# AronCao49/MoPA

Hardware: AMD Instinct MI355X
Metric: scans/sec (joint 2D+3D train step) at 1/2/4/8 MI355X; sparse-conv HBM GB/s (higher is better)
Workload: dtype f32

## Files before the change

### include/mopa_hip.h

```cpp
#ifndef MOPA_HIP_H
#define MOPA_HIP_H
#include <stddef.h>
#include <stdint.h>
#ifdef __cplusplus
extern "C" {
#endif


size_t mopa_scan_workspace_bytes(int64_t n);
int mopa_scan_exclusive_i32(const int32_t* in, int32_t* out, int32_t n, int32_t* total, void* ws, size_t ws_bytes, void* stream);
size_t mopa_voxel_hash_workspace_bytes(int64_t n_points);
int mopa_voxel_hash_build(const int64_t* coords, int64_t n_points, uint64_t* table_keys, int32_t* table_vals, int64_t table_cap, int32_t* point_row, uint64_t* row_keys, int32_t* num_rows, int32_t* status, void* ws, size_t ws_bytes, void* stream);
size_t mopa_coarsen_workspace_bytes(int64_t n_fine_cap);
int mopa_coarsen_build(const uint64_t* fine_keys, int32_t n_fine_cap, const int32_t* n_fine_dev, uint64_t* table_keys, int32_t* table_vals, int64_t table_cap, int32_t* parent, uint64_t* coarse_keys, int32_t* num_coarse, void* ws, size_t ws_bytes, void* stream);
int mopa_group_split(const int32_t* item_row, const int32_t* n_dev, int32_t n_host, int32_t n_cap, int32_t* out, void* stream);
int mopa_rulebook_subm(const uint64_t* row_keys, int32_t num_rows, const uint64_t* table_keys, const int32_t* table_vals, int64_t table_cap, int32_t spatial_size, int32_t* nbr , void* stream);
int mopa_rulebook_updown(const uint64_t* fine_keys, const int32_t* parent, int32_t num_fine, int32_t num_coarse, int32_t* ch , int32_t* up , void* stream);
size_t mopa_points_csr_workspace_bytes(int64_t num_rows);
int mopa_points_csr(const int32_t* point_row, int32_t n_points, int32_t num_rows, int32_t* row_start , int32_t* row_points , void* ws, size_t ws_bytes, void* stream);
int mopa_rotate_points_f32(const float* points, int32_t n, const float* rot_host , float* out, void* stream);
size_t mopa_voxelize_workspace_bytes(void);
int mopa_voxelize(const float* points, int32_t n, float scale, int32_t full_scale, const double* u_host, int32_t transl, int64_t batch_index, int64_t* coords , uint8_t* keep , void* ws, size_t ws_bytes, void* stream);

int mopa_spconv_fwd(const int32_t* nbr, int32_t K, int32_t num_out, const float* in, int32_t ld_in, int32_t cin, const float* weight, int32_t cout, int32_t w_flip, float* out, int32_t ld_out, void* stream);
int mopa_rulebook_groups_count(const int32_t* nbr, int32_t K, int32_t num_out, int32_t* tile_groups, void* stream);
int mopa_rulebook_groups_fill(const int32_t* nbr, int32_t K, int32_t num_out, const int32_t* grp_start, int32_t* grp_o, int32_t* grp_in, int32_t* grp_out, void* stream);
int mopa_rulebook_groups_count_batched(const int64_t* desc_host, int32_t ntables, int32_t total_tiles, int32_t* tile_groups, void* stream);
int mopa_rulebook_groups_fill_batched(const int64_t* desc_host, int32_t ntables, int32_t total_tiles, const int32_t* grp_start, int32_t* grp_o, int32_t* grp_in, int32_t* grp_out, void* stream);
int mopa_spconv_grouped_wants_packed(int32_t K, int32_t num_out, int32_t cin, int32_t cout);
int mopa_spconv_pack_weight(const float* w, int32_t K, int32_t cin, int32_t cout, int32_t transpose, int32_t ntw, float* wp, void* stream);
int mopa_spconv_pack_weights_batched(const int64_t* desc_host, int32_t n, void* stream);
size_t mopa_spconv_grouped_workspace_bytes(int32_t K, int32_t num_out, int32_t cout);
int mopa_spconv_fwd_grouped(const int32_t* grp_start, const int32_t* grp_o, const int32_t* grp_in, const int32_t* grp_out, int32_t K, int32_t num_out, const float* in, int32_t ld_in, int32_t cin, const float* weight, int32_t cout, int32_t w_flip, float* out, int32_t ld_out, void* ws, size_t ws_bytes, void* stream);
int mopa_spconv_transpose_weight(const float* weight, int32_t K, int32_t cin, int32_t cout, float* wt, void* stream);
size_t mopa_spconv_wgrad_workspace_bytes(int32_t K, int32_t num_out, int32_t cin, int32_t cout);
int mopa_spconv_bwd_weight(const int32_t* nbr, int32_t K, int32_t num_out, const float* in, int32_t ld_in, int32_t cin, const float* dout, int32_t ld_dout, int32_t cout, float* dweight, int32_t accumulate, void* ws, size_t ws_bytes, void* stream);

size_t mopa_rulebook_runs_bytes(int32_t K, int32_t num_out);
int mopa_rulebook_runs_build_batched(const int64_t* desc_host, int32_t n, void* stream);
int mopa_spconv_run_pack_weight(const float* w, int32_t K, int32_t cin, int32_t cout, int32_t transpose, float* wr, void* stream);
int mopa_spconv_run_wanted(int32_t K, int32_t num_out, int32_t cin, int32_t cout, int32_t one_rule_per_row);
int mopa_rulebook_runs_wanted(int32_t K, int32_t num_out, int32_t one_rule_per_row);
int mopa_spconv_run_form(int32_t cin, int32_t cout);
size_t mopa_spconv_run_workspace_bytes(int32_t K, int32_t num_out, int32_t cout);
int mopa_spconv_fwd_run(const int32_t* runs, int32_t K, int32_t num_out, const float* in, int32_t ld_in, int32_t cin, const float* weight_run, int32_t cout, int32_t w_flip, float* out, int32_t ld_out, int32_t one_rule_per_row, void* ws, size_t ws_bytes, void* stream);
int mopa_spconv_wgrad_run_wanted(int32_t K, int32_t num_out, int32_t cin, int32_t cout, int32_t one_rule_per_row);
size_t mopa_spconv_wgrad_run_workspace_bytes(int32_t K, int32_t num_out, int32_t cin, int32_t cout, int32_t one_rule_per_row);
int mopa_spconv_bwd_weight_run(const int32_t* runs, int32_t K, int32_t num_out, int32_t one_rule_per_row, int32_t swap, const float* in, int32_t ld_in, int32_t cin, const float* dout, int32_t ld_dout, int32_t cout, float* dweight, int32_t accumulate, void* ws, size_t ws_bytes, void* stream);

int mopa_exec_fn_id(const char* name_host);
int mopa_exec_fn_count(void);
int mopa_exec_replay(const int64_t* cmds_host, int64_t n_words, int64_t* fail_word_host);

int mopa_spconv_plan(int32_t K, int32_t num_out, int32_t cin, int32_t cout, int32_t ld_in, int32_t has_grouped, int32_t has_runs, int32_t one_rule_per_row);
size_t mopa_spconv_plan_workspace_bytes(int32_t plan, int32_t K, int32_t num_out, int32_t cout, int32_t one_rule_per_row);
int mopa_spconv_wgrad_plan(int32_t ckind, int32_t K, int32_t num_out, int32_t has_runs, int32_t one_rule_per_row, int32_t deconv_num_out, int32_t deconv_has_runs, int32_t deconv_one_rule_per_row, int32_t cin, int32_t cout);
size_t mopa_spconv_wgrad_plan_workspace_bytes(int32_t wplan, int32_t K, int32_t num_out, int32_t cin, int32_t cout, int32_t one_rule_per_row);
size_t mopa_scn_workspace_bytes(const int32_t* prog_host, int32_t n_ops, const int64_t* geom_host, int32_t num_classes, int32_t M);
int mopa_scn_forward(const int32_t* prog_host, int32_t n_ops, const int64_t* params_host, int64_t* forms_host, const int64_t* geom_host, const int64_t* bufs_host, const int64_t* io_host, void* ws, size_t ws_bytes, void* stream);
int mopa_scn_backward(const int32_t* prog_host, int32_t n_ops, const int32_t* plan_host, int32_t n_steps, const int64_t* params_host, int64_t* forms_host, const int64_t* grads_host, const int64_t* geom_host, const int64_t* bufs_host, const int64_t* gbufs_host, const int64_t* io_host, void* ws, size_t ws_bytes, void* stream);

size_t mopa_bnrelu_rows_workspace_bytes(int32_t num_rows, int32_t C);
int mopa_bn_act_fwd_groups(const float* x, int32_t ldx, float* y, int32_t ldy, int32_t num_rows, int32_t C, int32_t n_groups, int32_t split1, int32_t split2, const float* gamma, const float* beta, float* running_mean, float* running_var, float momentum, float eps, float leak, int32_t act, const float* res, int32_t ld_res, int32_t training, float* stats, void* ws, size_t ws_bytes, void* stream);
int mopa_bn_act_fwd_groups_bits(const float* x, int32_t ldx, float* y, int32_t ldy, int32_t num_rows, int32_t C, int32_t n_groups, int32_t split1, int32_t split2, const float* gamma, const float* beta, float* running_mean, float* running_var, float momentum, float eps, float leak, int32_t act, const float* res, int32_t ld_res, int32_t training, float* stats, int32_t want_bits, uint32_t* bits, void* ws, size_t ws_bytes, void* stream);
int mopa_bn_act_fwd(const float* x, int32_t ldx, float* y, int32_t ldy, int32_t num_rows, int32_t C, const float* gamma, const float* beta, float* running_mean, float* running_var, float momentum, float eps, float leak, int32_t act, const float* res, int32_t ld_res, int32_t training, float* stats, void* ws, size_t ws_bytes, void* stream);
int mopa_bnrelu_rows_fwd(const float* x, int32_t ldx, float* y, int32_t ldy, int32_t num_rows, int32_t C, const float* gamma, const float* beta, float* running_mean, float* running_var, float momentum, float eps, float leak, int32_t training, float* stats, void* ws, size_t ws_bytes, void* stream);
size_t mopa_bnrelu_rows_bwd_workspace_bytes(int32_t num_rows, int32_t C);
int mopa_bn_act_bwd_groups(const float* dy, int32_t ld_dy, const float* x, int32_t ldx, float* dx, int32_t ld_dx, int32_t num_rows, int32_t C, int32_t n_groups, int32_t split1, int32_t split2, const float* stats, float leak, int32_t act, const float* ymask, int32_t ld_ym, float* dres, int32_t ld_dres, int32_t accumulate_dres, int32_t training, float* dgamma, float* dbeta, int32_t accumulate_param_grads, int32_t accumulate_dx, void* ws, size_t ws_bytes, void* stream);
size_t mopa_bn_act_bwd_groups_fused_workspace_bytes(int32_t num_rows, int32_t C);
int mopa_bn_act_bwd_groups_fused(const float* dy, int32_t ld_dy, const float* x, int32_t ldx, float* dx, int32_t ld_dx, int32_t num_rows, int32_t C, int32_t n_groups, int32_t split1, int32_t split2, const float* stats, float leak, int32_t act, int32_t use_bits, const uint32_t* bits, float* dres, int32_t ld_dres, int32_t accumulate_dres, int32_t training, float* dgamma, float* dbeta, int32_t accumulate_param_grads, int32_t accumulate_dx, float* colsum_partial, void* ws, size_t ws_bytes, void* stream);
int mopa_bn_bwd_sums_groups(const float* dy, int32_t ld_dy, const float* x, int32_t ldx, int32_t num_rows, int32_t C, int32_t n_groups, int32_t split1, int32_t split2, const float* stats, float leak, int32_t act, const float* ymask, int32_t ld_ym, float* dgamma, float* dbeta, int32_t accumulate_param_grads, float* coef_out, void* ws, size_t ws_bytes, void* stream);
int mopa_bn_bwd_sums_groups_pool(const float* dpool, int32_t ld_dpool, const uint8_t* argmax, int32_t B, int32_t H, int32_t W, float* dy, int32_t ld_dy, int32_t accumulate_dy, const float* x, int32_t ldx, int32_t C, int32_t n_groups, const float* stats, float leak, int32_t act, float* dgamma, float* dbeta, int32_t accumulate_param_grads, float* coef_out, void* ws, size_t ws_bytes, void* stream);
int mopa_bn_act_bwd(const float* dy, int32_t ld_dy, const float* x, int32_t ldx, float* dx, int32_t ld_dx, int32_t num_rows, int32_t C, const float* stats, float leak, int32_t act, const float* ymask, int32_t ld_ym, float* dres, int32_t ld_dres, int32_t accumulate_dres, int32_t training, float* dgamma, float* dbeta, int32_t accumulate_param_grads, int32_t accumulate_dx, void* ws, size_t ws_bytes, void* stream);
int mopa_bnrelu_rows_bwd(const float* dy, int32_t ld_dy, const float* x, int32_t ldx, float* dx, int32_t ld_dx, int32_t num_rows, int32_t C, const float* stats, float leak, int32_t training, float* dgamma, float* dbeta, int32_t accumulate_param_grads, int32_t accumulate_dx, void* ws, size_t ws_bytes, void* stream);
int mopa_bn_sync_moments(const float* x, int32_t ldx, int32_t num_rows, int32_t C, double* moments, void* ws, size_t ws_bytes, void* stream);
int mopa_bn_act_fwd_sync(const float* x, int32_t ldx, float* y, int32_t ldy, int32_t num_rows, int32_t C, const float* gamma, const float* beta, float* running_mean, float* running_var, float momentum, float eps, float leak, int32_t act, const float* res, int32_t ld_res, const double* gathered, int32_t world, float* stats, void* stream);
int mopa_bn_sync_bwd_sums(const float* dy, int32_t ld_dy, const float* x, int32_t ldx, int32_t num_rows, int32_t C, const float* stats, float leak, int32_t act, const float* ymask, int32_t ld_ym, float* dgamma, float* dbeta, int32_t accumulate_param_grads, double* sums, void* ws, size_t ws_bytes, void* stream);
int mopa_bn_act_bwd_sync(const float* dy, int32_t ld_dy, const float* x, int32_t ldx, float* dx, int32_t ld_dx, int32_t num_rows, int32_t C, const float* stats, float leak, int32_t act, const float* ymask, int32_t ld_ym, float* dres, int32_t ld_dres, int32_t accumulate_dres, const double* sums_global, const double* gathered, int32_t world, int32_t accumulate_dx, float* coef_ws, void* stream);
int mopa_rows_add(const float* a, int32_t lda, const float* b, int32_t ldb, float* out, int32_t ldo, int32_t rows, int32_t C, void* stream);
int mopa_input_layer_fwd(const float* feats, int32_t cin, const int32_t* row_start, const int32_t* row_points, int32_t num_rows, float* out, int32_t ld_out, void* stream);
int mopa_input_layer_bwd(const float* dout, int32_t ld_dout, const int32_t* point_row, const int32_t* row_start, int32_t n_points, int32_t cin, float* dfeats, void* stream);
int mopa_heads_supported(int32_t M, int32_t num_classes);
int mopa_output_layer_heads_fwd(const float* y, int32_t ld_y, const int32_t* point_row, int32_t n_points, int32_t M, int32_t num_classes, const float* w1, const float* b1, const float* w2, const float* b2, float* feats, float* logit1, float* logit2, void* stream);
size_t mopa_output_layer_heads_bwd_workspace_bytes(int32_t n_points, int32_t M, int32_t num_classes);
int mopa_output_layer_heads_bwd(const float* dfeats, const float* dl1, const float* dl2, const float* feats, const float* w1, const float* w2, const int32_t* row_start, const int32_t* row_points, int32_t num_rows, int32_t n_points, int32_t M, int32_t num_classes, float* dy, int32_t ld_dy, float* dw1, float* db1, float* dw2, float* db2, int32_t accumulate, void* ws, size_t ws_bytes, void* stream);
int mopa_zero_rows(float* x, int32_t ld, int64_t rows, int32_t C, void* stream);
int mopa_copy_rows(const float* src, int32_t ld_src, float* dst, int32_t ld_dst, int64_t rows, int32_t C, void* stream);
int mopa_add_i64_many(const int64_t* ptrs_host, int32_t n, int64_t value, void* stream);

int mopa_conv2d_igemm(const float* in, const float* weight, const float* bias, float* out, const int32_t* geom_host, int32_t flags, void* stream);
int mopa_conv2d_igemm_classes(const float* in, const float* weight, const float* bias, float* out, const int32_t* geom4_host, int32_t flags, void* stream);
int mopa_conv2d_igemm_batched(const float* in, const float* weight, float* out, const int32_t* geom_host, int32_t nbatch, int64_t in_stride, int64_t w_stride, int64_t out_stride, int32_t flags, void* stream);
size_t mopa_conv2d_wgrad_workspace_bytes(const int32_t* geom_host);
int mopa_conv2d_bwd_weight(const float* in, const float* dy, float* dweight, const int32_t* geom_host, int32_t flags, void* ws, size_t ws_bytes, void* stream);
size_t mopa_convt_wgrad_workspace_bytes(const int32_t* geom_host);
int mopa_convt_bwd_weight(const float* in, const float* dy, float* dweight, const int32_t* geom_host, int32_t flags, void* ws, size_t ws_bytes, void* stream);
int mopa_stem_bwd_weight_bn(const float* in, const float* dy, int32_t ld_dy, const float* xbn, int32_t ld_x, const float* stats, const float* coef, int32_t n_groups, int32_t training, float* dweight, const int32_t* geom_host, int32_t flags, void* ws, size_t ws_bytes, void* stream);
int mopa_stem_bwd_weight2(const float* in, const float* dy, float* dweight, const int32_t* geom_host, int32_t flags, void* ws, size_t ws_bytes, void* stream);
int mopa_stem_bwd_weight_bn2(const float* in, const float* dy, int32_t ld_dy, const float* xbn, int32_t ld_x, const float* stats, const float* coef, int32_t n_groups, int32_t training, float* dweight, const int32_t* geom_host, int32_t flags, void* ws, size_t ws_bytes, void* stream);
size_t mopa_wino_wgrad_workspace_bytes(int32_t T, int32_t Cin, int32_t Cout);
int mopa_wino_bwd_weight(const float* V, const float* dM, int32_t T, int32_t Cin, int32_t Cout, float* dweight, int32_t flags, void* ws, size_t ws_bytes, void* stream);
size_t mopa_wino4_wgrad_workspace_bytes(int32_t T, int32_t Cin, int32_t Cout);
int mopa_wino4_bwd_weight(const float* V, const float* dM, int32_t T, int32_t Cin, int32_t Cout, float* dweight, int32_t flags, void* ws, size_t ws_bytes, void* stream);
int mopa_conv2d_relayout_weight(const float* src, float* dst, int32_t O, int32_t I, int32_t KH, int32_t KW, int32_t mode, int32_t inverse, int32_t accumulate, void* stream);
int mopa_conv2d_stem_relayout(const float* src, float* dst, int32_t O, int32_t inverse, int32_t accumulate, void* stream);
int mopa_img_to_nhwc4(const float* img, int32_t B, int32_t H, int32_t W, int32_t Hp, int32_t Wp, float* out, void* stream);
int mopa_stem_dgrad_image(const float* dout, int32_t ld, int32_t B, int32_t Hp, int32_t Wp, int32_t H, int32_t W, const float* w, float* dimg, void* stream);

int mopa_wino_weight(const float* weight, int32_t O, int32_t I, int32_t dgrad, float* U, void* stream);
int mopa_wino_input(const float* in, int32_t ld_in, int32_t B, int32_t H, int32_t W, int32_t C, float* V, void* stream);
int mopa_wino_output(const float* M, int32_t B, int32_t H, int32_t W, int32_t C, const float* bias, float* out, int32_t ld_out, int32_t accumulate, void* stream);
int mopa_wino_dout(const float* dy, int32_t ld, int32_t B, int32_t H, int32_t W, int32_t C, float* dM, void* stream);
int mopa_wino4_weight(const float* weight, int32_t O, int32_t I, int32_t dgrad, float* U, void* stream);
int mopa_wino4_input(const float* in, int32_t ld_in, int32_t B, int32_t H, int32_t W, int32_t C, float* V, void* stream);
int mopa_wino4_input_bn(const float* in, int32_t ld_in, int32_t B, int32_t H, int32_t W, int32_t C, const float* stats, int32_t n_groups, int32_t bn_c0, float* V, void* stream);
int mopa_wino4_output(const float* M, int32_t B, int32_t H, int32_t W, int32_t C, const float* bias, float* out, int32_t ld_out, int32_t accumulate, void* stream);
int mopa_wino4_dout(const float* dy, int32_t ld, int32_t B, int32_t H, int32_t W, int32_t C, float* dM, void* stream);
int mopa_conv2d_weight_forms_batched(const int64_t* desc_host, int32_t n, void* stream);
int mopa_wino4_weight_t(const float* weight, int32_t O, int32_t I, int32_t dgrad, float* Ut, void* stream);
int mopa_wino4_gemm_output(const float* V, const float* Ut, const float* bias, float* out, int32_t ld_out, int32_t B, int32_t H, int32_t W, int32_t Cin, int32_t Cout, int32_t accumulate, void* stream);
int mopa_wino4_weight_f(const float* weight, int32_t O, int32_t I, int32_t dgrad, float* Uf, void* stream);
int mopa_wino4_weight_q(const float* weight, int32_t O, int32_t I, int32_t dgrad, float* Uq, void* stream);
int mopa_wino4_conv_tiles32(int32_t mode);
int mopa_wino4_conv(const float* in, int32_t ld_in, const float* Uf, const float* bias, float* out, int32_t ld_out, int32_t B, int32_t H, int32_t W, int32_t Cin, int32_t Cout, int32_t accumulate, const float* stats, int32_t n_groups, int32_t bn_c0, float* V, void* stream);

int mopa_wino4_conv9(const float* in, int32_t ld_in, const float* Uq, const float* bias, float* out, int32_t ld_out, int32_t B, int32_t H, int32_t W, int32_t Cin, int32_t Cout, int32_t accumulate, const float* stats, int32_t n_groups, int32_t bn_c0, void* stream);

int mopa_wino4_wgrad_fused_ok(int32_t B, int32_t H, int32_t W, int32_t Cin, int32_t Cout);
size_t mopa_wino4_wgrad_fused_workspace_bytes(int32_t B, int32_t H, int32_t W, int32_t Cin, int32_t Cout);
int mopa_wino4_wgrad_fused(const float* in, int32_t ld_in, const float* stats, int32_t n_groups, int32_t bn_c0, const float* dy, int32_t ld_dy, int32_t B, int32_t H, int32_t W, int32_t Cin, int32_t Cout, float* dweight, int32_t flags, void* ws, size_t ws_bytes, void* stream);

int mopa_maxpool3x3s2_fwd(const float* x, int32_t ldx, int32_t B, int32_t H, int32_t W, int32_t C, float* y, int32_t ldy, uint8_t* argmax, void* stream);
int mopa_maxpool3x3s2_fwd_bn(const float* x, int32_t ldx, int32_t B, int32_t H, int32_t W, int32_t C, const float* stats, int32_t n_groups, float* y, int32_t ldy, uint8_t* argmax, void* stream);
int mopa_maxpool3x3s2_bwd(const float* dy, int32_t ld_dy, const uint8_t* argmax, int32_t B, int32_t H, int32_t W, int32_t C, float* dx, int32_t ld_dx, int32_t accumulate, void* stream);
int mopa_dropout_rows(const float* x, int32_t ldx, float* y, int32_t ldy, int64_t rows, int32_t C, float p, uint64_t seed, void* stream);
int mopa_dropout_rows_dseed(const float* x, int32_t ldx, float* y, int32_t ldy, int64_t rows, int32_t C, float p, const int64_t* seed_dev, int32_t site, void* stream);
int mopa_pixel_head_supported(int32_t M, int32_t num_classes);
int mopa_pixel_head_fwd(const float* x, int32_t ld, int32_t B, int32_t Hp, int32_t Wp, int32_t H, int32_t W, int32_t M, int32_t num_classes, const float* w, const float* bias, float* pred, void* stream);
size_t mopa_pixel_head_bwd_workspace_bytes(int32_t B, int32_t H, int32_t W, int32_t M, int32_t num_classes);
int mopa_pixel_head_bwd(const float* dpred, const float* x, int32_t ld, int32_t B, int32_t Hp, int32_t Wp, int32_t H, int32_t W, int32_t M, int32_t num_classes, const float* w, float* dx, int32_t ld_dx, int32_t accumulate_dx, float* dw, float* db, int32_t accumulate_params, void* ws, size_t ws_bytes, void* stream);
size_t mopa_colsum_workspace_bytes(int64_t num_rows, int32_t C);
int mopa_colsum(const float* x, int32_t ld, int64_t num_rows, int32_t C, float* out, int32_t accumulate, void* ws, size_t ws_bytes, void* stream);
size_t mopa_colsum_partial_blocks(int64_t num_rows);
int mopa_colsum_reduce(const float* partial, int64_t num_rows, int32_t C, float* out, int32_t accumulate, void* stream);
int mopa_pack_point_pix(const int64_t* idx, const int64_t* off_host, int32_t B, int32_t H, int32_t W, int32_t* pix, int32_t* status, void* stream);

size_t mopa_loss_workspace_bytes(int64_t n_rows);
int mopa_softmax_kl_fwd(const float* logit_p, const float* logit_q, int32_t N, int32_t C, float* loss, void* ws, size_t ws_bytes, void* stream);
int mopa_softmax_kl_bwd(const float* logit_p, const float* logit_q, int32_t N, int32_t C, const float* gout, float* dlogit_p, void* stream);
int mopa_wce_fwd(const float* logits, const int64_t* labels, const float* class_weight, int32_t N, int32_t C, int64_t ignore_index, float* loss, float* den, int32_t* status, void* ws, size_t ws_bytes, void* stream);
int mopa_wce_bwd(const float* logits, const int64_t* labels, const float* class_weight, int32_t N, int32_t C, int64_t ignore_index, const float* den, const float* gout, float* dlogits, void* stream);
size_t mopa_point_losses_workspace_bytes(int64_t n_rows);
int mopa_point_losses_fwd(const float* z2_main, const float* z2_xm, const float* z3_main, const float* z3_xm, const int64_t* y2, const int64_t* y3, const float* class_weight, int32_t N, int32_t C, int64_t ignore_index, float* scalars, int64_t* conf_2d, int64_t* conf_3d, const uint8_t* acc_mask, int64_t* acc_out, int32_t* status, void* ws, size_t ws_bytes, void* stream);
int mopa_point_losses_bwd(const float* z_main, const float* z_xm, const float* z_other_main, const int64_t* y, const float* class_weight, int32_t N, int32_t C, int64_t ignore_index, const float* den, const float* g, float* dz_main, float* dz_xm, void* stream);
size_t mopa_point_losses_seg_workspace_bytes(int32_t S);
int mopa_point_losses_seg_fwd(const float* z2_main, const float* z2_xm, const float* z3_main, const float* z3_xm, const float* class_weight, const int64_t* segs_host, int32_t S, int64_t N2, int64_t N3, int32_t C, int64_t ignore_index, float* scalars, int32_t* status, void* ws, size_t ws_bytes, void* stream);
int mopa_point_losses_seg_bwd(int32_t net, const float* z_main, const float* z_xm, const float* z_other_main, const float* class_weight, const int64_t* segs_host, int32_t S, int64_t N, int64_t N_other, int32_t C, int64_t ignore_index, const float* scalars, const float* g, float* dz_main, float* dz_xm, void* stream);
int mopa_softmax_fwd(const float* logits, int64_t n_rows, int32_t C, float* probs, void* stream);
int mopa_softmax_bwd(const float* probs, const float* dprobs, int64_t n_rows, int32_t C, float* dlogits, void* stream);
size_t mopa_mask_cons_workspace_bytes(int32_t B, int32_t HW, int32_t C);
size_t mopa_mask_cons_state_floats(int32_t B, int32_t C);
int mopa_mask_cons_fwd(const float* probs, const int32_t* masks, int32_t B, int32_t HW, int32_t C, int32_t k_norm, int32_t min_entropy, float* loss, float* state, void* ws, size_t ws_bytes, void* stream);
int mopa_mask_cons_bwd(const float* probs, const int32_t* masks, int32_t B, int32_t HW, int32_t C, int32_t k_norm, int32_t min_entropy, const float* state, const float* gout, float* dprobs, void* stream);

int mopa_pseudo_fuse(const float* logit_a, const float* logit_b, int32_t N, int32_t C, float* maxp, int64_t* label, void* stream);
size_t mopa_refine_pseudo_labels_workspace_bytes(int32_t C);
int mopa_refine_pseudo_labels(const float* prob, const int64_t* label_in, int32_t N, int32_t C, int64_t ignore_label, int64_t* label_out, void* ws, size_t ws_bytes, void* stream);
int mopa_ema_update(float* shadow, const float* param, int64_t n, float decay, void* stream);

int mopa_vgi_zslots(void);
int mopa_vgi_first_points(const float* points, int32_t stride, int32_t n, float voxel_size, int32_t ox, int32_t oy, int32_t X, int32_t Y, int32_t zlo, const uint8_t* g_mask, int32_t* first, int32_t* status, void* stream);
size_t mopa_vgi_first_points_rep_workspace_bytes(int32_t X, int32_t Y);
int mopa_vgi_first_points_rep(const float* points, int32_t stride, int32_t n, float voxel_size, double voxel_size64, int32_t ox, int32_t oy, int32_t X, int32_t Y, int32_t zlo, int32_t* first, int32_t* status, void* ws, size_t ws_bytes, void* stream);
size_t mopa_vgi_box_free_workspace_bytes(int32_t X, int32_t Y, int32_t Z);
int mopa_vgi_box_free(const int32_t* first, int32_t X, int32_t Y, int32_t zlo, int32_t gz0, int32_t Z, int32_t bx, int32_t by, int32_t bz, uint8_t* free_cells, void* ws, size_t ws_bytes, void* stream);
int mopa_vgi_ground_cells(const int32_t* first, const uint8_t* g_mask, int32_t X, int32_t Y, uint8_t* ground2d, void* stream);
int mopa_vgi_candidates(const uint8_t* free_cells, int32_t Xo, int32_t Yo, int32_t Zo, const double* params_host, const uint8_t* ground2d, int32_t ox, int32_t oy, int32_t X, int32_t Y, uint8_t* cand2d, int32_t* counts, void* stream);
int mopa_vgi_compact_cells(const uint8_t* cand2d, int32_t X, int32_t Y, int32_t ox, int32_t oy, int32_t* cells , int32_t* count, void* stream);
int mopa_vgi_road_height(const float* points, int32_t stride, int32_t n, float voxel_size, const int32_t* first, const uint8_t* g_mask, int32_t ox, int32_t oy, int32_t X, int32_t Y, int32_t zlo, int32_t cell_x, int32_t cell_y, double* out , void* stream);
size_t mopa_vgi_range_keep_workspace_bytes(int32_t n, int32_t W, int32_t H);
int mopa_vgi_range_keep(const double* points, int32_t n, int32_t n_scan, double fov_up, double fov_down, int32_t W, int32_t H, uint8_t* keep, void* ws, size_t ws_bytes, void* stream);
size_t mopa_voxelize_f64_workspace_bytes(void);
// ... 84 lines not shown
```

### mopa_amd/_abi.py

```python
SIGNATURES = {
    'mopa_scan_workspace_bytes': ('z', 'l'),
    'mopa_scan_exclusive_i32': ('i', 'ppippzp'),
    'mopa_voxel_hash_workspace_bytes': ('z', 'l'),
    'mopa_voxel_hash_build': ('i', 'plpplpppppzp'),
    'mopa_coarsen_workspace_bytes': ('z', 'l'),
    'mopa_coarsen_build': ('i', 'pippplppppzp'),
    'mopa_group_split': ('i', 'ppiipp'),
    'mopa_rulebook_subm': ('i', 'pipplipp'),
    'mopa_rulebook_updown': ('i', 'ppiippp'),
    'mopa_points_csr_workspace_bytes': ('z', 'l'),
    'mopa_points_csr': ('i', 'piipppzp'),
    'mopa_rotate_points_f32': ('i', 'pippp'),
    'mopa_voxelize_workspace_bytes': ('z', ''),
    'mopa_voxelize': ('i', 'pifipilpppzp'),
    'mopa_spconv_fwd': ('i', 'piipiipiipip'),
    'mopa_rulebook_groups_count': ('i', 'piipp'),
    'mopa_rulebook_groups_fill': ('i', 'piippppp'),
    'mopa_rulebook_groups_count_batched': ('i', 'piipp'),
    'mopa_rulebook_groups_fill_batched': ('i', 'piippppp'),
    'mopa_spconv_grouped_wants_packed': ('i', 'iiii'),
    'mopa_spconv_pack_weight': ('i', 'piiiiipp'),
    'mopa_spconv_pack_weights_batched': ('i', 'pip'),
    'mopa_spconv_grouped_workspace_bytes': ('z', 'iii'),
    'mopa_spconv_fwd_grouped': ('i', 'ppppiipiipiipipzp'),
    'mopa_spconv_transpose_weight': ('i', 'piiipp'),
    'mopa_spconv_wgrad_workspace_bytes': ('z', 'iiii'),
    'mopa_spconv_bwd_weight': ('i', 'piipiipiipipzp'),
    'mopa_rulebook_runs_bytes': ('z', 'ii'),
    'mopa_rulebook_runs_build_batched': ('i', 'pip'),
    'mopa_spconv_run_pack_weight': ('i', 'piiiipp'),
    'mopa_spconv_run_wanted': ('i', 'iiiii'),
    'mopa_rulebook_runs_wanted': ('i', 'iii'),
    'mopa_spconv_run_form': ('i', 'ii'),
    'mopa_spconv_run_workspace_bytes': ('z', 'iii'),
    'mopa_spconv_fwd_run': ('i', 'piipiipiipiipzp'),
    'mopa_spconv_wgrad_run_wanted': ('i', 'iiiii'),
    'mopa_spconv_wgrad_run_workspace_bytes': ('z', 'iiiii'),
    'mopa_spconv_bwd_weight_run': ('i', 'piiiipiipiipipzp'),
    'mopa_exec_fn_id': ('i', 'p'),
    'mopa_exec_fn_count': ('i', ''),
    'mopa_exec_replay': ('i', 'plp'),
    'mopa_spconv_plan': ('i', 'iiiiiiii'),
    'mopa_spconv_plan_workspace_bytes': ('z', 'iiiii'),
    'mopa_spconv_wgrad_plan': ('i', 'iiiiiiiiii'),
    'mopa_spconv_wgrad_plan_workspace_bytes': ('z', 'iiiiii'),
    'mopa_scn_workspace_bytes': ('z', 'pipii'),
    'mopa_scn_forward': ('i', 'pippppppzp'),
    'mopa_scn_backward': ('i', 'pipippppppppzp'),
    'mopa_bnrelu_rows_workspace_bytes': ('z', 'ii'),
    'mopa_bn_act_fwd_groups': ('i', 'pipiiiiiippppfffipiippzp'),
    'mopa_bn_act_fwd_groups_bits': ('i', 'pipiiiiiippppfffipiipippzp'),
    'mopa_bn_act_fwd': ('i', 'pipiiippppfffipiippzp'),
    'mopa_bnrelu_rows_fwd': ('i', 'pipiiippppfffippzp'),
    'mopa_bnrelu_rows_bwd_workspace_bytes': ('z', 'ii'),
    'mopa_bn_act_bwd_groups': ('i', 'pipipiiiiiipfipipiiippiipzp'),
    'mopa_bn_act_bwd_groups_fused_workspace_bytes': ('z', 'ii'),
    'mopa_bn_act_bwd_groups_fused': ('i', 'pipipiiiiiipfiippiiippiippzp'),
    'mopa_bn_bwd_sums_groups': ('i', 'pipiiiiiipfipippippzp'),
    'mopa_bn_bwd_sums_groups_pool': ('i', 'pipiiipiipiiipfippippzp'),
    'mopa_bn_act_bwd': ('i', 'pipipiiipfipipiiippiipzp'),
    'mopa_bnrelu_rows_bwd': ('i', 'pipipiiipfippiipzp'),
    'mopa_bn_sync_moments': ('i', 'piiippzp'),
    'mopa_bn_act_fwd_sync': ('i', 'pipiiippppfffipipipp'),
    'mopa_bn_sync_bwd_sums': ('i', 'pipiiipfipippippzp'),
    'mopa_bn_act_bwd_sync': ('i', 'pipipiiipfipipiippiipp'),
    'mopa_rows_add': ('i', 'pipipiiip'),
    'mopa_input_layer_fwd': ('i', 'pippipip'),
    'mopa_input_layer_bwd': ('i', 'pippiipp'),
    'mopa_heads_supported': ('i', 'ii'),
    'mopa_output_layer_heads_fwd': ('i', 'pipiiipppppppp'),
    'mopa_output_layer_heads_bwd_workspace_bytes': ('z', 'iii'),
    'mopa_output_layer_heads_bwd': ('i', 'ppppppppiiiipippppipzp'),
    'mopa_zero_rows': ('i', 'pilip'),
    'mopa_copy_rows': ('i', 'pipilip'),
    'mopa_add_i64_many': ('i', 'pilp'),
    'mopa_conv2d_igemm': ('i', 'pppppip'),
    'mopa_conv2d_igemm_classes': ('i', 'pppppip'),
    'mopa_conv2d_igemm_batched': ('i', 'ppppilllip'),
    'mopa_conv2d_wgrad_workspace_bytes': ('z', 'p'),
    'mopa_conv2d_bwd_weight': ('i', 'ppppipzp'),
    'mopa_convt_wgrad_workspace_bytes': ('z', 'p'),
    'mopa_convt_bwd_weight': ('i', 'ppppipzp'),
    'mopa_stem_bwd_weight_bn': ('i', 'ppipippiippipzp'),
    'mopa_stem_bwd_weight2': ('i', 'ppppipzp'),
    'mopa_stem_bwd_weight_bn2': ('i', 'ppipippiippipzp'),
    'mopa_wino_wgrad_workspace_bytes': ('z', 'iii'),
    'mopa_wino_bwd_weight': ('i', 'ppiiipipzp'),
    'mopa_wino4_wgrad_workspace_bytes': ('z', 'iii'),
    'mopa_wino4_bwd_weight': ('i', 'ppiiipipzp'),
    'mopa_conv2d_relayout_weight': ('i', 'ppiiiiiiip'),
    'mopa_conv2d_stem_relayout': ('i', 'ppiiip'),
    'mopa_img_to_nhwc4': ('i', 'piiiiipp'),
    'mopa_stem_dgrad_image': ('i', 'piiiiiippp'),
    'mopa_wino_weight': ('i', 'piiipp'),
    'mopa_wino_input': ('i', 'piiiiipp'),
    'mopa_wino_output': ('i', 'piiiippiip'),
    'mopa_wino_dout': ('i', 'piiiiipp'),
    'mopa_wino4_weight': ('i', 'piiipp'),
    'mopa_wino4_input': ('i', 'piiiiipp'),
    'mopa_wino4_input_bn': ('i', 'piiiiipiipp'),
    'mopa_wino4_output': ('i', 'piiiippiip'),
    'mopa_wino4_dout': ('i', 'piiiiipp'),
    'mopa_conv2d_weight_forms_batched': ('i', 'pip'),
    'mopa_wino4_weight_t': ('i', 'piiipp'),
    'mopa_wino4_gemm_output': ('i', 'ppppiiiiiiip'),
    'mopa_wino4_weight_f': ('i', 'piiipp'),
    'mopa_wino4_weight_q': ('i', 'piiipp'),
    'mopa_wino4_conv_tiles32': ('i', 'i'),
    'mopa_wino4_conv': ('i', 'pipppiiiiiiipiipp'),
    'mopa_wino4_conv9': ('i', 'pipppiiiiiiipiip'),
    'mopa_wino4_wgrad_fused_ok': ('i', 'iiiii'),
    'mopa_wino4_wgrad_fused_workspace_bytes': ('z', 'iiiii'),
    'mopa_wino4_wgrad_fused': ('i', 'pipiipiiiiiipipzp'),
    'mopa_maxpool3x3s2_fwd': ('i', 'piiiiipipp'),
    'mopa_maxpool3x3s2_fwd_bn': ('i', 'piiiiipipipp'),
    'mopa_maxpool3x3s2_bwd': ('i', 'pipiiiipiip'),
    'mopa_dropout_rows': ('i', 'pipilifup'),
    'mopa_dropout_rows_dseed': ('i', 'pipilifpip'),
    'mopa_pixel_head_supported': ('i', 'ii'),
    'mopa_pixel_head_fwd': ('i', 'piiiiiiiipppp'),
    'mopa_pixel_head_bwd_workspace_bytes': ('z', 'iiiii'),
    'mopa_pixel_head_bwd': ('i', 'ppiiiiiiiippiippipzp'),
    'mopa_colsum_workspace_bytes': ('z', 'li'),
    'mopa_colsum': ('i', 'pilipipzp'),
    'mopa_colsum_partial_blocks': ('z', 'l'),
    'mopa_colsum_reduce': ('i', 'plipip'),
    'mopa_pack_point_pix': ('i', 'ppiiippp'),
    'mopa_loss_workspace_bytes': ('z', 'l'),
    'mopa_softmax_kl_fwd': ('i', 'ppiippzp'),
    'mopa_softmax_kl_bwd': ('i', 'ppiippp'),
    'mopa_wce_fwd': ('i', 'pppiilppppzp'),
    'mopa_wce_bwd': ('i', 'pppiilpppp'),
    'mopa_point_losses_workspace_bytes': ('z', 'l'),
    'mopa_point_losses_fwd': ('i', 'pppppppiilpppppppzp'),
    'mopa_point_losses_bwd': ('i', 'pppppiilppppp'),
    'mopa_point_losses_seg_workspace_bytes': ('z', 'i'),
    'mopa_point_losses_seg_fwd': ('i', 'ppppppillilpppzp'),
    'mopa_point_losses_seg_bwd': ('i', 'ipppppillilppppp'),
    'mopa_softmax_fwd': ('i', 'plipp'),
    'mopa_softmax_bwd': ('i', 'pplipp'),
    'mopa_mask_cons_workspace_bytes': ('z', 'iii'),
    'mopa_mask_cons_state_floats': ('z', 'ii'),
    'mopa_mask_cons_fwd': ('i', 'ppiiiiipppzp'),
    'mopa_mask_cons_bwd': ('i', 'ppiiiiipppp'),
    'mopa_pseudo_fuse': ('i', 'ppiippp'),
    'mopa_refine_pseudo_labels_workspace_bytes': ('z', 'i'),
    'mopa_refine_pseudo_labels': ('i', 'ppiilppzp'),
    'mopa_ema_update': ('i', 'pplfp'),
    'mopa_vgi_zslots': ('i', ''),
    'mopa_vgi_first_points': ('i', 'piifiiiiipppp'),
    'mopa_vgi_first_points_rep_workspace_bytes': ('z', 'ii'),
    'mopa_vgi_first_points_rep': ('i', 'piifdiiiiipppzp'),
    'mopa_vgi_box_free_workspace_bytes': ('z', 'iii'),
    'mopa_vgi_box_free': ('i', 'piiiiiiiippzp'),
    'mopa_vgi_ground_cells': ('i', 'ppiipp'),
    'mopa_vgi_candidates': ('i', 'piiippiiiippp'),
    'mopa_vgi_compact_cells': ('i', 'piiiippp'),
    'mopa_vgi_road_height': ('i', 'piifppiiiiiiipp'),
    'mopa_vgi_range_keep_workspace_bytes': ('z', 'iii'),
    'mopa_vgi_range_keep': ('i', 'piiddiippzp'),
    'mopa_voxelize_f64_workspace_bytes': ('z', ''),
    'mopa_voxelize_f64': ('i', 'pippdipilpppzp'),
    'mopa_eval_logits_workspace_bytes': ('z', 'ii'),
    'mopa_eval_logits': ('i', 'plplpiipiippppppppzp'),
    'mopa_confusion_update': ('i', 'pplpiipp'),
    'mopa_imageprep_resize_u8': ('i', 'piiipipiiiipp'),
    'mopa_imageprep_contrast_sums': ('i', 'piliipppp'),
    'mopa_imageprep_pixels': ('i', 'piliippppppppp'),
# ... 32 lines not shown
    'mopa_jpeg_max_images': ('i', ''),
    'mopa_jpeg_header_bytes': ('i', ''),
    'mopa_jpeg_info': ('i', 'ppl'),
    'mopa_jpeg_coeff_bytes': ('z', 'p'),
    'mopa_jpeg_entropy_decode': ('i', 'pppll'),
    'mopa_jpeg_decode_batch': ('i', 'pppippp'),
    'mopa_ground_patches': ('i', ''),
    'mopa_ground_rows_per_block': ('i', ''),
    'mopa_ground_resident_capacity': ('i', ''),
    'mopa_ground_num_params': ('i', ''),
    'mopa_ground_workspace_bytes': ('z', 'll'),
    'mopa_ground_launches': ('i', 'l'),
    'mopa_ground_estimate': ('i', 'pipillpppzp'),
    'mopa_objects_rows_per_block': ('i', ''),
    'mopa_objects_max_classes': ('i', ''),
    'mopa_objects_num_params': ('i', ''),
    'mopa_objects_launches': ('i', ''),
    'mopa_objects_max_instances': ('z', 'lii'),
    'mopa_objects_workspace_bytes': ('z', 'llii'),
    'mopa_objects_extract': ('i', 'pipipillpipppppppppzp'),
    'mopa_adam_flat': ('i', 'pppplffffffffp'),
    'mopa_grad_stats_chunk': ('i', ''),
    'mopa_grad_stats_workspace_bytes': ('z', 'l'),
    'mopa_grad_stats': ('i', 'ppllffipppzp'),
    'mopa_adam_flat_guarded': ('i', 'pppplffffffffpp'),
    'mopa_adamw_flat': ('i', 'pppplffffffffp'),
    'mopa_adamw_flat_guarded': ('i', 'pppplffffffffpp'),
    'mopa_sgd_flat': ('i', 'ppplffffiifp'),
    'mopa_sgd_flat_guarded': ('i', 'ppplffffipfpp'),
}

HOST_PARAMS = {
    'mopa_a2d2prep_map': {0: 'cam_host'},
    'mopa_a2d2prep_points': {0: 'points_host', 1: 'row_host', 2: 'col_host', 3: 'refl_host', 4: 'label_host', 5: 'n_host'},
    'mopa_a2d2prep_remap': {0: 'src_host', 1: 'dst_host'},
    'mopa_add_i64_many': {0: 'ptrs_host'},
    'mopa_conv2d_bwd_weight': {3: 'geom_host'},
    'mopa_conv2d_igemm': {4: 'geom_host'},
    'mopa_conv2d_igemm_batched': {3: 'geom_host'},
    'mopa_conv2d_igemm_classes': {4: 'geom4_host'},
    'mopa_conv2d_weight_forms_batched': {0: 'desc_host'},
    'mopa_conv2d_wgrad_workspace_bytes': {0: 'geom_host'},
    'mopa_convt_bwd_weight': {3: 'geom_host'},
    'mopa_convt_wgrad_workspace_bytes': {0: 'geom_host'},
    'mopa_exec_fn_id': {0: 'name_host'},
    'mopa_exec_replay': {0: 'cmds_host', 2: 'fail_word_host'},
    'mopa_ground_estimate': {6: 'params_host'},
    'mopa_imageprep_contrast_sums': {0: 'src_host', 5: 'order_host', 6: 'factor_host'},
    'mopa_imageprep_contrast_sums4': {0: 'src_host', 5: 'order_host', 6: 'factor_host', 7: 'shift_host'},
    'mopa_imageprep_indices': {0: 'pts_host', 1: 'n_host', 7: 'win_host', 9: 'flip_host', 10: 'idx_host', 11: 'ori_host', 12: 'keep_host'},
    'mopa_imageprep_mask': {0: 'mask_host', 10: 'row_limit_host', 12: 'crop_host', 15: 'flip_host'},
    'mopa_imageprep_pixels': {0: 'src_host', 5: 'order_host', 6: 'factor_host', 8: 'flip_host', 11: 'norm_host'},
    'mopa_imageprep_pixels4': {0: 'src_host', 5: 'order_host', 6: 'factor_host', 7: 'shift_host', 9: 'flip_host', 12: 'norm_host'},
    'mopa_imageprep_resize_u8': {0: 'src_host'},
    'mopa_jpeg_coeff_bytes': {0: 'header_host'},
    'mopa_jpeg_decode_batch': {0: 'coeff_ptrs_host', 1: 'coeff_bytes_host', 2: 'headers_host', 4: 'dst_ptrs_host', 5: 'pitch_host'},
    'mopa_jpeg_entropy_decode': {0: 'data_host', 1: 'header_host', 2: 'coeff_host'},
    'mopa_jpeg_info': {0: 'data_host', 1: 'header_host'},
    'mopa_kittiprep_count': {0: 'scan_host', 1: 'n_host', 2: 'proj_host', 3: 'mask_host', 4: 'mask_n_host'},
    'mopa_kittiprep_ground': {0: 'gidx_host', 1: 'g_host', 2: 'n_host'},
    'mopa_kittiprep_scatter': {0: 'scan_host', 1: 'label_host', 3: 'n_host', 4: 'proj_host'},
    'mopa_nuscprep_count': {0: 'scan_host', 1: 'n_host', 2: 'cols_host'},
    'mopa_nuscprep_scatter': {0: 'scan_host', 1: 'n_host', 2: 'cols_host', 3: 'boxoff_host'},
    'mopa_objects_extract': {8: 'class_ids_host', 10: 'params_host'},
    'mopa_pack_point_pix': {1: 'off_host'},
    'mopa_point_losses_seg_bwd': {5: 'segs_host'},
    'mopa_point_losses_seg_fwd': {5: 'segs_host'},
    'mopa_refine_pseudo_labels_segmented': {0: 'prob_host', 1: 'label_host', 3: 'n_host', 4: 'out_host'},
    'mopa_rotate_points_f32': {2: 'rot_host'},
    'mopa_rulebook_groups_count_batched': {0: 'desc_host'},
    'mopa_rulebook_groups_fill_batched': {0: 'desc_host'},
    'mopa_rulebook_runs_build_batched': {0: 'desc_host'},
    'mopa_scanprep_compact': {0: 'src_host', 1: 'keep_in_host', 2: 'n_host', 3: 'u_host', 4: 'transl_host'},
    'mopa_scanprep_count': {0: 'src_host', 1: 'keep_in_host', 2: 'n_host', 3: 'u_host', 4: 'transl_host'},
    'mopa_scanprep_rotate': {0: 'src_host', 1: 'dst_host', 2: 'n_host', 3: 'rot_host'},
    'mopa_scanprep_take': {3: 'n_host', 5: 'label_host', 10: 'img_host', 11: 'src_host'},
    'mopa_scn_backward': {0: 'prog_host', 2: 'plan_host', 4: 'params_host', 5: 'forms_host', 6: 'grads_host', 7: 'geom_host', 8: 'bufs_host', 9: 'gbufs_host', 10: 'io_host'},
    'mopa_scn_forward': {0: 'prog_host', 2: 'params_host', 3: 'forms_host', 4: 'geom_host', 5: 'bufs_host', 6: 'io_host'},
    'mopa_scn_workspace_bytes': {0: 'prog_host', 2: 'geom_host'},
    'mopa_spconv_pack_weights_batched': {0: 'desc_host'},
    'mopa_stem_bwd_weight2': {3: 'geom_host'},
    'mopa_stem_bwd_weight_bn': {10: 'geom_host'},
    'mopa_stem_bwd_weight_bn2': {10: 'geom_host'},
    'mopa_vgi_candidates': {4: 'params_host'},
    'mopa_voxelize': {4: 'u_host'},
    'mopa_voxelize_f64': {3: 'rot_host', 6: 'u_host'},
}
```

### mopa_amd/csrc/conv2d.hip

```cpp
#include "common.h"
#include "wino4.h"
#include "weight_forms.h"
#include <stdlib.h>
#include <string.h>

struct ConvGeom {
  int B, IH, IW, OHl, OWl, OHa, OWa;
  int OS, OOY, OOX;
  int IS, IY0, IX0, IDY, IDX;
  int TH, TW, KH0, KW0, KS, KWF;
  int Cin, Cout, ld_in, ld_out;
};

#define BK 16
#define APAD 4

template <int BM, int BN, int TM, int TN>
__global__ __launch_bounds__(256, 2) void k_conv2d_igemm(const float* __restrict__ in, const float* __restrict__ w,
                                                          const float* __restrict__ bias, float* __restrict__ out,
                                                          const ConvGeom g, int accumulate, int64_t bs_in, int64_t bs_w,
                                                          int64_t bs_out) {
  in += blockIdx.z * bs_in;
  w += blockIdx.z * bs_w;
  out += blockIdx.z * bs_out;
// ... 992 lines not shown
                                                             int accumulate, int Cin, int Cout) {
  constexpr int NL = 256 / EW;
  __shared__ float red[NL][EW + 1];
  const int el = threadIdx.x % EW, cl = threadIdx.x / EW;
  const int64_t i = (int64_t)blockIdx.x * EW + el;
  float s = 0.f;
  if (i < n)
#pragma unroll 8
    for (int c = cl; c < nsplit; c += NL) s += slabs[(int64_t)c * n + i];
  red[cl][el] = s;
  __syncthreads();
  if (cl == 0 && i < n) {
    const int co = (int)(i % Cout);
    const int64_t r = i / Cout;
    const int ci = (int)(r % Cin), tap = (int)(r / Cin);
    const int64_t o = ((int64_t)ci * Cout + co) * 4 + tap;
    float t = 0.f;
#pragma unroll
    for (int k = 0; k < NL; ++k) t += red[k][el];
    dw[o] = (accumulate ? dw[o] : 0.f) + t;
  }
}

static bool convt_wgrad_geom(const ConvGeom& g) {
  return g.B > 0 && g.IH > 0 && g.IW > 0 && g.OHl == g.IH && g.OWl == g.IW && g.OHa >= 2 * g.IH && g.OWa >= 2 * g.IW && g.OS == 2 &&
         g.OOY == 0 && g.OOX == 0 && g.IS == 1 && g.IY0 == 0 && g.IX0 == 0 && g.TH == 1 && g.TW == 1 && g.Cin % 64 == 0 && g.Cin >= 64 &&
         g.Cout % 64 == 0 && g.Cout >= 64 && g.ld_in % 4 == 0 && g.ld_out % 4 == 0 && g.ld_in >= g.Cin && g.ld_out >= g.Cout &&
         (int64_t)g.B * g.IH * g.IW < (1ll << 31);
}

MOPA_API size_t mopa_convt_wgrad_workspace_bytes(const int32_t* geom_host) {
  return 4 * mopa_conv2d_wgrad_workspace_bytes(geom_host);
}

MOPA_API int mopa_convt_bwd_weight(const float* in, const float* dy, float* dweight, const int32_t* geom_host, int32_t flags, void* ws,
                                   size_t ws_bytes, void* stream) {
  ConvGeom g;
  memcpy(&g, geom_host, sizeof(g));
  if (!convt_wgrad_geom(g) || !wgrad_use_mfma(g)) return MOPA_ERR_ARG;
  if ((((uintptr_t)in | (uintptr_t)dy | (uintptr_t)ws) & 15) != 0) return MOPA_ERR_ARG;
  if (ws_bytes < mopa_convt_wgrad_workspace_bytes(geom_host)) return MOPA_ERR_WORKSPACE;
  int ns, mps;
  wgrad_split(g, &ns, &mps);
  hipStream_t st = (hipStream_t)stream;
  float* slabs = (float*)ws;
  dim3 grid(1, (g.Cin / 64) * (g.Cout / 64), ns);
  k_convt_wgrad_mfma<<<grid, 256, 0, st>>>(in, dy, slabs, g, mps);
  const int64_t n1 = (int64_t)g.Cin * g.Cout, n = 4 * n1;
  const int ew = reduce_ew(n1);
  const unsigned nb = (unsigned)cdiv64(n, ew);
  if (ew == 64) k_reduce_slabs_convt<64><<<nb, 256, 0, st>>>(slabs, ns, n, dweight, flags & 1, g.Cin, g.Cout);
  else if (ew == 32) k_reduce_slabs_convt<32><<<nb, 256, 0, st>>>(slabs, ns, n, dweight, flags & 1, g.Cin, g.Cout);
  else k_reduce_slabs_convt<16><<<nb, 256, 0, st>>>(slabs, ns, n, dweight, flags & 1, g.Cin, g.Cout);
  MOPA_CHECK_LAUNCH();
  return MOPA_OK;
}

MOPA_API int mopa_stem_bwd_weight_bn(const float* in, const float* dy, int32_t ld_dy, const float* xbn, int32_t ld_x, const float* stats,
                                     const float* coef, int32_t n_groups, int32_t training, float* dweight, const int32_t* geom_host,
                                     int32_t flags, void* ws, size_t ws_bytes, void* stream) {
  ConvGeom g;
  memcpy(&g, geom_host, sizeof(g));
  const int accumulate = flags & 1, oihw = (flags >> 1) & 1;
  if (!stem_wgrad_mfma(g) || g.OS != 1 || g.OOY != 0 || g.OOX != 0 || n_groups < 1 || n_groups > 3 || g.B % n_groups || ld_dy < 64 ||
      ld_x < 64 || ((ld_dy | ld_x | g.ld_in) & 3) || !xbn || !stats || !coef)
    return MOPA_ERR_ARG;
  if (oihw && (g.KS != 1 || g.KH0 != 0 || g.KW0 != 0 || g.KWF != g.TW)) return MOPA_ERR_ARG;
  if (ws_bytes < mopa_conv2d_wgrad_workspace_bytes(geom_host)) return MOPA_ERR_WORKSPACE;
  int ns, mps;
  wgrad_split(g, &ns, &mps);
  hipStream_t st = (hipStream_t)stream;
  float* slabs = (float*)ws;
  StemBn bn{xbn, stats, coef, ld_x, ld_dy, g.B / n_groups, n_groups, training};
  k_stem_wgrad_mfma<true><<<ns, 256, 0, st>>>(in, dy, slabs, g, mps, bn);
  const int64_t n = (int64_t)g.TH * g.TW * g.Cin * g.Cout;
  reduce_slabs2_launch(slabs, ns, n, dweight, accumulate, oihw, g.TH * g.TW, g.Cin, g.Cout, st);
  MOPA_CHECK_LAUNCH();
  return MOPA_OK;
}

#define SP 64
#define SSLOTS 512
static_assert(7 * (SP + 7) <= SSLOTS && SP % 16 == 0, "strip staging: two float4 per thread");
template <int NT>
__device__ __forceinline__ void stem_strip_mma(f32x16 (&acc)[4], const float* sp, const float* bp, int np) {
  constexpr int SW = 4 * (SP + 7);
  float b0 = bp[0], a0[NT];
#pragma unroll
  for (int n = 0; n < NT; ++n) a0[n] = sp[n * 2 * SW];
#define STEM_STRIP_PAIR(I)                                                                                          \
  {                                                                                                                 \
    const int nx = min((I) + 1, np - 1);                                                                            \
    const float b1 = bp[nx * 128];                                                                                  \
    float a1[NT];                                                                                                   \
    _Pragma("unroll") for (int n = 0; n < NT; ++n) a1[n] = sp[n * 2 * SW + nx * 8];                                 \
    _Pragma("unroll") for (int n = 0; n < NT; ++n) acc[n] = __builtin_amdgcn_mfma_f32_32x32x2f32(a0[n], b0, acc[n], 0, 0, 0); \
    b0 = b1;                                                                                                        \
    _Pragma("unroll") for (int n = 0; n < NT; ++n) a0[n] = a1[n];                                                   \
  }
  int i = 0;
  for (; i + 4 <= np; i += 4) {
#pragma unroll
    for (int u = 0; u < 4; ++u) STEM_STRIP_PAIR(i + u)
  }
  for (; i < np; ++i) STEM_STRIP_PAIR(i)
#undef STEM_STRIP_PAIR
}
template <bool BNB>
__global__ __launch_bounds__(256, 2) void k_stem_wgrad_strip(const float* __restrict__ in, const float* __restrict__ dy,
                                                              float* __restrict__ slabs, const ConvGeom g, int m_per_split,
                                                              const StemBn bn) {
  constexpr int SW = 4 * (SP + 7);
  constexpr int NB = SP / 16;
  __shared__ __attribute__((aligned(16))) float Ss[2][SSLOTS * 4];
  __shared__ __attribute__((aligned(16))) float Bs[2][SP][64];
  __shared__ __attribute__((aligned(16))) float cst[BNB ? 3 : 1][6][BNB ? 64 : 4];
  const int t = threadIdx.x;
  if (BNB) {
    for (int i = t; i < bn.n_groups * 6 * 64; i += 256) {
      const int gi = i / 384, k = (i - gi * 384) >> 6, c = i & 63;
      cst[gi][k][c] = k < 4 ? bn.stats[(gi * 4 + k) * 64 + c] : bn.coef[(gi * 2 + (k - 4)) * 64 + c];
    }
  }
  const int M = g.B * g.OHl * g.OWl, ohw = g.OHl * g.OWl;
  const int mbeg = blockIdx.x * m_per_split, mend = min(M, mbeg + m_per_split);
  const int lane = t & 63, wv = __builtin_amdgcn_readfirstlane(t >> 6);
  const int wco = (wv & 1) * 32, rt0 = wv >> 1;
  const int l32 = lane & 31, lk = lane >> 5;
  const int ld_dy = BNB ? bn.ld_dy : g.ld_out;
  f32x16 acc[4];
#pragma unroll
  for (int n = 0; n < 4; ++n)
#pragma unroll
    for (int e = 0; e < 16; ++e) acc[n][e] = 0.f;
  int scol[2], soff[2];
#pragma unroll
  for (int j = 0; j < 2; ++j) {
    const int e = t + 256 * j, r = e / (SP + 7);
    scol[j] = e < 7 * (SP + 7) ? e - r * (SP + 7) : 2 * SP;
    soff[j] = (r * g.IW + scol[j]) * 4;
  }
  const int bpx = t >> 4, bq = t & 15;
  float4 rs[2], rb[NB], rx[NB];
  int cm = mbeg, cb = __builtin_amdgcn_readfirstlane(cm / ohw), cy = __builtin_amdgcn_readfirstlane((cm - cb * ohw) / g.OWl);
  int cx = cm - cb * ohw - cy * g.OWl;
  int llen = 0, lgi = 0;
  auto load_chunk = [&]() {
    const int len = min(min(SP, g.OWl - cx), mend - cm);
    const float* sbase = in + ((int64_t)(cb * g.IH + cy) * g.IW + cx) * 4;
#pragma unroll
    for (int j = 0; j < 2; ++j) rs[j] = *reinterpret_cast<const float4*>(sbase + (scol[j] < len + 7 ? soff[j] : 0));
    const float* dbase = dy + (int64_t)cm * ld_dy + bq * 4;
#pragma unroll
    for (int j = 0; j < NB; ++j) rb[j] = *reinterpret_cast<const float4*>(dbase + (bpx + 16 * j < len ? (bpx + 16 * j) * ld_dy : 0));
    if (BNB) {
      const float* xbase = bn.xbn + (int64_t)cm * bn.ld_x + bq * 4;
#pragma unroll
      for (int j = 0; j < NB; ++j) rx[j] = *reinterpret_cast<const float4*>(xbase + (bpx + 16 * j < len ? (bpx + 16 * j) * bn.ld_x : 0));
      lgi = cb / bn.imgs_per_group;
    }
    llen = len;
    cm += len;
    cx += len;
    if (cx == g.OWl) {
      cx = 0;
      if (++cy == g.OHl) { cy = 0; ++cb; }
    }
  };
  auto store_chunk = [&](int buf) {
#pragma unroll
    for (int j = 0; j < 2; ++j) {
      const bool ok = scol[j] < llen + 7;
      *reinterpret_cast<float4*>(&Ss[buf][(t + 256 * j) * 4]) =
          make_float4(ok ? rs[j].x : 0.f, ok ? rs[j].y : 0.f, ok ? rs[j].z : 0.f, ok ? rs[j].w : 0.f);
    }
#pragma unroll
    for (int j = 0; j < NB; ++j) {
      const bool ok = bpx + 16 * j < llen;
      float o[4] = {rb[j].x, rb[j].y, rb[j].z, rb[j].w};
      if (BNB) {
        const float xs[4] = {rx[j].x, rx[j].y, rx[j].z, rx[j].w};
#pragma unroll
        for (int q = 0; q < 4; ++q) {
          const int c = bq * 4 + q;
          const float sc = cst[lgi][0][c], sh = cst[lgi][1][c], mean = cst[lgi][2][c], inv = cst[lgi][3][c], c0 = cst[lgi][4][c], c1 = cst[lgi][5][c];
          const float gs = o[q];
          const float yv = fmaf(xs[q], sc, sh);
          const float dz = yv > 0.f ? gs : gs * 0.f;
          if (bn.training) {
            const float xhat = (xs[q] - mean) * inv;
            o[q] = sc * (dz - c0 - xhat * c1);
          } else {
            o[q] = sc * dz;
          }
        }
      }
      *reinterpret_cast<float4*>(&Bs[buf][bpx + 16 * j][bq * 4]) = make_float4(ok ? o[0] : 0.f, ok ? o[1] : 0.f, ok ? o[2] : 0.f, ok ? o[3] : 0.f);
    }
  };
  int buf = 0, len = 0;
  if (BNB) __syncthreads();
  if (mbeg < mend) {
    load_chunk();
    store_chunk(0);
    len = llen;
  }
  __syncthreads();
  while (len > 0) {
    const bool more = cm < mend;
    if (more) load_chunk();
    const float* sp = &Ss[buf][rt0 * SW + 4 * lk + l32];
    const float* bp = &Bs[buf][lk][wco + l32];
    const int np = (len + 1) >> 1;
    if (rt0 == 0) stem_strip_mma<4>(acc, sp, bp, np);
    else stem_strip_mma<3>(acc, sp, bp, np);
    if (more) {
      store_chunk(buf ^ 1);
      __syncthreads();
      buf ^= 1;
      len = llen;
    } else {
      len = 0;
    }
  }
  float* dst = slabs + (int64_t)blockIdx.x * STEM_ROWS * 64 + wco + l32;
#pragma unroll
  for (int n = 0; n < 4; ++n) {
    const int rt = rt0 + 2 * n;
    if (rt < 7) {
#pragma unroll
      for (int e = 0; e < 16; ++e) dst[(int64_t)(rt * 32 + 8 * (e >> 2) + 4 * lk + (e & 3)) * 64] = acc[n][e];
    }
  }
}
static bool stem_strip_geom(const ConvGeom& g) {
  return stem_wgrad_mfma(g) && g.IS == 1 && g.IY0 == 0 && g.IX0 == 0 && g.IDY == 1 && g.IDX == 4 && g.ld_in == 4 && g.OS == 1 &&
         g.OOY == 0 && g.OOX == 0 && g.OHa == g.OHl && g.OWa == g.OWl && g.IH >= g.OHl + 6 && g.IW >= g.OWl + 7 && g.B > 0 && g.OHl > 0 &&
         g.OWl > 0 && (int64_t)g.B * g.IH * g.IW < (1ll << 29);
}
__global__ __launch_bounds__(256) void k_reduce_slabs_stem(const float* __restrict__ slabs, int nsplit, float* __restrict__ dw, int accumulate) {
  constexpr int EW = 16, NL = 256 / EW, n = STEM_ROWS * 64;
  __shared__ float red[NL][EW + 1];
  const int el = threadIdx.x % EW, cl = threadIdx.x / EW;
  const int i = blockIdx.x * EW + el;
  float s = 0.f;
#pragma unroll 8
  for (int c = cl; c < nsplit; c += NL) s += slabs[(int64_t)c * n + i];
  red[cl][el] = s;
  __syncthreads();
  if (cl == 0) {
    float t = 0.f;
#pragma unroll
    for (int k = 0; k < NL; ++k) t += red[k][el];
    const int o = i % 64;
    int r = i / 64;
    const int k16 = r % 16; r /= 16;
    const int tx = r % 2, kh = r / 2;
    const int kw = 4 * tx + k16 / 4, c = k16 % 4;
    if (kw < 7 && c < 3) {
      const int p = ((o * 3 + c) * 7 + kh) * 7 + kw;
      dw[p] = (accumulate ? dw[p] : 0.f) + t;
    }
  }
}
static int stem_wgrad2_launch(const float* in, const float* dy, float* dweight, const int32_t* geom_host, int32_t flags, void* ws,
                              size_t ws_bytes, void* stream, const StemBn* bn) {
  ConvGeom g;
  memcpy(&g, geom_host, sizeof(g));
  const int accumulate = flags & 1, param = (flags >> 1) & 1;
  if (!stem_strip_geom(g) || !in || !dy || !dweight || (flags & ~3)) return MOPA_ERR_ARG;
  if (!bn && (g.ld_out < 64 || (g.ld_out & 3))) return MOPA_ERR_ARG;
  static_assert(STEM_ROWS * 64 < 32 * 512, "k_reduce_slabs_stem is k_reduce_slabs2<16>");
  if (ws_bytes < mopa_conv2d_wgrad_workspace_bytes(geom_host)) return MOPA_ERR_WORKSPACE;
  int ns, mps;
  wgrad_split(g, &ns, &mps);
  hipStream_t st = (hipStream_t)stream;
  float* slabs = (float*)ws;
  if (bn) k_stem_wgrad_strip<true><<<ns, 256, 0, st>>>(in, dy, slabs, g, mps, *bn);
  else k_stem_wgrad_strip<false><<<ns, 256, 0, st>>>(in, dy, slabs, g, mps, StemBn{});
  const int n = STEM_ROWS * 64;
  if (param) k_reduce_slabs_stem<<<n / 16, 256, 0, st>>>(slabs, ns, dweight, accumulate);
  else reduce_slabs2_launch(slabs, ns, n, dweight, accumulate, 0, 14, 16, 64, st);
  MOPA_CHECK_LAUNCH();
  return MOPA_OK;
}
MOPA_API int mopa_stem_bwd_weight2(const float* in, const float* dy, float* dweight, const int32_t* geom_host, int32_t flags, void* ws,
                                   size_t ws_bytes, void* stream) {
  return stem_wgrad2_launch(in, dy, dweight, geom_host, flags, ws, ws_bytes, stream, nullptr);
}
MOPA_API int mopa_stem_bwd_weight_bn2(const float* in, const float* dy, int32_t ld_dy, const float* xbn, int32_t ld_x, const float* stats,
                                      const float* coef, int32_t n_groups, int32_t training, float* dweight, const int32_t* geom_host,
                                      int32_t flags, void* ws, size_t ws_bytes, void* stream) {
  ConvGeom g;
  memcpy(&g, geom_host, sizeof(g));
  if (n_groups < 1 || n_groups > 3 || g.B <= 0 || g.B % n_groups || ld_dy < 64 || ld_x < 64 || ((ld_dy | ld_x) & 3) || !xbn || !stats || !coef)
    return MOPA_ERR_ARG;
  const StemBn bn{xbn, stats, coef, ld_x, ld_dy, g.B / n_groups, n_groups, training};
  return stem_wgrad2_launch(in, dy, dweight, geom_host, flags, ws, ws_bytes, stream, &bn);
}

__global__ __launch_bounds__(256) void k_wino_dw(const float* __restrict__ slabs, int nsplit, int64_t n, float* __restrict__ dw,
                                                  int accumulate, int oihw, int Cin, int Cout) {
  __shared__ float red[16][17];
  const int e = threadIdx.x & 15, p = threadIdx.x >> 4;
  const int64_t i = (int64_t)blockIdx.x * 16 + e;
  float s = 0.f;
  if (i < n)
#pragma unroll 8
    for (int c = 0; c < nsplit; ++c) s += slabs[((int64_t)c * 16 + p) * n + i];
  red[p][e] = s;
  __syncthreads();
  if (p != 0 || i >= n) return;
  float u[4][4];
#pragma unroll
  for (int q = 0; q < 16; ++q) u[q >> 2][q & 3] = red[q][e];
  float t[3][4];
#pragma unroll
  for (int j = 0; j < 4; ++j) {
    t[0][j] = u[0][j] + 0.5f * (u[1][j] + u[2][j]);
    t[1][j] = 0.5f * (u[1][j] - u[2][j]);
    t[2][j] = 0.5f * (u[1][j] + u[2][j]) + u[3][j];
  }
  const int co = (int)(i % Cout), ci = (int)(i / Cout);
  const int64_t base = oihw ? ((int64_t)co * Cin + ci) * 9 : i, step = oihw ? 1 : n;
#pragma unroll
  for (int a = 0; a < 3; ++a) {
    float g0 = t[a][0] + 0.5f * (t[a][1] + t[a][2]), g1 = 0.5f * (t[a][1] - t[a][2]), g2 = 0.5f * (t[a][1] + t[a][2]) + t[a][3];
    float* d = dw + base + (int64_t)(a * 3) * step;
    if (accumulate) { g0 += d[0]; g1 += d[step]; g2 += d[2 * step]; }
    d[0] = g0; d[step] = g1; d[2 * step] = g2;
  }
}

template <int EW>
__global__ __launch_bounds__(256) void k_wino4_dw(const float* __restrict__ slabs, int nsplit, int64_t n, float* __restrict__ dw,
                                                   int accumulate, int oihw, int Cin, int Cout) {
  constexpr int NQ = 256 / EW;
  __shared__ float red[36][EW + 1];
  const int e = threadIdx.x % EW, q = threadIdx.x / EW;
  const int64_t i = (int64_t)blockIdx.x * EW + e;
#pragma unroll
  for (int k = 0; k < (36 + NQ - 1) / NQ; ++k) {
    const int p = q + k * NQ;
    if (p < 36) {
      float s = 0.f;
      if (i < n) {
#pragma unroll 8
        for (int c = 0; c < nsplit; ++c) s += slabs[((int64_t)c * 36 + p) * n + i];
      }
      red[p][e] = s;
    }
  }
  __syncthreads();
  if (q != 0 || i >= n) return;
  float t[3][6];
#pragma unroll
  for (int j = 0; j < 6; ++j) {
    const float u0 = red[0 * 6 + j][e], u1 = red[1 * 6 + j][e], u2 = red[2 * 6 + j][e], u3 = red[3 * 6 + j][e], u4 = red[4 * 6 + j][e],
                u5 = red[5 * 6 + j][e];
    t[0][j] = 0.25f * u0 - (1.f / 6.f) * (u1 + u2) + (1.f / 24.f) * (u3 + u4);
    t[1][j] = (1.f / 6.f) * (u2 - u1) + (1.f / 12.f) * (u3 - u4);
    t[2][j] = -(1.f / 6.f) * (u1 + u2) + (1.f / 6.f) * (u3 + u4) + u5;
  }
  const int co = (int)(i % Cout), ci = (int)(i / Cout);
  const int64_t base = oihw ? ((int64_t)co * Cin + ci) * 9 : i, step = oihw ? 1 : n;
#pragma unroll
  for (int a = 0; a < 3; ++a) {
    float g0 = 0.25f * t[a][0] - (1.f / 6.f) * (t[a][1] + t[a][2]) + (1.f / 24.f) * (t[a][3] + t[a][4]);
    float g1 = (1.f / 6.f) * (t[a][2] - t[a][1]) + (1.f / 12.f) * (t[a][3] - t[a][4]);
    float g2 = -(1.f / 6.f) * (t[a][1] + t[a][2]) + (1.f / 6.f) * (t[a][3] + t[a][4]) + t[a][5];
    float* d = dw + base + (int64_t)(a * 3) * step;
    if (accumulate) { g0 += d[0]; g1 += d[step]; g2 += d[2 * step]; }
    d[0] = g0; d[step] = g1; d[2 * step] = g2;
  }
}

int wino4_dw_launch(const float* slabs, int nsplit, int Cin, int Cout, float* dweight, int flags, hipStream_t st) {
  const int64_t n = (int64_t)Cin * Cout;
  const int ew = reduce_ew(n), acc = flags & 1, oihw = (flags >> 1) & 1;
  const unsigned nb = (unsigned)cdiv64(n, ew);
  if (ew == 64) k_wino4_dw<64><<<nb, 256, 0, st>>>(slabs, nsplit, n, dweight, acc, oihw, Cin, Cout);
// ... 182 lines not shown
```

### mopa_amd/csrc/exec_table.inc

```
static const char* const EXEC_NAMES[] = {
  "mopa_a2d2prep_map",
  "mopa_a2d2prep_points",
  "mopa_a2d2prep_remap",
  "mopa_adam_flat",
  "mopa_adam_flat_guarded",
  "mopa_adamw_flat",
  "mopa_adamw_flat_guarded",
  "mopa_add_i64_many",
  "mopa_bn_act_bwd",
  "mopa_bn_act_bwd_groups",
  "mopa_bn_act_bwd_groups_fused",
  "mopa_bn_act_bwd_sync",
  "mopa_bn_act_fwd",
  "mopa_bn_act_fwd_groups",
  "mopa_bn_act_fwd_groups_bits",
  "mopa_bn_act_fwd_sync",
  "mopa_bn_bwd_sums_groups",
  "mopa_bn_bwd_sums_groups_pool",
  "mopa_bn_sync_bwd_sums",
  "mopa_bn_sync_moments",
  "mopa_bnrelu_rows_bwd",
  "mopa_bnrelu_rows_fwd",
  "mopa_coarsen_build",
  "mopa_colsum",
// ... 6 lines not shown
  "mopa_conv2d_relayout_weight",
  "mopa_conv2d_stem_relayout",
  "mopa_conv2d_weight_forms_batched",
  "mopa_convt_bwd_weight",
  "mopa_copy_rows",
  "mopa_dropout_rows",
  "mopa_dropout_rows_dseed",
  "mopa_ema_update",
  "mopa_eval_logits",
  "mopa_grad_stats",
  "mopa_ground_estimate",
  "mopa_group_split",
  "mopa_imageprep_contrast_sums",
  "mopa_imageprep_contrast_sums4",
  "mopa_imageprep_indices",
  "mopa_imageprep_mask",
  "mopa_imageprep_pixels",
  "mopa_imageprep_pixels4",
  "mopa_imageprep_resize_u8",
  "mopa_img_to_nhwc4",
  "mopa_input_layer_bwd",
  "mopa_input_layer_fwd",
  "mopa_jpeg_decode_batch",
  "mopa_kittiprep_count",
  "mopa_kittiprep_ground",
  "mopa_kittiprep_scatter",
  "mopa_mask_cons_bwd",
  "mopa_mask_cons_fwd",
  "mopa_maxpool3x3s2_bwd",
  "mopa_maxpool3x3s2_fwd",
  "mopa_maxpool3x3s2_fwd_bn",
  "mopa_nuscprep_count",
  "mopa_nuscprep_scatter",
  "mopa_nuscprep_setup",
  "mopa_objects_extract",
  "mopa_output_layer_heads_bwd",
  "mopa_output_layer_heads_fwd",
  "mopa_pack_point_pix",
  "mopa_pixel_head_bwd",
  "mopa_pixel_head_fwd",
  "mopa_point_losses_bwd",
  "mopa_point_losses_fwd",
  "mopa_point_losses_seg_bwd",
  "mopa_point_losses_seg_fwd",
  "mopa_points_csr",
  "mopa_pseudo_fuse",
  "mopa_refine_pseudo_labels",
  "mopa_refine_pseudo_labels_segmented",
  "mopa_rotate_points_f32",
  "mopa_rows_add",
  "mopa_rulebook_groups_count",
  "mopa_rulebook_groups_count_batched",
  "mopa_rulebook_groups_fill",
  "mopa_rulebook_groups_fill_batched",
  "mopa_rulebook_runs_build_batched",
  "mopa_rulebook_subm",
  "mopa_rulebook_updown",
  "mopa_scan_exclusive_i32",
  "mopa_scanprep_compact",
  "mopa_scanprep_count",
  "mopa_scanprep_rotate",
  "mopa_scanprep_take",
  "mopa_scn_backward",
  "mopa_scn_forward",
  "mopa_sgd_flat",
  "mopa_sgd_flat_guarded",
  "mopa_softmax_bwd",
  "mopa_softmax_fwd",
  "mopa_softmax_kl_bwd",
  "mopa_softmax_kl_fwd",
  "mopa_spconv_bwd_weight",
  "mopa_spconv_bwd_weight_run",
  "mopa_spconv_fwd",
  "mopa_spconv_fwd_grouped",
  "mopa_spconv_fwd_run",
  "mopa_spconv_pack_weight",
  "mopa_spconv_pack_weights_batched",
  "mopa_spconv_run_pack_weight",
  "mopa_spconv_transpose_weight",
  "mopa_stem_bwd_weight2",
  "mopa_stem_bwd_weight_bn",
  "mopa_stem_bwd_weight_bn2",
  "mopa_stem_dgrad_image",
  "mopa_vgi_box_free",
  "mopa_vgi_candidates",
  "mopa_vgi_compact_cells",
  "mopa_vgi_first_points",
  "mopa_vgi_first_points_rep",
  "mopa_vgi_ground_cells",
  "mopa_vgi_range_keep",
  "mopa_vgi_road_height",
  "mopa_voxel_hash_build",
  "mopa_voxelize",
  "mopa_voxelize_f64",
  "mopa_wce_bwd",
  "mopa_wce_fwd",
  "mopa_wino4_bwd_weight",
  "mopa_wino4_conv",
  "mopa_wino4_conv9",
  "mopa_wino4_dout",
  "mopa_wino4_gemm_output",
  "mopa_wino4_input",
  "mopa_wino4_input_bn",
  "mopa_wino4_output",
  "mopa_wino4_weight",
  "mopa_wino4_weight_f",
  "mopa_wino4_weight_q",
  "mopa_wino4_weight_t",
  "mopa_wino4_wgrad_fused",
  "mopa_wino_bwd_weight",
  "mopa_wino_dout",
  "mopa_wino_input",
  "mopa_wino_output",
  "mopa_wino_weight",
  "mopa_zero_rows",
};
static const int EXEC_N = 145;
static int exec_dispatch(int id, const int64_t* a, int nargs) {
  switch (id) {
    case 0: return nargs == 6 ? mopa_a2d2prep_map((const double*)(uintptr_t)a[0], (int32_t)a[1], (int32_t)a[2], (int16_t*)(uintptr_t)a[3], (uint16_t*)(uintptr_t)a[4], (void*)(uintptr_t)a[5]) : MOPA_ERR_ARG;
    case 1: return nargs == 21 ? mopa_a2d2prep_points((const void* const*)(uintptr_t)a[0], (const void* const*)(uintptr_t)a[1], (const void* const*)(uintptr_t)a[2], (const void* const*)(uintptr_t)a[3], (const void* const*)(uintptr_t)a[4], (const int32_t*)(uintptr_t)a[5], (int32_t)a[6], (int32_t)a[7], (int32_t)a[8], (const int16_t*)(uintptr_t)a[9], (const uint16_t*)(uintptr_t)a[10], (int32_t)a[11], (int32_t)a[12], (const uint8_t*)(uintptr_t)a[13], (int32_t)a[14], (float*)(uintptr_t)a[15], (float*)(uintptr_t)a[16], (uint8_t*)(uintptr_t)a[17], (float*)(uintptr_t)a[18], (int32_t*)(uintptr_t)a[19], (void*)(uintptr_t)a[20]) : MOPA_ERR_ARG;
    case 2: return nargs == 8 ? mopa_a2d2prep_remap((const void* const*)(uintptr_t)a[0], (void* const*)(uintptr_t)a[1], (int32_t)a[2], (int32_t)a[3], (int32_t)a[4], (const int16_t*)(uintptr_t)a[5], (const uint16_t*)(uintptr_t)a[6], (void*)(uintptr_t)a[7]) : MOPA_ERR_ARG;
    case 3: return nargs == 14 ? mopa_adam_flat((float*)(uintptr_t)a[0], (const float*)(uintptr_t)a[1], (float*)(uintptr_t)a[2], (float*)(uintptr_t)a[3], (int64_t)a[4], (float)slot_f(a[5]), (float)slot_f(a[6]), (float)slot_f(a[7]), (float)slot_f(a[8]), (float)slot_f(a[9]), (float)slot_f(a[10]), (float)slot_f(a[11]), (float)slot_f(a[12]), (void*)(uintptr_t)a[13]) : MOPA_ERR_ARG;
    case 4: return nargs == 15 ? mopa_adam_flat_guarded((float*)(uintptr_t)a[0], (const float*)(uintptr_t)a[1], (float*)(uintptr_t)a[2], (float*)(uintptr_t)a[3], (int64_t)a[4], (float)slot_f(a[5]), (float)slot_f(a[6]), (float)slot_f(a[7]), (float)slot_f(a[8]), (float)slot_f(a[9]), (float)slot_f(a[10]), (float)slot_f(a[11]), (float)slot_f(a[12]), (const void*)(uintptr_t)a[13], (void*)(uintptr_t)a[14]) : MOPA_ERR_ARG;
    case 5: return nargs == 14 ? mopa_adamw_flat((float*)(uintptr_t)a[0], (const float*)(uintptr_t)a[1], (float*)(uintptr_t)a[2], (float*)(uintptr_t)a[3], (int64_t)a[4], (float)slot_f(a[5]), (float)slot_f(a[6]), (float)slot_f(a[7]), (float)slot_f(a[8]), (float)slot_f(a[9]), (float)slot_f(a[10]), (float)slot_f(a[11]), (float)slot_f(a[12]), (void*)(uintptr_t)a[13]) : MOPA_ERR_ARG;
    case 6: return nargs == 15 ? mopa_adamw_flat_guarded((float*)(uintptr_t)a[0], (const float*)(uintptr_t)a[1], (float*)(uintptr_t)a[2], (float*)(uintptr_t)a[3], (int64_t)a[4], (float)slot_f(a[5]), (float)slot_f(a[6]), (float)slot_f(a[7]), (float)slot_f(a[8]), (float)slot_f(a[9]), (float)slot_f(a[10]), (float)slot_f(a[11]), (float)slot_f(a[12]), (const void*)(uintptr_t)a[13], (void*)(uintptr_t)a[14]) : MOPA_ERR_ARG;
    case 7: return nargs == 4 ? mopa_add_i64_many((const int64_t*)(uintptr_t)a[0], (int32_t)a[1], (int64_t)a[2], (void*)(uintptr_t)a[3]) : MOPA_ERR_ARG;
    case 8: return nargs == 24 ? mopa_bn_act_bwd((const float*)(uintptr_t)a[0], (int32_t)a[1], (const float*)(uintptr_t)a[2], (int32_t)a[3], (float*)(uintptr_t)a[4], (int32_t)a[5], (int32_t)a[6], (int32_t)a[7], (const float*)(uintptr_t)a[8], (float)slot_f(a[9]), (int32_t)a[10], (const float*)(uintptr_t)a[11], (int32_t)a[12], (float*)(uintptr_t)a[13], (int32_t)a[14], (int32_t)a[15], (int32_t)a[16], (float*)(uintptr_t)a[17], (float*)(uintptr_t)a[18], (int32_t)a[19], (int32_t)a[20], (void*)(uintptr_t)a[21], (size_t)a[22], (void*)(uintptr_t)a[23]) : MOPA_ERR_ARG;
    case 9: return nargs == 27 ? mopa_bn_act_bwd_groups((const float*)(uintptr_t)a[0], (int32_t)a[1], (const float*)(uintptr_t)a[2], (int32_t)a[3], (float*)(uintptr_t)a[4], (int32_t)a[5], (int32_t)a[6], (int32_t)a[7], (int32_t)a[8], (int32_t)a[9], (int32_t)a[10], (const float*)(uintptr_t)a[11], (float)slot_f(a[12]), (int32_t)a[13], (const float*)(uintptr_t)a[14], (int32_t)a[15], (float*)(uintptr_t)a[16], (int32_t)a[17], (int32_t)a[18], (int32_t)a[19], (float*)(uintptr_t)a[20], (float*)(uintptr_t)a[21], (int32_t)a[22], (int32_t)a[23], (void*)(uintptr_t)a[24], (size_t)a[25], (void*)(uintptr_t)a[26]) : MOPA_ERR_ARG;
    case 10: return nargs == 28 ? mopa_bn_act_bwd_groups_fused((const float*)(uintptr_t)a[0], (int32_t)a[1], (const float*)(uintptr_t)a[2], (int32_t)a[3], (float*)(uintptr_t)a[4], (int32_t)a[5], (int32_t)a[6], (int32_t)a[7], (int32_t)a[8], (int32_t)a[9], (int32_t)a[10], (const float*)(uintptr_t)a[11], (float)slot_f(a[12]), (int32_t)a[13], (int32_t)a[14], (const uint32_t*)(uintptr_t)a[15], (float*)(uintptr_t)a[16], (int32_t)a[17], (int32_t)a[18], (int32_t)a[19], (float*)(uintptr_t)a[20], (float*)(uintptr_t)a[21], (int32_t)a[22], (int32_t)a[23], (float*)(uintptr_t)a[24], (void*)(uintptr_t)a[25], (size_t)a[26], (void*)(uintptr_t)a[27]) : MOPA_ERR_ARG;
    case 11: return nargs == 22 ? mopa_bn_act_bwd_sync((const float*)(uintptr_t)a[0], (int32_t)a[1], (const float*)(uintptr_t)a[2], (int32_t)a[3], (float*)(uintptr_t)a[4], (int32_t)a[5], (int32_t)a[6], (int32_t)a[7], (const float*)(uintptr_t)a[8], (float)slot_f(a[9]), (int32_t)a[10], (const float*)(uintptr_t)a[11], (int32_t)a[12], (float*)(uintptr_t)a[13], (int32_t)a[14], (int32_t)a[15], (const double*)(uintptr_t)a[16], (const double*)(uintptr_t)a[17], (int32_t)a[18], (int32_t)a[19], (float*)(uintptr_t)a[20], (void*)(uintptr_t)a[21]) : MOPA_ERR_ARG;
    case 12: return nargs == 21 ? mopa_bn_act_fwd((const float*)(uintptr_t)a[0], (int32_t)a[1], (float*)(uintptr_t)a[2], (int32_t)a[3], (int32_t)a[4], (int32_t)a[5], (const float*)(uintptr_t)a[6], (const float*)(uintptr_t)a[7], (float*)(uintptr_t)a[8], (float*)(uintptr_t)a[9], (float)slot_f(a[10]), (float)slot_f(a[11]), (float)slot_f(a[12]), (int32_t)a[13], (const float*)(uintptr_t)a[14], (int32_t)a[15], (int32_t)a[16], (float*)(uintptr_t)a[17], (void*)(uintptr_t)a[18], (size_t)a[19], (void*)(uintptr_t)a[20]) : MOPA_ERR_ARG;
    case 13: return nargs == 24 ? mopa_bn_act_fwd_groups((const float*)(uintptr_t)a[0], (int32_t)a[1], (float*)(uintptr_t)a[2], (int32_t)a[3], (int32_t)a[4], (int32_t)a[5], (int32_t)a[6], (int32_t)a[7], (int32_t)a[8], (const float*)(uintptr_t)a[9], (const float*)(uintptr_t)a[10], (float*)(uintptr_t)a[11], (float*)(uintptr_t)a[12], (float)slot_f(a[13]), (float)slot_f(a[14]), (float)slot_f(a[15]), (int32_t)a[16], (const float*)(uintptr_t)a[17], (int32_t)a[18], (int32_t)a[19], (float*)(uintptr_t)a[20], (void*)(uintptr_t)a[21], (size_t)a[22], (void*)(uintptr_t)a[23]) : MOPA_ERR_ARG;
    case 14: return nargs == 26 ? mopa_bn_act_fwd_groups_bits((const float*)(uintptr_t)a[0], (int32_t)a[1], (float*)(uintptr_t)a[2], (int32_t)a[3], (int32_t)a[4], (int32_t)a[5], (int32_t)a[6], (int32_t)a[7], (int32_t)a[8], (const float*)(uintptr_t)a[9], (const float*)(uintptr_t)a[10], (float*)(uintptr_t)a[11], (float*)(uintptr_t)a[12], (float)slot_f(a[13]), (float)slot_f(a[14]), (float)slot_f(a[15]), (int32_t)a[16], (const float*)(uintptr_t)a[17], (int32_t)a[18], (int32_t)a[19], (float*)(uintptr_t)a[20], (int32_t)a[21], (uint32_t*)(uintptr_t)a[22], (void*)(uintptr_t)a[23], (size_t)a[24], (void*)(uintptr_t)a[25]) : MOPA_ERR_ARG;
    case 15: return nargs == 20 ? mopa_bn_act_fwd_sync((const float*)(uintptr_t)a[0], (int32_t)a[1], (float*)(uintptr_t)a[2], (int32_t)a[3], (int32_t)a[4], (int32_t)a[5], (const float*)(uintptr_t)a[6], (const float*)(uintptr_t)a[7], (float*)(uintptr_t)a[8], (float*)(uintptr_t)a[9], (float)slot_f(a[10]), (float)slot_f(a[11]), (float)slot_f(a[12]), (int32_t)a[13], (const float*)(uintptr_t)a[14], (int32_t)a[15], (const double*)(uintptr_t)a[16], (int32_t)a[17], (float*)(uintptr_t)a[18], (void*)(uintptr_t)a[19]) : MOPA_ERR_ARG;
    case 16: return nargs == 21 ? mopa_bn_bwd_sums_groups((const float*)(uintptr_t)a[0], (int32_t)a[1], (const float*)(uintptr_t)a[2], (int32_t)a[3], (int32_t)a[4], (int32_t)a[5], (int32_t)a[6], (int32_t)a[7], (int32_t)a[8], (const float*)(uintptr_t)a[9], (float)slot_f(a[10]), (int32_t)a[11], (const float*)(uintptr_t)a[12], (int32_t)a[13], (float*)(uintptr_t)a[14], (float*)(uintptr_t)a[15], (int32_t)a[16], (float*)(uintptr_t)a[17], (void*)(uintptr_t)a[18], (size_t)a[19], (void*)(uintptr_t)a[20]) : MOPA_ERR_ARG;
    case 17: return nargs == 23 ? mopa_bn_bwd_sums_groups_pool((const float*)(uintptr_t)a[0], (int32_t)a[1], (const uint8_t*)(uintptr_t)a[2], (int32_t)a[3], (int32_t)a[4], (int32_t)a[5], (float*)(uintptr_t)a[6], (int32_t)a[7], (int32_t)a[8], (const float*)(uintptr_t)a[9], (int32_t)a[10], (int32_t)a[11], (int32_t)a[12], (const float*)(uintptr_t)a[13], (float)slot_f(a[14]), (int32_t)a[15], (float*)(uintptr_t)a[16], (float*)(uintptr_t)a[17], (int32_t)a[18], (float*)(uintptr_t)a[19], (void*)(uintptr_t)a[20], (size_t)a[21], (void*)(uintptr_t)a[22]) : MOPA_ERR_ARG;
    case 18: return nargs == 18 ? mopa_bn_sync_bwd_sums((const float*)(uintptr_t)a[0], (int32_t)a[1], (const float*)(uintptr_t)a[2], (int32_t)a[3], (int32_t)a[4], (int32_t)a[5], (const float*)(uintptr_t)a[6], (float)slot_f(a[7]), (int32_t)a[8], (const float*)(uintptr_t)a[9], (int32_t)a[10], (float*)(uintptr_t)a[11], (float*)(uintptr_t)a[12], (int32_t)a[13], (double*)(uintptr_t)a[14], (void*)(uintptr_t)a[15], (size_t)a[16], (void*)(uintptr_t)a[17]) : MOPA_ERR_ARG;
    case 19: return nargs == 8 ? mopa_bn_sync_moments((const float*)(uintptr_t)a[0], (int32_t)a[1], (int32_t)a[2], (int32_t)a[3], (double*)(uintptr_t)a[4], (void*)(uintptr_t)a[5], (size_t)a[6], (void*)(uintptr_t)a[7]) : MOPA_ERR_ARG;
    case 20: return nargs == 18 ? mopa_bnrelu_rows_bwd((const float*)(uintptr_t)a[0], (int32_t)a[1], (const float*)(uintptr_t)a[2], (int32_t)a[3], (float*)(uintptr_t)a[4], (int32_t)a[5], (int32_t)a[6], (int32_t)a[7], (const float*)(uintptr_t)a[8], (float)slot_f(a[9]), (int32_t)a[10], (float*)(uintptr_t)a[11], (float*)(uintptr_t)a[12], (int32_t)a[13], (int32_t)a[14], (void*)(uintptr_t)a[15], (size_t)a[16], (void*)(uintptr_t)a[17]) : MOPA_ERR_ARG;
    case 21: return nargs == 18 ? mopa_bnrelu_rows_fwd((const float*)(uintptr_t)a[0], (int32_t)a[1], (float*)(uintptr_t)a[2], (int32_t)a[3], (int32_t)a[4], (int32_t)a[5], (const float*)(uintptr_t)a[6], (const float*)(uintptr_t)a[7], (float*)(uintptr_t)a[8], (float*)(uintptr_t)a[9], (float)slot_f(a[10]), (float)slot_f(a[11]), (float)slot_f(a[12]), (int32_t)a[13], (float*)(uintptr_t)a[14], (void*)(uintptr_t)a[15], (size_t)a[16], (void*)(uintptr_t)a[17]) : MOPA_ERR_ARG;
    case 22: return nargs == 12 ? mopa_coarsen_build((const uint64_t*)(uintptr_t)a[0], (int32_t)a[1], (const int32_t*)(uintptr_t)a[2], (uint64_t*)(uintptr_t)a[3], (int32_t*)(uintptr_t)a[4], (int64_t)a[5], (int32_t*)(uintptr_t)a[6], (uint64_t*)(uintptr_t)a[7], (int32_t*)(uintptr_t)a[8], (void*)(uintptr_t)a[9], (size_t)a[10], (void*)(uintptr_t)a[11]) : MOPA_ERR_ARG;
    case 23: return nargs == 9 ? mopa_colsum((const float*)(uintptr_t)a[0], (int32_t)a[1], (int64_t)a[2], (int32_t)a[3], (float*)(uintptr_t)a[4], (int32_t)a[5], (void*)(uintptr_t)a[6], (size_t)a[7], (void*)(uintptr_t)a[8]) : MOPA_ERR_ARG;
    case 24: return nargs == 6 ? mopa_colsum_reduce((const float*)(uintptr_t)a[0], (int64_t)a[1], (int32_t)a[2], (float*)(uintptr_t)a[3], (int32_t)a[4], (void*)(uintptr_t)a[5]) : MOPA_ERR_ARG;
    case 25: return nargs == 8 ? mopa_confusion_update((const int64_t*)(uintptr_t)a[0], (const int64_t*)(uintptr_t)a[1], (int64_t)a[2], (const int32_t*)(uintptr_t)a[3], (int32_t)a[4], (int32_t)a[5], (int64_t*)(uintptr_t)a[6], (void*)(uintptr_t)a[7]) : MOPA_ERR_ARG;
    case 26: return nargs == 8 ? mopa_conv2d_bwd_weight((const float*)(uintptr_t)a[0], (const float*)(uintptr_t)a[1], (float*)(uintptr_t)a[2], (const int32_t*)(uintptr_t)a[3], (int32_t)a[4], (void*)(uintptr_t)a[5], (size_t)a[6], (void*)(uintptr_t)a[7]) : MOPA_ERR_ARG;
    case 27: return nargs == 7 ? mopa_conv2d_igemm((const float*)(uintptr_t)a[0], (const float*)(uintptr_t)a[1], (const float*)(uintptr_t)a[2], (float*)(uintptr_t)a[3], (const int32_t*)(uintptr_t)a[4], (int32_t)a[5], (void*)(uintptr_t)a[6]) : MOPA_ERR_ARG;
    case 28: return nargs == 10 ? mopa_conv2d_igemm_batched((const float*)(uintptr_t)a[0], (const float*)(uintptr_t)a[1], (float*)(uintptr_t)a[2], (const int32_t*)(uintptr_t)a[3], (int32_t)a[4], (int64_t)a[5], (int64_t)a[6], (int64_t)a[7], (int32_t)a[8], (void*)(uintptr_t)a[9]) : MOPA_ERR_ARG;
    case 29: return nargs == 7 ? mopa_conv2d_igemm_classes((const float*)(uintptr_t)a[0], (const float*)(uintptr_t)a[1], (const float*)(uintptr_t)a[2], (float*)(uintptr_t)a[3], (const int32_t*)(uintptr_t)a[4], (int32_t)a[5], (void*)(uintptr_t)a[6]) : MOPA_ERR_ARG;
    case 30: return nargs == 10 ? mopa_conv2d_relayout_weight((const float*)(uintptr_t)a[0], (float*)(uintptr_t)a[1], (int32_t)a[2], (int32_t)a[3], (int32_t)a[4], (int32_t)a[5], (int32_t)a[6], (int32_t)a[7], (int32_t)a[8], (void*)(uintptr_t)a[9]) : MOPA_ERR_ARG;
    case 31: return nargs == 6 ? mopa_conv2d_stem_relayout((const float*)(uintptr_t)a[0], (float*)(uintptr_t)a[1], (int32_t)a[2], (int32_t)a[3], (int32_t)a[4], (void*)(uintptr_t)a[5]) : MOPA_ERR_ARG;
    case 32: return nargs == 3 ? mopa_conv2d_weight_forms_batched((const int64_t*)(uintptr_t)a[0], (int32_t)a[1], (void*)(uintptr_t)a[2]) : MOPA_ERR_ARG;
    case 33: return nargs == 8 ? mopa_convt_bwd_weight((const float*)(uintptr_t)a[0], (const float*)(uintptr_t)a[1], (float*)(uintptr_t)a[2], (const int32_t*)(uintptr_t)a[3], (int32_t)a[4], (void*)(uintptr_t)a[5], (size_t)a[6], (void*)(uintptr_t)a[7]) : MOPA_ERR_ARG;
    case 34: return nargs == 7 ? mopa_copy_rows((const float*)(uintptr_t)a[0], (int32_t)a[1], (float*)(uintptr_t)a[2], (int32_t)a[3], (int64_t)a[4], (int32_t)a[5], (void*)(uintptr_t)a[6]) : MOPA_ERR_ARG;
    case 35: return nargs == 9 ? mopa_dropout_rows((const float*)(uintptr_t)a[0], (int32_t)a[1], (float*)(uintptr_t)a[2], (int32_t)a[3], (int64_t)a[4], (int32_t)a[5], (float)slot_f(a[6]), (uint64_t)a[7], (void*)(uintptr_t)a[8]) : MOPA_ERR_ARG;
    case 36: return nargs == 10 ? mopa_dropout_rows_dseed((const float*)(uintptr_t)a[0], (int32_t)a[1], (float*)(uintptr_t)a[2], (int32_t)a[3], (int64_t)a[4], (int32_t)a[5], (float)slot_f(a[6]), (const int64_t*)(uintptr_t)a[7], (int32_t)a[8], (void*)(uintptr_t)a[9]) : MOPA_ERR_ARG;
    case 37: return nargs == 5 ? mopa_ema_update((float*)(uintptr_t)a[0], (const float*)(uintptr_t)a[1], (int64_t)a[2], (float)slot_f(a[3]), (void*)(uintptr_t)a[4]) : MOPA_ERR_ARG;
    case 38: return nargs == 20 ? mopa_eval_logits((const float*)(uintptr_t)a[0], (int64_t)a[1], (const float*)(uintptr_t)a[2], (int64_t)a[3], (const int64_t*)(uintptr_t)a[4], (int32_t)a[5], (int32_t)a[6], (const int32_t*)(uintptr_t)a[7], (int32_t)a[8], (int32_t)a[9], (int64_t*)(uintptr_t)a[10], (int64_t*)(uintptr_t)a[11], (int64_t*)(uintptr_t)a[12], (int64_t*)(uintptr_t)a[13], (float*)(uintptr_t)a[14], (uint8_t*)(uintptr_t)a[15], (float*)(uintptr_t)a[16], (void*)(uintptr_t)a[17], (size_t)a[18], (void*)(uintptr_t)a[19]) : MOPA_ERR_ARG;
    case 39: return nargs == 12 ? mopa_grad_stats((const float*)(uintptr_t)a[0], (const void*)(uintptr_t)a[1], (int64_t)a[2], (int64_t)a[3], (float)slot_f(a[4]), (float)slot_f(a[5]), (int)a[6], (float*)(uintptr_t)a[7], (void*)(uintptr_t)a[8], (void*)(uintptr_t)a[9], (size_t)a[10], (void*)(uintptr_t)a[11]) : MOPA_ERR_ARG;
    case 40: return nargs == 11 ? mopa_ground_estimate((const float*)(uintptr_t)a[0], (int32_t)a[1], (const int32_t*)(uintptr_t)a[2], (int32_t)a[3], (int64_t)a[4], (int64_t)a[5], (const double*)(uintptr_t)a[6], (uint8_t*)(uintptr_t)a[7], (void*)(uintptr_t)a[8], (size_t)a[9], (void*)(uintptr_t)a[10]) : MOPA_ERR_ARG;
    case 41: return nargs == 6 ? mopa_group_split((const int32_t*)(uintptr_t)a[0], (const int32_t*)(uintptr_t)a[1], (int32_t)a[2], (int32_t)a[3], (int32_t*)(uintptr_t)a[4], (void*)(uintptr_t)a[5]) : MOPA_ERR_ARG;
    case 42: return nargs == 9 ? mopa_imageprep_contrast_sums((const void* const*)(uintptr_t)a[0], (int)a[1], (int64_t)a[2], (int)a[3], (int)a[4], (const int32_t*)(uintptr_t)a[5], (const float*)(uintptr_t)a[6], (void*)(uintptr_t)a[7], (void*)(uintptr_t)a[8]) : MOPA_ERR_ARG;
    case 43: return nargs == 10 ? mopa_imageprep_contrast_sums4((const void* const*)(uintptr_t)a[0], (int)a[1], (int64_t)a[2], (int)a[3], (int)a[4], (const int32_t*)(uintptr_t)a[5], (const float*)(uintptr_t)a[6], (const int32_t*)(uintptr_t)a[7], (void*)(uintptr_t)a[8], (void*)(uintptr_t)a[9]) : MOPA_ERR_ARG;
    case 44: return nargs == 15 ? mopa_imageprep_indices((const void* const*)(uintptr_t)a[0], (const int32_t*)(uintptr_t)a[1], (int)a[2], (int)a[3], (int)a[4], (double)slot_f(a[5]), (double)slot_f(a[6]), (const int32_t*)(uintptr_t)a[7], (int)a[8], (const int32_t*)(uintptr_t)a[9], (void* const*)(uintptr_t)a[10], (void* const*)(uintptr_t)a[11], (void* const*)(uintptr_t)a[12], (int32_t*)(uintptr_t)a[13], (void*)(uintptr_t)a[14]) : MOPA_ERR_ARG;
    case 45: return nargs == 20 ? mopa_imageprep_mask((const void* const*)(uintptr_t)a[0], (int)a[1], (int)a[2], (int)a[3], (const int32_t*)(uintptr_t)a[4], (const int32_t*)(uintptr_t)a[5], (int)a[6], (int)a[7], (int)a[8], (int)a[9], (const int32_t*)(uintptr_t)a[10], (const int32_t*)(uintptr_t)a[11], (const int32_t*)(uintptr_t)a[12], (int)a[13], (int)a[14], (const int32_t*)(uintptr_t)a[15], (int32_t*)(uintptr_t)a[16], (void*)(uintptr_t)a[17], (size_t)a[18], (void*)(uintptr_t)a[19]) : MOPA_ERR_ARG;
    case 46: return nargs == 14 ? mopa_imageprep_pixels((const void* const*)(uintptr_t)a[0], (int)a[1], (int64_t)a[2], (int)a[3], (int)a[4], (const int32_t*)(uintptr_t)a[5], (const float*)(uintptr_t)a[6], (const void*)(uintptr_t)a[7], (const int32_t*)(uintptr_t)a[8], (uint8_t*)(uintptr_t)a[9], (float*)(uintptr_t)a[10], (const float*)(uintptr_t)a[11], (float*)(uintptr_t)a[12], (void*)(uintptr_t)a[13]) : MOPA_ERR_ARG;
    case 47: return nargs == 15 ? mopa_imageprep_pixels4((const void* const*)(uintptr_t)a[0], (int)a[1], (int64_t)a[2], (int)a[3], (int)a[4], (const int32_t*)(uintptr_t)a[5], (const float*)(uintptr_t)a[6], (const int32_t*)(uintptr_t)a[7], (const void*)(uintptr_t)a[8], (const int32_t*)(uintptr_t)a[9], (uint8_t*)(uintptr_t)a[10], (float*)(uintptr_t)a[11], (const float*)(uintptr_t)a[12], (float*)(uintptr_t)a[13], (void*)(uintptr_t)a[14]) : MOPA_ERR_ARG;
    case 48: return nargs == 13 ? mopa_imageprep_resize_u8((const void* const*)(uintptr_t)a[0], (int)a[1], (int)a[2], (int)a[3], (const int32_t*)(uintptr_t)a[4], (int)a[5], (const int32_t*)(uintptr_t)a[6], (int)a[7], (int)a[8], (int)a[9], (int)a[10], (uint8_t*)(uintptr_t)a[11], (void*)(uintptr_t)a[12]) : MOPA_ERR_ARG;
    case 49: return nargs == 8 ? mopa_img_to_nhwc4((const float*)(uintptr_t)a[0], (int32_t)a[1], (int32_t)a[2], (int32_t)a[3], (int32_t)a[4], (int32_t)a[5], (float*)(uintptr_t)a[6], (void*)(uintptr_t)a[7]) : MOPA_ERR_ARG;
    case 50: return nargs == 8 ? mopa_input_layer_bwd((const float*)(uintptr_t)a[0], (int32_t)a[1], (const int32_t*)(uintptr_t)a[2], (const int32_t*)(uintptr_t)a[3], (int32_t)a[4], (int32_t)a[5], (float*)(uintptr_t)a[6], (void*)(uintptr_t)a[7]) : MOPA_ERR_ARG;
    case 51: return nargs == 8 ? mopa_input_layer_fwd((const float*)(uintptr_t)a[0], (int32_t)a[1], (const int32_t*)(uintptr_t)a[2], (const int32_t*)(uintptr_t)a[3], (int32_t)a[4], (float*)(uintptr_t)a[5], (int32_t)a[6], (void*)(uintptr_t)a[7]) : MOPA_ERR_ARG;
    case 52: return nargs == 7 ? mopa_jpeg_decode_batch((const void* const*)(uintptr_t)a[0], (const int64_t*)(uintptr_t)a[1], (const void*)(uintptr_t)a[2], (int32_t)a[3], (void* const*)(uintptr_t)a[4], (const int64_t*)(uintptr_t)a[5], (void*)(uintptr_t)a[6]) : MOPA_ERR_ARG;
    case 53: return nargs == 14 ? mopa_kittiprep_count((const void* const*)(uintptr_t)a[0], (const int32_t*)(uintptr_t)a[1], (const float*)(uintptr_t)a[2], (const void* const*)(uintptr_t)a[3], (const int32_t*)(uintptr_t)a[4], (int32_t)a[5], (int32_t)a[6], (int32_t)a[7], (uint8_t*)(uintptr_t)a[8], (const int32_t*)(uintptr_t)a[9], (int64_t*)(uintptr_t)a[10], (void*)(uintptr_t)a[11], (size_t)a[12], (void*)(uintptr_t)a[13]) : MOPA_ERR_ARG;
    case 54: return nargs == 7 ? mopa_kittiprep_ground((const void* const*)(uintptr_t)a[0], (const int32_t*)(uintptr_t)a[1], (const int32_t*)(uintptr_t)a[2], (int32_t)a[3], (uint8_t*)(uintptr_t)a[4], (int32_t*)(uintptr_t)a[5], (void*)(uintptr_t)a[6]) : MOPA_ERR_ARG;
    case 55: return nargs == 21 ? mopa_kittiprep_scatter((const void* const*)(uintptr_t)a[0], (const void* const*)(uintptr_t)a[1], (int32_t)a[2], (const int32_t*)(uintptr_t)a[3], (const float*)(uintptr_t)a[4], (int32_t)a[5], (int32_t)a[6], (int32_t)a[7], (const uint8_t*)(uintptr_t)a[8], (const uint8_t*)(uintptr_t)a[9], (float*)(uintptr_t)a[10], (float*)(uintptr_t)a[11], (int16_t*)(uintptr_t)a[12], (float*)(uintptr_t)a[13], (uint8_t*)(uintptr_t)a[14], (uint8_t*)(uintptr_t)a[15], (float*)(uintptr_t)a[16], (int16_t*)(uintptr_t)a[17], (void*)(uintptr_t)a[18], (size_t)a[19], (void*)(uintptr_t)a[20]) : MOPA_ERR_ARG;
    case 56: return nargs == 11 ? mopa_mask_cons_bwd((const float*)(uintptr_t)a[0], (const int32_t*)(uintptr_t)a[1], (int32_t)a[2], (int32_t)a[3], (int32_t)a[4], (int32_t)a[5], (int32_t)a[6], (const float*)(uintptr_t)a[7], (const float*)(uintptr_t)a[8], (float*)(uintptr_t)a[9], (void*)(uintptr_t)a[10]) : MOPA_ERR_ARG;
    case 57: return nargs == 12 ? mopa_mask_cons_fwd((const float*)(uintptr_t)a[0], (const int32_t*)(uintptr_t)a[1], (int32_t)a[2], (int32_t)a[3], (int32_t)a[4], (int32_t)a[5], (int32_t)a[6], (float*)(uintptr_t)a[7], (float*)(uintptr_t)a[8], (void*)(uintptr_t)a[9], (size_t)a[10], (void*)(uintptr_t)a[11]) : MOPA_ERR_ARG;
    case 58: return nargs == 11 ? mopa_maxpool3x3s2_bwd((const float*)(uintptr_t)a[0], (int32_t)a[1], (const uint8_t*)(uintptr_t)a[2], (int32_t)a[3], (int32_t)a[4], (int32_t)a[5], (int32_t)a[6], (float*)(uintptr_t)a[7], (int32_t)a[8], (int32_t)a[9], (void*)(uintptr_t)a[10]) : MOPA_ERR_ARG;
    case 59: return nargs == 10 ? mopa_maxpool3x3s2_fwd((const float*)(uintptr_t)a[0], (int32_t)a[1], (int32_t)a[2], (int32_t)a[3], (int32_t)a[4], (int32_t)a[5], (float*)(uintptr_t)a[6], (int32_t)a[7], (uint8_t*)(uintptr_t)a[8], (void*)(uintptr_t)a[9]) : MOPA_ERR_ARG;
    case 60: return nargs == 12 ? mopa_maxpool3x3s2_fwd_bn((const float*)(uintptr_t)a[0], (int32_t)a[1], (int32_t)a[2], (int32_t)a[3], (int32_t)a[4], (int32_t)a[5], (const float*)(uintptr_t)a[6], (int32_t)a[7], (float*)(uintptr_t)a[8], (int32_t)a[9], (uint8_t*)(uintptr_t)a[10], (void*)(uintptr_t)a[11]) : MOPA_ERR_ARG;
    case 61: return nargs == 13 ? mopa_nuscprep_count((const void* const*)(uintptr_t)a[0], (const int32_t*)(uintptr_t)a[1], (const int32_t*)(uintptr_t)a[2], (int32_t)a[3], (const double*)(uintptr_t)a[4], (int32_t)a[5], (int32_t)a[6], (uint8_t*)(uintptr_t)a[7], (const int32_t*)(uintptr_t)a[8], (int64_t*)(uintptr_t)a[9], (void*)(uintptr_t)a[10], (size_t)a[11], (void*)(uintptr_t)a[12]) : MOPA_ERR_ARG;
    case 62: return nargs == 17 ? mopa_nuscprep_scatter((const void* const*)(uintptr_t)a[0], (const int32_t*)(uintptr_t)a[1], (const int32_t*)(uintptr_t)a[2], (const int32_t*)(uintptr_t)a[3], (int32_t)a[4], (const double*)(uintptr_t)a[5], (int32_t)a[6], (int32_t)a[7], (const uint8_t*)(uintptr_t)a[8], (const uint8_t*)(uintptr_t)a[9], (float*)(uintptr_t)a[10], (float*)(uintptr_t)a[11], (uint8_t*)(uintptr_t)a[12], (uint8_t*)(uintptr_t)a[13], (void*)(uintptr_t)a[14], (size_t)a[15], (void*)(uintptr_t)a[16]) : MOPA_ERR_ARG;
    case 63: return nargs == 6 ? mopa_nuscprep_setup((const double*)(uintptr_t)a[0], (const double*)(uintptr_t)a[1], (int32_t)a[2], (int32_t)a[3], (double*)(uintptr_t)a[4], (void*)(uintptr_t)a[5]) : MOPA_ERR_ARG;
    case 64: return nargs == 21 ? mopa_objects_extract((const float*)(uintptr_t)a[0], (int32_t)a[1], (const void*)(uintptr_t)a[2], (int32_t)a[3], (const int32_t*)(uintptr_t)a[4], (int32_t)a[5], (int64_t)a[6], (int64_t)a[7], (const int32_t*)(uintptr_t)a[8], (int32_t)a[9], (const double*)(uintptr_t)a[10], (int32_t*)(uintptr_t)a[11], (int32_t*)(uintptr_t)a[12], (int32_t*)(uintptr_t)a[13], (double*)(uintptr_t)a[14], (uint8_t*)(uintptr_t)a[15], (float*)(uintptr_t)a[16], (int32_t*)(uintptr_t)a[17], (void*)(uintptr_t)a[18], (size_t)a[19], (void*)(uintptr_t)a[20]) : MOPA_ERR_ARG;
    case 65: return nargs == 22 ? mopa_output_layer_heads_bwd((const float*)(uintptr_t)a[0], (const float*)(uintptr_t)a[1], (const float*)(uintptr_t)a[2], (const float*)(uintptr_t)a[3], (const float*)(uintptr_t)a[4], (const float*)(uintptr_t)a[5], (const int32_t*)(uintptr_t)a[6], (const int32_t*)(uintptr_t)a[7], (int32_t)a[8], (int32_t)a[9], (int32_t)a[10], (int32_t)a[11], (float*)(uintptr_t)a[12], (int32_t)a[13], (float*)(uintptr_t)a[14], (float*)(uintptr_t)a[15], (float*)(uintptr_t)a[16], (float*)(uintptr_t)a[17], (int32_t)a[18], (void*)(uintptr_t)a[19], (size_t)a[20], (void*)(uintptr_t)a[21]) : MOPA_ERR_ARG;
    case 66: return nargs == 14 ? mopa_output_layer_heads_fwd((const float*)(uintptr_t)a[0], (int32_t)a[1], (const int32_t*)(uintptr_t)a[2], (int32_t)a[3], (int32_t)a[4], (int32_t)a[5], (const float*)(uintptr_t)a[6], (const float*)(uintptr_t)a[7], (const float*)(uintptr_t)a[8], (const float*)(uintptr_t)a[9], (float*)(uintptr_t)a[10], (float*)(uintptr_t)a[11], (float*)(uintptr_t)a[12], (void*)(uintptr_t)a[13]) : MOPA_ERR_ARG;
    case 67: return nargs == 8 ? mopa_pack_point_pix((const int64_t*)(uintptr_t)a[0], (const int64_t*)(uintptr_t)a[1], (int32_t)a[2], (int32_t)a[3], (int32_t)a[4], (int32_t*)(uintptr_t)a[5], (int32_t*)(uintptr_t)a[6], (void*)(uintptr_t)a[7]) : MOPA_ERR_ARG;
    case 68: return nargs == 20 ? mopa_pixel_head_bwd((const float*)(uintptr_t)a[0], (const float*)(uintptr_t)a[1], (int32_t)a[2], (int32_t)a[3], (int32_t)a[4], (int32_t)a[5], (int32_t)a[6], (int32_t)a[7], (int32_t)a[8], (int32_t)a[9], (const float*)(uintptr_t)a[10], (float*)(uintptr_t)a[11], (int32_t)a[12], (int32_t)a[13], (float*)(uintptr_t)a[14], (float*)(uintptr_t)a[15], (int32_t)a[16], (void*)(uintptr_t)a[17], (size_t)a[18], (void*)(uintptr_t)a[19]) : MOPA_ERR_ARG;
    case 69: return nargs == 13 ? mopa_pixel_head_fwd((const float*)(uintptr_t)a[0], (int32_t)a[1], (int32_t)a[2], (int32_t)a[3], (int32_t)a[4], (int32_t)a[5], (int32_t)a[6], (int32_t)a[7], (int32_t)a[8], (const float*)(uintptr_t)a[9], (const float*)(uintptr_t)a[10], (float*)(uintptr_t)a[11], (void*)(uintptr_t)a[12]) : MOPA_ERR_ARG;
    case 70: return nargs == 13 ? mopa_point_losses_bwd((const float*)(uintptr_t)a[0], (const float*)(uintptr_t)a[1], (const float*)(uintptr_t)a[2], (const int64_t*)(uintptr_t)a[3], (const float*)(uintptr_t)a[4], (int32_t)a[5], (int32_t)a[6], (int64_t)a[7], (const float*)(uintptr_t)a[8], (const float*)(uintptr_t)a[9], (float*)(uintptr_t)a[10], (float*)(uintptr_t)a[11], (void*)(uintptr_t)a[12]) : MOPA_ERR_ARG;
    case 71: return nargs == 19 ? mopa_point_losses_fwd((const float*)(uintptr_t)a[0], (const float*)(uintptr_t)a[1], (const float*)(uintptr_t)a[2], (const float*)(uintptr_t)a[3], (const int64_t*)(uintptr_t)a[4], (const int64_t*)(uintptr_t)a[5], (const float*)(uintptr_t)a[6], (int32_t)a[7], (int32_t)a[8], (int64_t)a[9], (float*)(uintptr_t)a[10], (int64_t*)(uintptr_t)a[11], (int64_t*)(uintptr_t)a[12], (const uint8_t*)(uintptr_t)a[13], (int64_t*)(uintptr_t)a[14], (int32_t*)(uintptr_t)a[15], (void*)(uintptr_t)a[16], (size_t)a[17], (void*)(uintptr_t)a[18]) : MOPA_ERR_ARG;
    case 72: return nargs == 16 ? mopa_point_losses_seg_bwd((int32_t)a[0], (const float*)(uintptr_t)a[1], (const float*)(uintptr_t)a[2], (const float*)(uintptr_t)a[3], (const float*)(uintptr_t)a[4], (const int64_t*)(uintptr_t)a[5], (int32_t)a[6], (int64_t)a[7], (int64_t)a[8], (int32_t)a[9], (int64_t)a[10], (const float*)(uintptr_t)a[11], (const float*)(uintptr_t)a[12], (float*)(uintptr_t)a[13], (float*)(uintptr_t)a[14], (void*)(uintptr_t)a[15]) : MOPA_ERR_ARG;
    case 73: return nargs == 16 ? mopa_point_losses_seg_fwd((const float*)(uintptr_t)a[0], (const float*)(uintptr_t)a[1], (const float*)(uintptr_t)a[2], (const float*)(uintptr_t)a[3], (const float*)(uintptr_t)a[4], (const int64_t*)(uintptr_t)a[5], (int32_t)a[6], (int64_t)a[7], (int64_t)a[8], (int32_t)a[9], (int64_t)a[10], (float*)(uintptr_t)a[11], (int32_t*)(uintptr_t)a[12], (void*)(uintptr_t)a[13], (size_t)a[14], (void*)(uintptr_t)a[15]) : MOPA_ERR_ARG;
    case 74: return nargs == 8 ? mopa_points_csr((const int32_t*)(uintptr_t)a[0], (int32_t)a[1], (int32_t)a[2], (int32_t*)(uintptr_t)a[3], (int32_t*)(uintptr_t)a[4], (void*)(uintptr_t)a[5], (size_t)a[6], (void*)(uintptr_t)a[7]) : MOPA_ERR_ARG;
    case 75: return nargs == 7 ? mopa_pseudo_fuse((const float*)(uintptr_t)a[0], (const float*)(uintptr_t)a[1], (int32_t)a[2], (int32_t)a[3], (float*)(uintptr_t)a[4], (int64_t*)(uintptr_t)a[5], (void*)(uintptr_t)a[6]) : MOPA_ERR_ARG;
    case 76: return nargs == 9 ? mopa_refine_pseudo_labels((const float*)(uintptr_t)a[0], (const int64_t*)(uintptr_t)a[1], (int32_t)a[2], (int32_t)a[3], (int64_t)a[4], (int64_t*)(uintptr_t)a[5], (void*)(uintptr_t)a[6], (size_t)a[7], (void*)(uintptr_t)a[8]) : MOPA_ERR_ARG;
    case 77: return nargs == 11 ? mopa_refine_pseudo_labels_segmented((const void* const*)(uintptr_t)a[0], (const void* const*)(uintptr_t)a[1], (int32_t)a[2], (const int32_t*)(uintptr_t)a[3], (void* const*)(uintptr_t)a[4], (int32_t)a[5], (int32_t)a[6], (int64_t)a[7], (void*)(uintptr_t)a[8], (size_t)a[9], (void*)(uintptr_t)a[10]) : MOPA_ERR_ARG;
    case 78: return nargs == 5 ? mopa_rotate_points_f32((const float*)(uintptr_t)a[0], (int32_t)a[1], (const float*)(uintptr_t)a[2], (float*)(uintptr_t)a[3], (void*)(uintptr_t)a[4]) : MOPA_ERR_ARG;
    case 79: return nargs == 9 ? mopa_rows_add((const float*)(uintptr_t)a[0], (int32_t)a[1], (const float*)(uintptr_t)a[2], (int32_t)a[3], (float*)(uintptr_t)a[4], (int32_t)a[5], (int32_t)a[6], (int32_t)a[7], (void*)(uintptr_t)a[8]) : MOPA_ERR_ARG;
    case 80: return nargs == 5 ? mopa_rulebook_groups_count((const int32_t*)(uintptr_t)a[0], (int32_t)a[1], (int32_t)a[2], (int32_t*)(uintptr_t)a[3], (void*)(uintptr_t)a[4]) : MOPA_ERR_ARG;
    case 81: return nargs == 5 ? mopa_rulebook_groups_count_batched((const int64_t*)(uintptr_t)a[0], (int32_t)a[1], (int32_t)a[2], (int32_t*)(uintptr_t)a[3], (void*)(uintptr_t)a[4]) : MOPA_ERR_ARG;
    case 82: return nargs == 8 ? mopa_rulebook_groups_fill((const int32_t*)(uintptr_t)a[0], (int32_t)a[1], (int32_t)a[2], (const int32_t*)(uintptr_t)a[3], (int32_t*)(uintptr_t)a[4], (int32_t*)(uintptr_t)a[5], (int32_t*)(uintptr_t)a[6], (void*)(uintptr_t)a[7]) : MOPA_ERR_ARG;
    case 83: return nargs == 8 ? mopa_rulebook_groups_fill_batched((const int64_t*)(uintptr_t)a[0], (int32_t)a[1], (int32_t)a[2], (const int32_t*)(uintptr_t)a[3], (int32_t*)(uintptr_t)a[4], (int32_t*)(uintptr_t)a[5], (int32_t*)(uintptr_t)a[6], (void*)(uintptr_t)a[7]) : MOPA_ERR_ARG;
    case 84: return nargs == 3 ? mopa_rulebook_runs_build_batched((const int64_t*)(uintptr_t)a[0], (int32_t)a[1], (void*)(uintptr_t)a[2]) : MOPA_ERR_ARG;
    case 85: return nargs == 8 ? mopa_rulebook_subm((const uint64_t*)(uintptr_t)a[0], (int32_t)a[1], (const uint64_t*)(uintptr_t)a[2], (const int32_t*)(uintptr_t)a[3], (int64_t)a[4], (int32_t)a[5], (int32_t*)(uintptr_t)a[6], (void*)(uintptr_t)a[7]) : MOPA_ERR_ARG;
    case 86: return nargs == 7 ? mopa_rulebook_updown((const uint64_t*)(uintptr_t)a[0], (const int32_t*)(uintptr_t)a[1], (int32_t)a[2], (int32_t)a[3], (int32_t*)(uintptr_t)a[4], (int32_t*)(uintptr_t)a[5], (void*)(uintptr_t)a[6]) : MOPA_ERR_ARG;
    case 87: return nargs == 7 ? mopa_scan_exclusive_i32((const int32_t*)(uintptr_t)a[0], (int32_t*)(uintptr_t)a[1], (int32_t)a[2], (int32_t*)(uintptr_t)a[3], (void*)(uintptr_t)a[4], (size_t)a[5], (void*)(uintptr_t)a[6]) : MOPA_ERR_ARG;
    case 88: return nargs == 22 ? mopa_scanprep_compact((const void* const*)(uintptr_t)a[0], (const void* const*)(uintptr_t)a[1], (const int32_t*)(uintptr_t)a[2], (const double*)(uintptr_t)a[3], (const int32_t*)(uintptr_t)a[4], (int32_t)a[5], (int32_t)a[6], (int32_t)a[7], (float)slot_f(a[8]), (int32_t)a[9], (int32_t)a[10], (const uint8_t*)(uintptr_t)a[11], (int64_t*)(uintptr_t)a[12], (int64_t*)(uintptr_t)a[13], (int64_t*)(uintptr_t)a[14], (int64_t)a[15], (uint8_t*)(uintptr_t)a[16], (int64_t*)(uintptr_t)a[17], (int32_t*)(uintptr_t)a[18], (void*)(uintptr_t)a[19], (size_t)a[20], (void*)(uintptr_t)a[21]) : MOPA_ERR_ARG;
    case 89: return nargs == 15 ? mopa_scanprep_count((const void* const*)(uintptr_t)a[0], (const void* const*)(uintptr_t)a[1], (const int32_t*)(uintptr_t)a[2], (const double*)(uintptr_t)a[3], (const int32_t*)(uintptr_t)a[4], (int32_t)a[5], (int32_t)a[6], (float)slot_f(a[7]), (int32_t)a[8], (int32_t)a[9], (uint8_t*)(uintptr_t)a[10], (int64_t*)(uintptr_t)a[11], (void*)(uintptr_t)a[12], (size_t)a[13], (void*)(uintptr_t)a[14]) : MOPA_ERR_ARG;
    case 90: return nargs == 6 ? mopa_scanprep_rotate((const void* const*)(uintptr_t)a[0], (void* const*)(uintptr_t)a[1], (const int32_t*)(uintptr_t)a[2], (const float*)(uintptr_t)a[3], (int32_t)a[4], (void*)(uintptr_t)a[5]) : MOPA_ERR_ARG;
    case 91: return nargs == 20 ? mopa_scanprep_take((const int64_t*)(uintptr_t)a[0], (int64_t)a[1], (int64_t)a[2], (const int32_t*)(uintptr_t)a[3], (int32_t)a[4], (const void* const*)(uintptr_t)a[5], (int32_t)a[6], (const int64_t*)(uintptr_t)a[7], (int64_t)a[8], (int64_t)a[9], (const void* const*)(uintptr_t)a[10], (const void* const*)(uintptr_t)a[11], (const int64_t*)(uintptr_t)a[12], (const int64_t*)(uintptr_t)a[13], (int64_t*)(uintptr_t)a[14], (int64_t*)(uintptr_t)a[15], (float*)(uintptr_t)a[16], (int64_t*)(uintptr_t)a[17], (int64_t*)(uintptr_t)a[18], (void*)(uintptr_t)a[19]) : MOPA_ERR_ARG;
    case 92: return nargs == 14 ? mopa_scn_backward((const int32_t*)(uintptr_t)a[0], (int32_t)a[1], (const int32_t*)(uintptr_t)a[2], (int32_t)a[3], (const int64_t*)(uintptr_t)a[4], (int64_t*)(uintptr_t)a[5], (const int64_t*)(uintptr_t)a[6], (const int64_t*)(uintptr_t)a[7], (const int64_t*)(uintptr_t)a[8], (const int64_t*)(uintptr_t)a[9], (const int64_t*)(uintptr_t)a[10], (void*)(uintptr_t)a[11], (size_t)a[12], (void*)(uintptr_t)a[13]) : MOPA_ERR_ARG;
    case 93: return nargs == 10 ? mopa_scn_forward((const int32_t*)(uintptr_t)a[0], (int32_t)a[1], (const int64_t*)(uintptr_t)a[2], (int64_t*)(uintptr_t)a[3], (const int64_t*)(uintptr_t)a[4], (const int64_t*)(uintptr_t)a[5], (const int64_t*)(uintptr_t)a[6], (void*)(uintptr_t)a[7], (size_t)a[8], (void*)(uintptr_t)a[9]) : MOPA_ERR_ARG;
    case 94: return nargs == 12 ? mopa_sgd_flat((float*)(uintptr_t)a[0], (const float*)(uintptr_t)a[1], (float*)(uintptr_t)a[2], (int64_t)a[3], (float)slot_f(a[4]), (float)slot_f(a[5]), (float)slot_f(a[6]), (float)slot_f(a[7]), (int)a[8], (int)a[9], (float)slot_f(a[10]), (void*)(uintptr_t)a[11]) : MOPA_ERR_ARG;
    case 95: return nargs == 13 ? mopa_sgd_flat_guarded((float*)(uintptr_t)a[0], (const float*)(uintptr_t)a[1], (float*)(uintptr_t)a[2], (int64_t)a[3], (float)slot_f(a[4]), (float)slot_f(a[5]), (float)slot_f(a[6]), (float)slot_f(a[7]), (int)a[8], (int*)(uintptr_t)a[9], (float)slot_f(a[10]), (const void*)(uintptr_t)a[11], (void*)(uintptr_t)a[12]) : MOPA_ERR_ARG;
    case 96: return nargs == 6 ? mopa_softmax_bwd((const float*)(uintptr_t)a[0], (const float*)(uintptr_t)a[1], (int64_t)a[2], (int32_t)a[3], (float*)(uintptr_t)a[4], (void*)(uintptr_t)a[5]) : MOPA_ERR_ARG;
    case 97: return nargs == 5 ? mopa_softmax_fwd((const float*)(uintptr_t)a[0], (int64_t)a[1], (int32_t)a[2], (float*)(uintptr_t)a[3], (void*)(uintptr_t)a[4]) : MOPA_ERR_ARG;
    case 98: return nargs == 7 ? mopa_softmax_kl_bwd((const float*)(uintptr_t)a[0], (const float*)(uintptr_t)a[1], (int32_t)a[2], (int32_t)a[3], (const float*)(uintptr_t)a[4], (float*)(uintptr_t)a[5], (void*)(uintptr_t)a[6]) : MOPA_ERR_ARG;
    case 99: return nargs == 8 ? mopa_softmax_kl_fwd((const float*)(uintptr_t)a[0], (const float*)(uintptr_t)a[1], (int32_t)a[2], (int32_t)a[3], (float*)(uintptr_t)a[4], (void*)(uintptr_t)a[5], (size_t)a[6], (void*)(uintptr_t)a[7]) : MOPA_ERR_ARG;
    case 100: return nargs == 14 ? mopa_spconv_bwd_weight((const int32_t*)(uintptr_t)a[0], (int32_t)a[1], (int32_t)a[2], (const float*)(uintptr_t)a[3], (int32_t)a[4], (int32_t)a[5], (const float*)(uintptr_t)a[6], (int32_t)a[7], (int32_t)a[8], (float*)(uintptr_t)a[9], (int32_t)a[10], (void*)(uintptr_t)a[11], (size_t)a[12], (void*)(uintptr_t)a[13]) : MOPA_ERR_ARG;
    case 101: return nargs == 16 ? mopa_spconv_bwd_weight_run((const int32_t*)(uintptr_t)a[0], (int32_t)a[1], (int32_t)a[2], (int32_t)a[3], (int32_t)a[4], (const float*)(uintptr_t)a[5], (int32_t)a[6], (int32_t)a[7], (const float*)(uintptr_t)a[8], (int32_t)a[9], (int32_t)a[10], (float*)(uintptr_t)a[11], (int32_t)a[12], (void*)(uintptr_t)a[13], (size_t)a[14], (void*)(uintptr_t)a[15]) : MOPA_ERR_ARG;
    case 102: return nargs == 12 ? mopa_spconv_fwd((const int32_t*)(uintptr_t)a[0], (int32_t)a[1], (int32_t)a[2], (const float*)(uintptr_t)a[3], (int32_t)a[4], (int32_t)a[5], (const float*)(uintptr_t)a[6], (int32_t)a[7], (int32_t)a[8], (float*)(uintptr_t)a[9], (int32_t)a[10], (void*)(uintptr_t)a[11]) : MOPA_ERR_ARG;
    case 103: return nargs == 17 ? mopa_spconv_fwd_grouped((const int32_t*)(uintptr_t)a[0], (const int32_t*)(uintptr_t)a[1], (const int32_t*)(uintptr_t)a[2], (const int32_t*)(uintptr_t)a[3], (int32_t)a[4], (int32_t)a[5], (const float*)(uintptr_t)a[6], (int32_t)a[7], (int32_t)a[8], (const float*)(uintptr_t)a[9], (int32_t)a[10], (int32_t)a[11], (float*)(uintptr_t)a[12], (int32_t)a[13], (void*)(uintptr_t)a[14], (size_t)a[15], (void*)(uintptr_t)a[16]) : MOPA_ERR_ARG;
    case 104: return nargs == 15 ? mopa_spconv_fwd_run((const int32_t*)(uintptr_t)a[0], (int32_t)a[1], (int32_t)a[2], (const float*)(uintptr_t)a[3], (int32_t)a[4], (int32_t)a[5], (const float*)(uintptr_t)a[6], (int32_t)a[7], (int32_t)a[8], (float*)(uintptr_t)a[9], (int32_t)a[10], (int32_t)a[11], (void*)(uintptr_t)a[12], (size_t)a[13], (void*)(uintptr_t)a[14]) : MOPA_ERR_ARG;
    case 105: return nargs == 8 ? mopa_spconv_pack_weight((const float*)(uintptr_t)a[0], (int32_t)a[1], (int32_t)a[2], (int32_t)a[3], (int32_t)a[4], (int32_t)a[5], (float*)(uintptr_t)a[6], (void*)(uintptr_t)a[7]) : MOPA_ERR_ARG;
    case 106: return nargs == 3 ? mopa_spconv_pack_weights_batched((const int64_t*)(uintptr_t)a[0], (int32_t)a[1], (void*)(uintptr_t)a[2]) : MOPA_ERR_ARG;
    case 107: return nargs == 7 ? mopa_spconv_run_pack_weight((const float*)(uintptr_t)a[0], (int32_t)a[1], (int32_t)a[2], (int32_t)a[3], (int32_t)a[4], (float*)(uintptr_t)a[5], (void*)(uintptr_t)a[6]) : MOPA_ERR_ARG;
    case 108: return nargs == 6 ? mopa_spconv_transpose_weight((const float*)(uintptr_t)a[0], (int32_t)a[1], (int32_t)a[2], (int32_t)a[3], (float*)(uintptr_t)a[4], (void*)(uintptr_t)a[5]) : MOPA_ERR_ARG;
    case 109: return nargs == 8 ? mopa_stem_bwd_weight2((const float*)(uintptr_t)a[0], (const float*)(uintptr_t)a[1], (float*)(uintptr_t)a[2], (const int32_t*)(uintptr_t)a[3], (int32_t)a[4], (void*)(uintptr_t)a[5], (size_t)a[6], (void*)(uintptr_t)a[7]) : MOPA_ERR_ARG;
    case 110: return nargs == 15 ? mopa_stem_bwd_weight_bn((const float*)(uintptr_t)a[0], (const float*)(uintptr_t)a[1], (int32_t)a[2], (const float*)(uintptr_t)a[3], (int32_t)a[4], (const float*)(uintptr_t)a[5], (const float*)(uintptr_t)a[6], (int32_t)a[7], (int32_t)a[8], (float*)(uintptr_t)a[9], (const int32_t*)(uintptr_t)a[10], (int32_t)a[11], (void*)(uintptr_t)a[12], (size_t)a[13], (void*)(uintptr_t)a[14]) : MOPA_ERR_ARG;
    case 111: return nargs == 15 ? mopa_stem_bwd_weight_bn2((const float*)(uintptr_t)a[0], (const float*)(uintptr_t)a[1], (int32_t)a[2], (const float*)(uintptr_t)a[3], (int32_t)a[4], (const float*)(uintptr_t)a[5], (const float*)(uintptr_t)a[6], (int32_t)a[7], (int32_t)a[8], (float*)(uintptr_t)a[9], (const int32_t*)(uintptr_t)a[10], (int32_t)a[11], (void*)(uintptr_t)a[12], (size_t)a[13], (void*)(uintptr_t)a[14]) : MOPA_ERR_ARG;
    case 112: return nargs == 10 ? mopa_stem_dgrad_image((const float*)(uintptr_t)a[0], (int32_t)a[1], (int32_t)a[2], (int32_t)a[3], (int32_t)a[4], (int32_t)a[5], (int32_t)a[6], (const float*)(uintptr_t)a[7], (float*)(uintptr_t)a[8], (void*)(uintptr_t)a[9]) : MOPA_ERR_ARG;
    case 113: return nargs == 13 ? mopa_vgi_box_free((const int32_t*)(uintptr_t)a[0], (int32_t)a[1], (int32_t)a[2], (int32_t)a[3], (int32_t)a[4], (int32_t)a[5], (int32_t)a[6], (int32_t)a[7], (int32_t)a[8], (uint8_t*)(uintptr_t)a[9], (void*)(uintptr_t)a[10], (size_t)a[11], (void*)(uintptr_t)a[12]) : MOPA_ERR_ARG;
    case 114: return nargs == 13 ? mopa_vgi_candidates((const uint8_t*)(uintptr_t)a[0], (int32_t)a[1], (int32_t)a[2], (int32_t)a[3], (const double*)(uintptr_t)a[4], (const uint8_t*)(uintptr_t)a[5], (int32_t)a[6], (int32_t)a[7], (int32_t)a[8], (int32_t)a[9], (uint8_t*)(uintptr_t)a[10], (int32_t*)(uintptr_t)a[11], (void*)(uintptr_t)a[12]) : MOPA_ERR_ARG;
    case 115: return nargs == 8 ? mopa_vgi_compact_cells((const uint8_t*)(uintptr_t)a[0], (int32_t)a[1], (int32_t)a[2], (int32_t)a[3], (int32_t)a[4], (int32_t*)(uintptr_t)a[5], (int32_t*)(uintptr_t)a[6], (void*)(uintptr_t)a[7]) : MOPA_ERR_ARG;
    case 116: return nargs == 13 ? mopa_vgi_first_points((const float*)(uintptr_t)a[0], (int32_t)a[1], (int32_t)a[2], (float)slot_f(a[3]), (int32_t)a[4], (int32_t)a[5], (int32_t)a[6], (int32_t)a[7], (int32_t)a[8], (const uint8_t*)(uintptr_t)a[9], (int32_t*)(uintptr_t)a[10], (int32_t*)(uintptr_t)a[11], (void*)(uintptr_t)a[12]) : MOPA_ERR_ARG;
    case 117: return nargs == 15 ? mopa_vgi_first_points_rep((const float*)(uintptr_t)a[0], (int32_t)a[1], (int32_t)a[2], (float)slot_f(a[3]), (double)slot_f(a[4]), (int32_t)a[5], (int32_t)a[6], (int32_t)a[7], (int32_t)a[8], (int32_t)a[9], (int32_t*)(uintptr_t)a[10], (int32_t*)(uintptr_t)a[11], (void*)(uintptr_t)a[12], (size_t)a[13], (void*)(uintptr_t)a[14]) : MOPA_ERR_ARG;
    case 118: return nargs == 6 ? mopa_vgi_ground_cells((const int32_t*)(uintptr_t)a[0], (const uint8_t*)(uintptr_t)a[1], (int32_t)a[2], (int32_t)a[3], (uint8_t*)(uintptr_t)a[4], (void*)(uintptr_t)a[5]) : MOPA_ERR_ARG;
    case 119: return nargs == 11 ? mopa_vgi_range_keep((const double*)(uintptr_t)a[0], (int32_t)a[1], (int32_t)a[2], (double)slot_f(a[3]), (double)slot_f(a[4]), (int32_t)a[5], (int32_t)a[6], (uint8_t*)(uintptr_t)a[7], (void*)(uintptr_t)a[8], (size_t)a[9], (void*)(uintptr_t)a[10]) : MOPA_ERR_ARG;
    case 120: return nargs == 15 ? mopa_vgi_road_height((const float*)(uintptr_t)a[0], (int32_t)a[1], (int32_t)a[2], (float)slot_f(a[3]), (const int32_t*)(uintptr_t)a[4], (const uint8_t*)(uintptr_t)a[5], (int32_t)a[6], (int32_t)a[7], (int32_t)a[8], (int32_t)a[9], (int32_t)a[10], (int32_t)a[11], (int32_t)a[12], (double*)(uintptr_t)a[13], (void*)(uintptr_t)a[14]) : MOPA_ERR_ARG;
    case 121: return nargs == 12 ? mopa_voxel_hash_build((const int64_t*)(uintptr_t)a[0], (int64_t)a[1], (uint64_t*)(uintptr_t)a[2], (int32_t*)(uintptr_t)a[3], (int64_t)a[4], (int32_t*)(uintptr_t)a[5], (uint64_t*)(uintptr_t)a[6], (int32_t*)(uintptr_t)a[7], (int32_t*)(uintptr_t)a[8], (void*)(uintptr_t)a[9], (size_t)a[10], (void*)(uintptr_t)a[11]) : MOPA_ERR_ARG;
    case 122: return nargs == 12 ? mopa_voxelize((const float*)(uintptr_t)a[0], (int32_t)a[1], (float)slot_f(a[2]), (int32_t)a[3], (const double*)(uintptr_t)a[4], (int32_t)a[5], (int64_t)a[6], (int64_t*)(uintptr_t)a[7], (uint8_t*)(uintptr_t)a[8], (void*)(uintptr_t)a[9], (size_t)a[10], (void*)(uintptr_t)a[11]) : MOPA_ERR_ARG;
    case 123: return nargs == 14 ? mopa_voxelize_f64((const double*)(uintptr_t)a[0], (int32_t)a[1], (const uint8_t*)(uintptr_t)a[2], (const double*)(uintptr_t)a[3], (double)slot_f(a[4]), (int32_t)a[5], (const double*)(uintptr_t)a[6], (int32_t)a[7], (int64_t)a[8], (int64_t*)(uintptr_t)a[9], (uint8_t*)(uintptr_t)a[10], (void*)(uintptr_t)a[11], (size_t)a[12], (void*)(uintptr_t)a[13]) : MOPA_ERR_ARG;
    case 124: return nargs == 10 ? mopa_wce_bwd((const float*)(uintptr_t)a[0], (const int64_t*)(uintptr_t)a[1], (const float*)(uintptr_t)a[2], (int32_t)a[3], (int32_t)a[4], (int64_t)a[5], (const float*)(uintptr_t)a[6], (const float*)(uintptr_t)a[7], (float*)(uintptr_t)a[8], (void*)(uintptr_t)a[9]) : MOPA_ERR_ARG;
    case 125: return nargs == 12 ? mopa_wce_fwd((const float*)(uintptr_t)a[0], (const int64_t*)(uintptr_t)a[1], (const float*)(uintptr_t)a[2], (int32_t)a[3], (int32_t)a[4], (int64_t)a[5], (float*)(uintptr_t)a[6], (float*)(uintptr_t)a[7], (int32_t*)(uintptr_t)a[8], (void*)(uintptr_t)a[9], (size_t)a[10], (void*)(uintptr_t)a[11]) : MOPA_ERR_ARG;
    case 126: return nargs == 10 ? mopa_wino4_bwd_weight((const float*)(uintptr_t)a[0], (const float*)(uintptr_t)a[1], (int32_t)a[2], (int32_t)a[3], (int32_t)a[4], (float*)(uintptr_t)a[5], (int32_t)a[6], (void*)(uintptr_t)a[7], (size_t)a[8], (void*)(uintptr_t)a[9]) : MOPA_ERR_ARG;
    case 127: return nargs == 17 ? mopa_wino4_conv((const float*)(uintptr_t)a[0], (int32_t)a[1], (const float*)(uintptr_t)a[2], (const float*)(uintptr_t)a[3], (float*)(uintptr_t)a[4], (int32_t)a[5], (int32_t)a[6], (int32_t)a[7], (int32_t)a[8], (int32_t)a[9], (int32_t)a[10], (int32_t)a[11], (const float*)(uintptr_t)a[12], (int32_t)a[13], (int32_t)a[14], (float*)(uintptr_t)a[15], (void*)(uintptr_t)a[16]) : MOPA_ERR_ARG;
    case 128: return nargs == 16 ? mopa_wino4_conv9((const float*)(uintptr_t)a[0], (int32_t)a[1], (const float*)(uintptr_t)a[2], (const float*)(uintptr_t)a[3], (float*)(uintptr_t)a[4], (int32_t)a[5], (int32_t)a[6], (int32_t)a[7], (int32_t)a[8], (int32_t)a[9], (int32_t)a[10], (int32_t)a[11], (const float*)(uintptr_t)a[12], (int32_t)a[13], (int32_t)a[14], (void*)(uintptr_t)a[15]) : MOPA_ERR_ARG;
    case 129: return nargs == 8 ? mopa_wino4_dout((const float*)(uintptr_t)a[0], (int32_t)a[1], (int32_t)a[2], (int32_t)a[3], (int32_t)a[4], (int32_t)a[5], (float*)(uintptr_t)a[6], (void*)(uintptr_t)a[7]) : MOPA_ERR_ARG;
    case 130: return nargs == 12 ? mopa_wino4_gemm_output((const float*)(uintptr_t)a[0], (const float*)(uintptr_t)a[1], (const float*)(uintptr_t)a[2], (float*)(uintptr_t)a[3], (int32_t)a[4], (int32_t)a[5], (int32_t)a[6], (int32_t)a[7], (int32_t)a[8], (int32_t)a[9], (int32_t)a[10], (void*)(uintptr_t)a[11]) : MOPA_ERR_ARG;
    case 131: return nargs == 8 ? mopa_wino4_input((const float*)(uintptr_t)a[0], (int32_t)a[1], (int32_t)a[2], (int32_t)a[3], (int32_t)a[4], (int32_t)a[5], (float*)(uintptr_t)a[6], (void*)(uintptr_t)a[7]) : MOPA_ERR_ARG;
    case 132: return nargs == 11 ? mopa_wino4_input_bn((const float*)(uintptr_t)a[0], (int32_t)a[1], (int32_t)a[2], (int32_t)a[3], (int32_t)a[4], (int32_t)a[5], (const float*)(uintptr_t)a[6], (int32_t)a[7], (int32_t)a[8], (float*)(uintptr_t)a[9], (void*)(uintptr_t)a[10]) : MOPA_ERR_ARG;
    case 133: return nargs == 10 ? mopa_wino4_output((const float*)(uintptr_t)a[0], (int32_t)a[1], (int32_t)a[2], (int32_t)a[3], (int32_t)a[4], (const float*)(uintptr_t)a[5], (float*)(uintptr_t)a[6], (int32_t)a[7], (int32_t)a[8], (void*)(uintptr_t)a[9]) : MOPA_ERR_ARG;
    case 134: return nargs == 6 ? mopa_wino4_weight((const float*)(uintptr_t)a[0], (int32_t)a[1], (int32_t)a[2], (int32_t)a[3], (float*)(uintptr_t)a[4], (void*)(uintptr_t)a[5]) : MOPA_ERR_ARG;
    case 135: return nargs == 6 ? mopa_wino4_weight_f((const float*)(uintptr_t)a[0], (int32_t)a[1], (int32_t)a[2], (int32_t)a[3], (float*)(uintptr_t)a[4], (void*)(uintptr_t)a[5]) : MOPA_ERR_ARG;
    case 136: return nargs == 6 ? mopa_wino4_weight_q((const float*)(uintptr_t)a[0], (int32_t)a[1], (int32_t)a[2], (int32_t)a[3], (float*)(uintptr_t)a[4], (void*)(uintptr_t)a[5]) : MOPA_ERR_ARG;
    case 137: return nargs == 6 ? mopa_wino4_weight_t((const float*)(uintptr_t)a[0], (int32_t)a[1], (int32_t)a[2], (int32_t)a[3], (float*)(uintptr_t)a[4], (void*)(uintptr_t)a[5]) : MOPA_ERR_ARG;
    case 138: return nargs == 17 ? mopa_wino4_wgrad_fused((const float*)(uintptr_t)a[0], (int32_t)a[1], (const float*)(uintptr_t)a[2], (int32_t)a[3], (int32_t)a[4], (const float*)(uintptr_t)a[5], (int32_t)a[6], (int32_t)a[7], (int32_t)a[8], (int32_t)a[9], (int32_t)a[10], (int32_t)a[11], (float*)(uintptr_t)a[12], (int32_t)a[13], (void*)(uintptr_t)a[14], (size_t)a[15], (void*)(uintptr_t)a[16]) : MOPA_ERR_ARG;
    case 139: return nargs == 10 ? mopa_wino_bwd_weight((const float*)(uintptr_t)a[0], (const float*)(uintptr_t)a[1], (int32_t)a[2], (int32_t)a[3], (int32_t)a[4], (float*)(uintptr_t)a[5], (int32_t)a[6], (void*)(uintptr_t)a[7], (size_t)a[8], (void*)(uintptr_t)a[9]) : MOPA_ERR_ARG;
    case 140: return nargs == 8 ? mopa_wino_dout((const float*)(uintptr_t)a[0], (int32_t)a[1], (int32_t)a[2], (int32_t)a[3], (int32_t)a[4], (int32_t)a[5], (float*)(uintptr_t)a[6], (void*)(uintptr_t)a[7]) : MOPA_ERR_ARG;
    case 141: return nargs == 8 ? mopa_wino_input((const float*)(uintptr_t)a[0], (int32_t)a[1], (int32_t)a[2], (int32_t)a[3], (int32_t)a[4], (int32_t)a[5], (float*)(uintptr_t)a[6], (void*)(uintptr_t)a[7]) : MOPA_ERR_ARG;
    case 142: return nargs == 10 ? mopa_wino_output((const float*)(uintptr_t)a[0], (int32_t)a[1], (int32_t)a[2], (int32_t)a[3], (int32_t)a[4], (const float*)(uintptr_t)a[5], (float*)(uintptr_t)a[6], (int32_t)a[7], (int32_t)a[8], (void*)(uintptr_t)a[9]) : MOPA_ERR_ARG;
    case 143: return nargs == 6 ? mopa_wino_weight((const float*)(uintptr_t)a[0], (int32_t)a[1], (int32_t)a[2], (int32_t)a[3], (float*)(uintptr_t)a[4], (void*)(uintptr_t)a[5]) : MOPA_ERR_ARG;
    case 144: return nargs == 5 ? mopa_zero_rows((float*)(uintptr_t)a[0], (int32_t)a[1], (int64_t)a[2], (int32_t)a[3], (void*)(uintptr_t)a[4]) : MOPA_ERR_ARG;
    default: return MOPA_ERR_ARG;
  }
}
```

### mopa_amd/dense2d.py

```python
from __future__ import annotations

import ctypes
import os
from typing import NamedTuple

import numpy as np
import torch

from . import _lib, syncbn
from ._lib import GradSink, call, host_i32, ptr, query, stream, workspace
from .sparse3d import View

BN_EPS = 1e-5
BN_MOMENTUM = 0.1
DEBUG = None
LAYERS = [("layer1", 64, 3, 1), ("layer2", 128, 4, 2), ("layer3", 256, 6, 2), ("layer4", 512, 3, 2)]


class Img(View):

    __slots__ = ("B", "H", "W", "partial", "pool")

    def __init__(self, t, B, H, W, col=0, C=None):
        super().__init__(t, col, C)
# ... 444 lines not shown
        geoms = []
        for ph in range(2):
            for pw in range(2):
                khs = [kh for kh in range(k) if (ph + p - kh) % 2 == 0]
                kws = [kw for kw in range(k) if (pw + p - kw) % 2 == 0]
                ohl, owl = (x.H - ph + 1) // 2, (x.W - pw + 1) // 2
                if not khs or not kws or ohl <= 0 or owl <= 0:
                    continue
                geoms.append(_geom(B=x.B, IH=dout.H, IW=dout.W, OHl=ohl, OWl=owl, OHa=x.H, OWa=x.W, OS=2, OOY=ph, OOX=pw,
                                   IY0=(ph + p - khs[0]) // 2, IX0=(pw + p - kws[0]) // 2, IDY=-1, IDX=-1, TH=len(khs),
                                   TW=len(kws), KH0=khs[0], KW0=kws[0], KS=2, KWF=k, Cin=self.O, Cout=self.I, ld_in=dout.ld,
                                   ld_out=dx.ld))
        return geoms

    def dgrad_s2(self, x: Img, dout: Img, dx: Img, wt, acc_dx: bool):
        geoms = self.dgrad_s2_geoms(x, dout, dx)
        if len(geoms) == 4 and conv_classes(dout, dx):
            igemm_classes(dout.p, wt, None, dx.p, geoms, acc_dx)
            return
        if not acc_dx:
            call("mopa_zero_rows", dx.p, dx.ld, dx.rows, dx.C, stream())
        for g in geoms:
            igemm(dout.p, wt, None, dx.p, g, True)


class ConvTOp:

    def __init__(self, weight, bias):
        self.w, self.b = weight, bias
        self.I, self.O = weight.shape[0], weight.shape[1]

    def _geom(self, x: Img, out: Img, ky, kx):
        return _geom(B=x.B, IH=x.H, IW=x.W, OHl=x.H, OWl=x.W, OHa=out.H, OWa=out.W, OS=2, OOY=ky, OOX=kx, TH=1, TW=1,
                     KH0=ky, KW0=kx, KWF=2, Cin=self.I, Cout=self.O, ld_in=x.ld, ld_out=out.ld)

    def forward(self, x: Img, out: Img):
        wl = relayout_cached(self.w, (2, 2, self.I, self.O), self.O, self.I, 2, 2, 2)
        geoms = [self._geom(x, out, ky, kx) for ky in range(2) for kx in range(2)]
        if conv_classes(x, out):
            igemm_classes(x.p, wl, self.b, out.p, geoms)
            return
        for g in geoms:
            igemm(x.p, wl, self.b, out.p, g)

    def wgrad(self, x: Img, dout: Img, dw, acc_params: bool = False):
        dev = self.w.device
        if conv_classes(x, dout) and self.I % 64 == 0 and dout.H >= 2 * x.H and dout.W >= 2 * x.W:
            convt_wgrad(x.p, dout.p, dw, self._geom(x, dout, 0, 0), dev, accumulate=acc_params)
            return
        dwl = torch.empty(2, 2, self.I, self.O, dtype=torch.float32, device=dev)
        for ky in range(2):
            for kx in range(2):
                g = self._geom(x, dout, ky, kx)
                g[17], g[18] = 0, 0
                wgrad(x.p, dout.p, ptr(dwl, (ky * 2 + kx) * self.I * self.O), g, dev)
        relayout(dwl, dw, self.O, self.I, 2, 2, 2, inverse=True, accumulate=acc_params)

    def backward(self, x: Img, dout: Img, dx: Img, dw, db, acc_params: bool = False, wgrad_side: bool = False, db_partial=None):
        dev = self.w.device
        with _on(wgrad_stream(dev) if wgrad_side else None, dout.t, db_partial):
            self.wgrad(x, dout, dw, acc_params)
            colsum(dout, db, accumulate=acc_params, partial=db_partial)
        wt = relayout_cached(self.w, (2, 2, self.O, self.I), self.O, self.I, 2, 2, 3)
        g = _geom(B=x.B, IH=dout.H, IW=dout.W, OHl=x.H, OWl=x.W, OHa=x.H, OWa=x.W, IS=2, TH=2, TW=2, KWF=2,
                  Cin=self.O, Cout=self.I, ld_in=dout.ld, ld_out=dx.ld)
        igemm(dout.p, wt, None, dx.p, g, False)


def colsum(x: View, out: torch.Tensor, accumulate=False, partial=None):
    if partial is not None:
        call("mopa_colsum_reduce", ptr(partial), x.rows, x.C, ptr(out), int(accumulate), stream())
        return
    wsb = query("mopa_colsum_workspace_bytes", x.rows, x.C)
    ws = workspace.get(wsb, out.device)
    call("mopa_colsum", x.p, x.ld, x.rows, x.C, ptr(out), int(accumulate), ptr(ws), ws.numel(), stream())


DEFER_BN = os.environ.get("MOPA_DEFER_BN", "1") != "0"
DEFER_UP_BN = os.environ.get("MOPA_DEFER_UP_BN", "1") != "0"
DEFER_STEM_BN = os.environ.get("MOPA_DEFER_STEM_BN", "1") != "0"
STEM_BN_FUSED_BWD = os.environ.get("MOPA_STEM_BN_FUSED_BWD", "1") != "0" and os.environ.get("MOPA_CONV2D_MFMA", "1") != "0"
STEM_BWD2 = frozenset({"1": ("wgrad", "pool"), "0": ()}.get(os.environ.get("MOPA_STEM_BWD2", "1"), (os.environ.get("MOPA_STEM_BWD2"),)))
STEM_BWD2_MIN_PIXELS = int(os.environ.get("MOPA_STEM_BWD2_MIN_PIXELS", str(1 << 17)))
BN_MASK_BITS = os.environ.get("MOPA_BN_MASK_BITS", "1") != "0"
BN_COLSUM_FUSED = os.environ.get("MOPA_BN_COLSUM_FUSED", "1") != "0"


BN_KEYS = (".weight", ".bias", ".running_mean", ".running_var")


def _pl(v):
    return (v.p, v.ld) if v is not None else (None, 0)


def _bn_tail(query_name, x):
    ws = workspace.get(query(query_name, x.rows, x.C), x.t.device)
    return ptr(ws), ws.numel(), stream()


def bn_fwd(x: View, y: View, P, name, act, res, training, stats):
    if training and syncbn.active():
        return syncbn.fwd(x, y, *(P[name + k] for k in BN_KEYS), BN_MOMENTUM, BN_EPS, 0.0, act, res, stats)
    call("mopa_bn_act_fwd", x.p, x.ld, y.p, y.ld, x.rows, x.C, *(ptr(P[name + k]) for k in BN_KEYS), BN_MOMENTUM, BN_EPS, 0.0, int(act),
         *_pl(res), int(training), ptr(stats), *_bn_tail("mopa_bnrelu_rows_workspace_bytes", x))


def bn_fwd_groups(x: View, y: View | None, P, name, act, res, training, stats, G, bits=None):
    n = x.rows // G
    call("mopa_bn_act_fwd_groups" + ("_bits" if bits is not None else ""), x.p, x.ld, *_pl(y), x.rows, x.C, G, n, 2 * n,
         *(ptr(P[name + k]) for k in BN_KEYS), BN_MOMENTUM, BN_EPS, 0.0, int(act), *_pl(res), int(training), ptr(stats),
         *((1, ptr(bits)) if bits is not None else ()), *_bn_tail("mopa_bnrelu_rows_workspace_bytes", x))


def bn_bwd_groups(dy: View, x: View, dx: View, stats, act, ymask, dres, acc_dres, training, dgamma, dbeta, G, acc_params=False):
    n = x.rows // G
    call("mopa_bn_act_bwd_groups", dy.p, dy.ld, x.p, x.ld, dx.p, dx.ld, x.rows, x.C, G, n, 2 * n, ptr(stats), 0.0, int(act), *_pl(ymask),
         *_pl(dres), int(acc_dres), int(training), ptr(dgamma), ptr(dbeta), int(acc_params), 0,
         *_bn_tail("mopa_bnrelu_rows_bwd_workspace_bytes", x))


def bn_bwd_fused(dy: View, x: View, dx: View, stats, act, bits, dres, acc_dres, training, dgamma, dbeta, G, acc_params=False,
                 want_colsum=False):
    n = x.rows // G
    partial = torch.empty(query("mopa_colsum_partial_blocks", x.rows) * x.C, dtype=torch.float32, device=x.t.device) if want_colsum else None
    call("mopa_bn_act_bwd_groups_fused", dy.p, dy.ld, x.p, x.ld, dx.p, dx.ld, x.rows, x.C, G, n, 2 * n, ptr(stats), 0.0, int(act),
         int(bits is not None), ptr(bits), *_pl(dres), int(acc_dres), int(training), ptr(dgamma), ptr(dbeta), int(acc_params), 0,
         ptr(partial), *_bn_tail("mopa_bn_act_bwd_groups_fused_workspace_bytes", x))
    return partial


def bn_bwd(dy: View, x: View, dx: View, stats, act, ymask, dres, acc_dres, training, dgamma, dbeta, acc_dx=False,
           acc_params=False, gathered=None):
    if gathered is not None:
        return syncbn.bwd(dy, x, dx, stats, 0.0, act, ymask, dres, acc_dres, dgamma, dbeta, acc_params, acc_dx, gathered)
    call("mopa_bn_act_bwd", dy.p, dy.ld, x.p, x.ld, dx.p, dx.ld, x.rows, x.C, ptr(stats), 0.0, int(act), *_pl(ymask), *_pl(dres),
         int(acc_dres), int(training), ptr(dgamma), ptr(dbeta), int(acc_params), int(acc_dx), *_bn_tail("mopa_bnrelu_rows_bwd_workspace_bytes", x))


def bn_bwd_sums(dy: View, x: Img, stats, act, dgamma, dbeta, G, acc_params=False, pool=None):
    n, coef = x.rows // G, torch.empty(G, 2, x.C, dtype=torch.float32, device=x.t.device)
    head = (dy.p, dy.ld, x.p, x.ld, x.rows, x.C, G, n, 2 * n) if pool is None else \
        (pool[0].p, pool[0].ld, ptr(pool[1]), x.B, x.H, x.W, dy.p, dy.ld, int(pool[2]), x.p, x.ld, x.C, G)
    call("mopa_bn_bwd_sums_groups" + ("" if pool is None else "_pool"), *head, ptr(stats), 0.0, int(act), *((None, 0) if pool is None else ()),
         ptr(dgamma), ptr(dbeta), int(acc_params), ptr(coef), *_bn_tail("mopa_bnrelu_rows_workspace_bytes", x))
    return coef


class BnPlan(NamedTuple):
    fwd: str
    bwd: str
    bits: bool
    colsum: bool
    pool_inside: bool
    stem_wgrad: str


def bn_plan(C, G, training, keep_tape, act, res, deferred, sync, biased=False, stem=False, pool_reader=False, grid=(0, 0, 0),
            want_dimg=False, bits=None) -> BnPlan:
    synced = bool(training and sync and not deferred)
    second = lambda part: part in STEM_BWD2 and STEM_BN_FUSED_BWD and grid[0] * grid[1] * grid[2] >= STEM_BWD2_MIN_PIXELS
    if bits is None:
        bits = bool(BN_MASK_BITS and not deferred and keep_tape and training and res and act == 1 and C % 32 == 0 and not sync)
    fwd = ("stats" if deferred else "groups_bits" if bits else "groups" if G > 1 and not (training and sync) else "sync" if synced else "single")
    sums = bool(STEM_BN_FUSED_BWD and stem and C == 64 and not want_dimg and not res and act == 1 and not synced)
    pool_inside = bool(sums and pool_reader and deferred and second("pool"))
    fusable = not synced and (not res or bits)
# ... 40 lines not shown
        assert (pool is not None) == plan.pool_inside
        if plan.stem_wgrad != "plain":
            return StemGrad(dy, x, stats, bn_bwd_sums(dy, x, stats, act, dgamma, dbeta, G, acc_params, pool))
        dx = new_img(x.B, x.H, x.W, x.C, x.t.device)
        ymask = self.y if self.res is not None else None
        if plan.bwd == "fused":
            dx.partial = bn_bwd_fused(dy, x, dx, stats, act, self.bits, dres, acc_dres, training, dgamma, dbeta, G, acc_params, plan.colsum)
        elif plan.bwd == "groups":
            bn_bwd_groups(dy, x, dx, stats, act, ymask, dres, acc_dres, training, dgamma, dbeta, G, acc_params)
        else:
            for g in range(G):
                bn_bwd(_group(dy, g, G), _group(x, g, G), _group(dx, g, G), stats[g], act, _group(ymask, g, G), _group(dres, g, G), acc_dres,
                       training, dgamma, dbeta, acc_params=acc_params or g > 0, gathered=None if self.gathered is None else self.gathered[g])
        return dx


def _group(v: Img, g, G):
    if G == 1 or v is None:
        return v
    n = v.rows // G
    return Img(v.t[g * n:(g + 1) * n], v.B // G, v.H, v.W, v.col, v.C)


class _NoTape:

    def append(self, rec):
        pass


def _backbone_forward(P, imgc, training, drop_p, drop_seed, seed_t, dev, groups=1, keep_tape=True):
    pre = "net_2d."
    B, _, H, W = imgc.shape
    G = groups
    seeds = tuple(drop_seed) if isinstance(drop_seed, (tuple, list)) else (drop_seed,) * G
    Hp, Wp = (H + 15) // 16 * 16, (W + 15) // 16 * 16
    tape = [] if keep_tape else _NoTape()
    nbt = []

    def bn(name, x, act=1, res=None, out=None, defer=False, **layer):
        op = layer["op"] if "op" in layer else BnOp(P, name, act, res, G, **layer)
        if training:
            nbt.append(P[name + ".num_batches_tracked"])
        tape.append(("bn", op))
        return op.forward(x, out, training, keep_tape, defer)

    def takes_lazy(name, B, H, W):
        cout, cin = P[name + ".weight"].shape[:2]
        return conv_plan(cin, cout, 3, 1, 1, B, H, W, training).takes_lazy

    def conv(name, x, k, s, p, bias=False, out=None):
        op = ConvOp(P[name + ".weight"], P[name + ".bias"] if bias else None, k, s, p)
        oh, ow = op.out_hw(x.H, x.W)
        out = out if out is not None else new_img(x.B, oh, ow, op.O, dev)
        V = op.forward(x, out, keep_v=training)
        tape.append(("conv", name, op, x, out, V))
        return out

    def convT(name, x, out=None):
        op = ConvTOp(P[name + ".weight"], P[name + ".bias"])
        out = out if out is not None else new_img(x.B, 2 * x.H, 2 * x.W, op.O, dev)
        op.forward(x, out)
        tape.append(("convT", name, op, x, out))
        return out

    def dropout(x, site, out=None):
        y = out if out is not None else new_img(x.B, x.H, x.W, x.C, dev)
        p = drop_p if training else 0.0
        for g in range(G):
            dropout_rows(_group(x, g, G), _group(y, g, G), p, seeds[g], None if seed_t is None else seed_t[g:], site)
        tape.append(("dropout", site, x, y, p))
        return y

    x4 = torch.empty(B, Hp + 6, Wp + 8, 4, dtype=torch.float32, device=dev)
    call("mopa_img_to_nhwc4", ptr(imgc), B, H, W, Hp, Wp, ptr(x4), stream())
    w1 = torch.empty(7, 2, 16, 64, dtype=torch.float32, device=dev)
    call("mopa_conv2d_stem_relayout", ptr(P[pre + "conv1.weight"]), ptr(w1), 64, 0, 0, stream())
    J = {}
    J[0] = torch.empty(B * Hp * Wp, 128, dtype=torch.float32, device=dev)
    lazy_stem = (DEFER_BN and DEFER_UP_BN and DEFER_STEM_BN and not (training and syncbn.active())
                 and takes_lazy(pre + "dec_conv_stage1", B, Hp, Wp))
    c1 = Img(J[0], B, Hp, Wp, 0, 64) if lazy_stem else new_img(B, Hp, Wp, 64, dev)
    stem_g = _geom(B=B, IH=Hp + 6, IW=Wp + 8, OHl=Hp, OWl=Wp, OHa=Hp, OWa=Wp, IDX=4, TH=7, TW=2, KWF=2, Cin=16,
                   Cout=64, ld_in=4, ld_out=c1.ld)
    igemm(ptr(x4), w1, None, c1.p, stem_g)
    bn1 = BnOp(P, pre + "bn1", G=G, stem_grid=(B, Hp, Wp))
    tape.append(("stem", x4, c1, stem_g, bn1))
    H2, W2 = Hp // 2, Wp // 2
    x = new_img(B, H2, W2, 64, dev)
    amax = torch.empty(B * H2 * W2 * 64, dtype=torch.uint8, device=dev)
    skip0 = bn(pre + "bn1", c1, out=None if lazy_stem else Img(J[0], B, Hp, Wp, 0, 64), defer=lazy_stem, op=bn1)
    if lazy_stem:
        call("mopa_maxpool3x3s2_fwd_bn", c1.p, c1.ld, B, Hp, Wp, 64, ptr(skip0.bn[0]), G, x.p, x.ld, ptr(amax), stream())
    else:
        call("mopa_maxpool3x3s2_fwd", skip0.p, skip0.ld, B, Hp, Wp, 64, x.p, x.ld, ptr(amax), stream())
    tape.append(("maxpool", skip0, x, amax, bn1))
    for li, (lname, c, nblocks, stride) in enumerate(LAYERS):
        for b in range(nblocks):
            q = f"{pre}{lname}.{b}."
            s = stride if b == 0 else 1
            has_ds = (q + "downsample.0.weight") in P
            z1 = conv(q + "conv1", x, 3, s, 1)
            defer = (DEFER_BN and not (training and syncbn.active())
                     and takes_lazy(q + "conv2", z1.B, z1.H, z1.W))
            y1 = bn(q + "bn1", z1, defer=defer)
            z = conv(q + "conv2", y1, 3, 1, 1)
            idt = bn(q + "downsample.1", conv(q + "downsample.0", x, 1, s, 0), act=0) if has_ds else x
            last = b == nblocks - 1
            out = None
            if last and lname in ("layer1", "layer2"):
                lvl = li + 1
                J[lvl] = torch.empty(z.rows, 2 * c, dtype=torch.float32, device=dev)
                out = Img(J[lvl], z.B, z.H, z.W, 0, c)
            x = bn(q + "bn2", z, act=1, res=idt, out=out)
        if lname == "layer3":
            J[3] = torch.empty(x.rows, 2 * c, dtype=torch.float32, device=dev)
            x = dropout(x, 0, out=Img(J[3], x.B, x.H, x.W, 0, c))
        if lname == "layer4":
            x = dropout(x, 1)
    for stage, lvl in (("5", 3), ("4", 2), ("3", 1), ("2", 0)):
        tname = f"{pre}dec_t_conv_stage{stage}."
        cj = J[lvl].shape[1] // 2
        cname = pre + "dec_conv_stage1" if lvl == 0 else f"{pre}dec_conv_stage{int(stage) - 1}.0"
        lazy_up = (DEFER_BN and DEFER_UP_BN and not (training and syncbn.active())
                   and takes_lazy(cname, x.B, 2 * x.H, 2 * x.W))
        if lazy_up:
            right = Img(J[lvl], x.B, 2 * x.H, 2 * x.W, cj, cj)
            up_raw = convT(tname + "0", x, out=right)
            ylazy = bn(tname + "1", up_raw, defer=True, biased=True)
            if lvl == 0 and lazy_stem:
                st2 = torch.empty(G, 4, 2 * cj, dtype=torch.float32, device=dev)
                for half, src in enumerate((skip0.bn[0], ylazy.bn[0])):
                    call("mopa_copy_rows", ptr(src), cj, ptr(st2, half * cj), 2 * cj, G * 4, cj, stream())
                joined = LazyImg(Img(J[lvl], up_raw.B, up_raw.H, up_raw.W, 0, 2 * cj), st2, G)
            else:
                joined = LazyImg(Img(J[lvl], up_raw.B, up_raw.H, up_raw.W, 0, 2 * cj), ylazy.bn[0], G, c0=cj)
        else:
            up_raw = convT(tname + "0", x)
            bn(tname + "1", up_raw, out=Img(J[lvl], up_raw.B, up_raw.H, up_raw.W, cj, cj), biased=True)
            joined = Img(J[lvl], up_raw.B, up_raw.H, up_raw.W, 0, 2 * cj)
        tape.append(("join", lvl, cj, lazy_up, lvl == 0 and lazy_stem))
        if lvl == 0:
            x = conv(pre + "dec_conv_stage1", joined, 3, 1, 1, bias=True)
        else:
            x = bn(cname[:-1] + "1", conv(cname, joined, 3, 1, 1, bias=True), biased=True)
    for i in range(0, len(nbt), 64):
        tab = np.zeros(64, np.int64)
        tab[:len(nbt[i:i + 64])] = [t.data_ptr() for t in nbt[i:i + 64]]
        call("mopa_add_i64_many", tab.ctypes.data, len(nbt[i:i + 64]), G, stream())
    return x, tape, J


def dropout_rows(x: View, y: View, p, seed, seed_t, site):
    if seed_t is not None:
        call("mopa_dropout_rows_dseed", x.p, x.ld, y.p, y.ld, x.rows, x.C, float(p), ptr(seed_t), site, stream())
    else:
        call("mopa_dropout_rows", x.p, x.ld, y.p, y.ld, x.rows, x.C, float(p), seed * 2 + site, stream())


def _backbone_backward(P, sink, tape, J, feat, dfeat, training, drop_seed, seed_t, want_dimg, H, W, groups=1):
    dev = feat.t.device
    G = groups
    seeds = tuple(drop_seed) if isinstance(drop_seed, (tuple, list)) else (drop_seed,) * G
    pre = "net_2d."
    B, Hp, Wp = feat.B, feat.H, feat.W
    gmap = {}
    dimg = None

# ... 365 lines not shown
```

Baseline: 417.9.

## Add packed-tap strip kernel for 7x7 stem forward and packed wgrad

Adds a dedicated stem forward kernel that packs the 147 real taps of the 7x7x3 stem into 74 MFMA k-pairs. It stages a strip of input rows in LDS and reuses an LDS-resident weight tile, replacing the generic implicit-GEMM, which pads the taps to 7x32. The stem wgrad strip kernel gets a packed variant that computes only the real taps, using 3 accumulator tiles instead of 4, and zero-fills the padding rows. The aim is to cut wasted MFMA work on padded channels, at the cost of irregular LDS addressing and more kernel variants.

```diff
diff --git a/include/mopa_hip.h b/include/mopa_hip.h
--- a/include/mopa_hip.h
+++ b/include/mopa_hip.h
@@ -98,6 +98,7 @@
 int mopa_stem_bwd_weight_bn(const float* in, const float* dy, int32_t ld_dy, const float* xbn, int32_t ld_x, const float* stats, const float* coef, int32_t n_groups, int32_t training, float* dweight, const int32_t* geom_host, int32_t flags, void* ws, size_t ws_bytes, void* stream);
 int mopa_stem_bwd_weight2(const float* in, const float* dy, float* dweight, const int32_t* geom_host, int32_t flags, void* ws, size_t ws_bytes, void* stream);
 int mopa_stem_bwd_weight_bn2(const float* in, const float* dy, int32_t ld_dy, const float* xbn, int32_t ld_x, const float* stats, const float* coef, int32_t n_groups, int32_t training, float* dweight, const int32_t* geom_host, int32_t flags, void* ws, size_t ws_bytes, void* stream);
+int mopa_stem_fwd(const float* in, const float* weight, float* out, const int32_t* geom_host, void* stream);
 size_t mopa_wino_wgrad_workspace_bytes(int32_t T, int32_t Cin, int32_t Cout);
 int mopa_wino_bwd_weight(const float* V, const float* dM, int32_t T, int32_t Cin, int32_t Cout, float* dweight, int32_t flags, void* ws, size_t ws_bytes, void* stream);
 size_t mopa_wino4_wgrad_workspace_bytes(int32_t T, int32_t Cin, int32_t Cout);
diff --git a/mopa_amd/_abi.py b/mopa_amd/_abi.py
--- a/mopa_amd/_abi.py
+++ b/mopa_amd/_abi.py
@@ -84,6 +84,7 @@
     'mopa_stem_bwd_weight_bn': ('i', 'ppipippiippipzp'),
     'mopa_stem_bwd_weight2': ('i', 'ppppipzp'),
     'mopa_stem_bwd_weight_bn2': ('i', 'ppipippiippipzp'),
+    'mopa_stem_fwd': ('i', 'ppppp'),
     'mopa_wino_wgrad_workspace_bytes': ('z', 'iii'),
     'mopa_wino_bwd_weight': ('i', 'ppiiipipzp'),
     'mopa_wino4_wgrad_workspace_bytes': ('z', 'iii'),
@@ -282,6 +283,7 @@
     'mopa_stem_bwd_weight2': {3: 'geom_host'},
     'mopa_stem_bwd_weight_bn': {10: 'geom_host'},
     'mopa_stem_bwd_weight_bn2': {10: 'geom_host'},
+    'mopa_stem_fwd': {3: 'geom_host'},
     'mopa_vgi_candidates': {4: 'params_host'},
     'mopa_voxelize': {4: 'u_host'},
     'mopa_voxelize_f64': {3: 'rot_host', 6: 'u_host'},
diff --git a/mopa_amd/csrc/conv2d.hip b/mopa_amd/csrc/conv2d.hip
--- a/mopa_amd/csrc/conv2d.hip
+++ b/mopa_amd/csrc/conv2d.hip
@@ -1098,18 +1098,18 @@
 #define SP 64
 #define SSLOTS 512
 static_assert(7 * (SP + 7) <= SSLOTS && SP % 16 == 0, "strip staging: two float4 per thread");
-template <int NT>
-__device__ __forceinline__ void stem_strip_mma(f32x16 (&acc)[4], const float* sp, const float* bp, int np) {
-  constexpr int SW = 4 * (SP + 7);
+#define STEM_TAPS 147
+template <int NT, int NA>
+__device__ __forceinline__ void stem_strip_mma(f32x16 (&acc)[NA], const float* sp, const int (&so)[NA], const float* bp, int np) {
   float b0 = bp[0], a0[NT];
 #pragma unroll
-  for (int n = 0; n < NT; ++n) a0[n] = sp[n * 2 * SW];
+  for (int n = 0; n < NT; ++n) a0[n] = sp[so[n]];
 #define STEM_STRIP_PAIR(I)                                                                                          \
   {                                                                                                                 \
     const int nx = min((I) + 1, np - 1);                                                                            \
     const float b1 = bp[nx * 128];                                                                                  \
     float a1[NT];                                                                                                   \
-    _Pragma("unroll") for (int n = 0; n < NT; ++n) a1[n] = sp[n * 2 * SW + nx * 8];                                 \
+    _Pragma("unroll") for (int n = 0; n < NT; ++n) a1[n] = sp[so[n] + nx * 8];                                      \
     _Pragma("unroll") for (int n = 0; n < NT; ++n) acc[n] = __builtin_amdgcn_mfma_f32_32x32x2f32(a0[n], b0, acc[n], 0, 0, 0); \
     b0 = b1;                                                                                                        \
     _Pragma("unroll") for (int n = 0; n < NT; ++n) a0[n] = a1[n];                                                   \
@@ -1122,7 +1122,7 @@
   for (; i < np; ++i) STEM_STRIP_PAIR(i)
 #undef STEM_STRIP_PAIR
 }
-template <bool BNB>
+template <bool BNB, bool PACKED>
 __global__ __launch_bounds__(256, 2) void k_stem_wgrad_strip(const float* __restrict__ in, const float* __restrict__ dy,
                                                               float* __restrict__ slabs, const ConvGeom g, int m_per_split,
                                                               const StemBn bn) {
@@ -1141,14 +1141,20 @@
   const int M = g.B * g.OHl * g.OWl, ohw = g.OHl * g.OWl;
   const int mbeg = blockIdx.x * m_per_split, mend = min(M, mbeg + m_per_split);
   const int lane = t & 63, wv = __builtin_amdgcn_readfirstlane(t >> 6);
-  const int wco = (wv & 1) * 32, rt0 = wv >> 1;
+  constexpr int NA = PACKED ? 3 : 4;
+  const int wp = wv >> 1;
+  const int wco = (wv & 1) * 32;
   const int l32 = lane & 31, lk = lane >> 5;
   const int ld_dy = BNB ? bn.ld_dy : g.ld_out;
-  f32x16 acc[4];
-#pragma unroll
-  for (int n = 0; n < 4; ++n)
+  f32x16 acc[NA];
+  int so[NA];
+#pragma unroll
+  for (int n = 0; n < NA; ++n) {
 #pragma unroll
     for (int e = 0; e < 16; ++e) acc[n][e] = 0.f;
+    const int k = (wp * 3 + n) * 32 + l32;
+    so[n] = !PACKED ? (wp + 2 * n) * SW + l32 : k < STEM_TAPS ? (k / 21) * SW + 4 * ((k % 21) / 3) + k % 3 : 0;
+  }
   int scol[2], soff[2];
 #pragma unroll
   for (int j = 0; j < 2; ++j) {
@@ -1225,11 +1231,11 @@
   while (len > 0) {
     const bool more = cm < mend;
     if (more) load_chunk();
-    const float* sp = &Ss[buf][rt0 * SW + 4 * lk + l32];
+    const float* sp = &Ss[buf][4 * lk];
     const float* bp = &Bs[buf][lk][wco + l32];
     const int np = (len + 1) >> 1;
-    if (rt0 == 0) stem_strip_mma<4>(acc, sp, bp, np);
-    else stem_strip_mma<3>(acc, sp, bp, np);
+    if (wp == 0) stem_strip_mma<NA, NA>(acc, sp, so, bp, np);
+    else stem_strip_mma<NA - 1, NA>(acc, sp, so, bp, np);
     if (more) {
       store_chunk(buf ^ 1);
       __syncthreads();
@@ -1239,13 +1245,24 @@
       len = 0;
     }
   }
-  float* dst = slabs + (int64_t)blockIdx.x * STEM_ROWS * 64 + wco + l32;
-#pragma unroll
-  for (int n = 0; n < 4; ++n) {
-    const int rt = rt0 + 2 * n;
-    if (rt < 7) {
-#pragma unroll
-      for (int e = 0; e < 16; ++e) dst[(int64_t)(rt * 32 + 8 * (e >> 2) + 4 * lk + (e & 3)) * 64] = acc[n][e];
+  float* slab = slabs + (int64_t)blockIdx.x * STEM_ROWS * 64;
+  float* dst = slab + wco + l32;
+#pragma unroll
+  for (int n = 0; n < NA; ++n) {
+    const int rt = PACKED ? wp * 3 + n : wp + 2 * n;
+    if (rt < (PACKED ? 5 : 7)) {
+#pragma unroll
+      for (int e = 0; e < 16; ++e) {
+        const int k = rt * 32 + 8 * (e >> 2) + 4 * lk + (e & 3);
+        if (!PACKED) dst[k * 64] = acc[n][e];
+        else if (k < STEM_TAPS) dst[((k / 21) * 32 + 4 * ((k % 21) / 3) + k % 3) * 64] = acc[n][e];
+      }
+    }
+  }
+  if (PACKED) {
+    for (int i = t; i < (STEM_ROWS - STEM_TAPS) * 64; i += 256) {
+      const int p = i >> 6, q = p % 11;
+      slab[((p / 11) * 32 + (q < 7 ? 4 * q + 3 : q + 21)) * 64 + (i & 63)] = 0.f;
     }
   }
 }
@@ -1292,8 +1309,10 @@
   wgrad_split(g, &ns, &mps);
   hipStream_t st = (hipStream_t)stream;
   float* slabs = (float*)ws;
-  if (bn) k_stem_wgrad_strip<true><<<ns, 256, 0, st>>>(in, dy, slabs, g, mps, *bn);
-  else k_stem_wgrad_strip<false><<<ns, 256, 0, st>>>(in, dy, slabs, g, mps, StemBn{});
+  if (bn && param) k_stem_wgrad_strip<true, true><<<ns, 256, 0, st>>>(in, dy, slabs, g, mps, *bn);
+  else if (bn) k_stem_wgrad_strip<true, false><<<ns, 256, 0, st>>>(in, dy, slabs, g, mps, *bn);
+  else if (param) k_stem_wgrad_strip<false, true><<<ns, 256, 0, st>>>(in, dy, slabs, g, mps, StemBn{});
+  else k_stem_wgrad_strip<false, false><<<ns, 256, 0, st>>>(in, dy, slabs, g, mps, StemBn{});
   const int n = STEM_ROWS * 64;
   if (param) k_reduce_slabs_stem<<<n / 16, 256, 0, st>>>(slabs, ns, dweight, accumulate);
   else reduce_slabs2_launch(slabs, ns, n, dweight, accumulate, 0, 14, 16, 64, st);
@@ -1313,6 +1332,146 @@
     return MOPA_ERR_ARG;
   const StemBn bn{xbn, stats, coef, ld_x, ld_dy, g.B / n_groups, n_groups, training};
   return stem_wgrad2_launch(in, dy, dweight, geom_host, flags, ws, ws_bytes, stream, &bn);
+}
+
+#define FSP 128
+#define FCW (FSP + 7)
+#define FKP 74
+static_assert(2 * FKP > STEM_TAPS && 2 * FKP - STEM_TAPS == 1, "one zero row");
+__host__ __device__ constexpr int stem_fwd_off(int k) { return ((k / 21) * 3 + k % 3) * FCW + (k % 21) / 3; }
+__global__ __launch_bounds__(256, 2) void k_stem_fwd_strip(const float* __restrict__ in, const float* __restrict__ w,
+                                                            float* __restrict__ out, const ConvGeom g, int chunks_per_block, int nchunks) {
+  constexpr int NS = (7 * FCW + 255) / 256;
+  __shared__ __attribute__((aligned(16))) float Wf[2 * FKP][64];
+  __shared__ float Fs[2][21 * FCW];
+  const int t = threadIdx.x;
+  for (int i = t; i < 2 * FKP * 16; i += 256) {
+    const int k = i >> 4, q = i & 15;
+    float4 v = make_float4(0.f, 0.f, 0.f, 0.f);
+    if (k < STEM_TAPS) v = *reinterpret_cast<const float4*>(w + ((k / 21) * 32 + 4 * ((k % 21) / 3) + k % 3) * 64 + q * 4);
+    *reinterpret_cast<float4*>(&Wf[k][q * 4]) = v;
+  }
+  const int lane = t & 63, wv = __builtin_amdgcn_readfirstlane(t >> 6);
+  const int l32 = lane & 31, lk = lane >> 5;
+  int scol[NS], soff[NS], sdst[NS];
+#pragma unroll
+  for (int j = 0; j < NS; ++j) {
+    const int e = t + 256 * j, r = e / FCW, col = e - r * FCW;
+    scol[j] = e < 7 * FCW ? col : 2 * FSP;
+    soff[j] = (r * g.IW + col) * 4;
+    sdst[j] = r * 3 * FCW + col;
+  }
+  float4 rs[NS];
+  const int cpr = (g.OWl + FSP - 1) / FSP;
+  int cc = blockIdx.x * chunks_per_block;
+  const int cend = min(nchunks, cc + chunks_per_block);
+  int crow = __builtin_amdgcn_readfirstlane(cc / cpr), cxc = cc - crow * cpr;
+  int cb = __builtin_amdgcn_readfirstlane(crow / g.OHl), cy = crow - cb * g.OHl;
+  int llen = 0;
+  int64_t lout = 0;
+  auto load_chunk = [&]() {
+    const int cx = cxc * FSP;
+    const int len = min(FSP, g.OWl - cx);
+    const float* sbase = in + ((int64_t)(cb * g.IH + cy) * g.IW + cx) * 4;
+#pragma unroll
+    for (int j = 0; j < NS; ++j) rs[j] = *reinterpret_cast<const float4*>(sbase + (scol[j] < len + 7 ? soff[j] : 0));
+    llen = len;
+    lout = ((int64_t)(cb * g.OHa + cy) * g.OWa + cx) * g.ld_out;
+    ++cc;
+    if (++cxc == cpr) {
+      cxc = 0;
+      if (++cy == g.OHl) { cy = 0; ++cb; }
+    }
+  };
+  auto store_chunk = [&](int buf) {
+#pragma unroll
+    for (int j = 0; j < NS; ++j) {
+      if (scol[j] < FCW) {
+        float* d = &Fs[buf][sdst[j]];
+        d[0] = rs[j].x;
+        d[FCW] = rs[j].y;
+        d[2 * FCW] = rs[j].z;
+      }
+    }
+  };
+  int buf = 0, len = 0;
+  int64_t obase = 0;
+  if (cc < cend) {
+    load_chunk();
+    store_chunk(0);
+    len = llen;
+    obase = lout;
+  }
+  __syncthreads();
+  const int p0 = wv * 32;
+  const int d1 = lk * FCW, d2 = lk * (1 - 2 * FCW), d3 = lk * (FCW - 6);
+  while (len > 0) {
+    const bool more = cc < cend;
+    if (more) load_chunk();
+    if (p0 < len) {
+      f32x16 acc[2];
+#pragma unroll
+      for (int n = 0; n < 2; ++n)
+#pragma unroll
+        for (int e = 0; e < 16; ++e) acc[n][e] = 0.f;
+      const float* sp = &Fs[buf][p0 + l32];
+      const float* sp1 = sp + d1;
+      const float* sp2 = sp + d2;
+      const float* sp3 = sp + d3;
+      const float* bp = &Wf[lk][l32];
+      static_assert(stem_fwd_off(STEM_TAPS - 1) + 1 - 2 * FCW == 18 * FCW + 7, "the zero row's operand");
+#define STEM_FWD_A(J)                                                                                               \
+  ((2 * (J) + 1 >= STEM_TAPS || stem_fwd_off(2 * (J) + 1) - stem_fwd_off(2 * (J)) == 1 - 2 * FCW ? sp2              \
+    : stem_fwd_off(2 * (J) + 1) - stem_fwd_off(2 * (J)) == FCW                                   ? sp1              \
+                                                                                                  : sp3)[stem_fwd_off(2 * (J))])
+      float a0 = STEM_FWD_A(0), b00 = bp[0], b01 = bp[32];
+#pragma unroll
+      for (int j = 0; j < FKP; ++j) {
+        const int nx = j + 1 < FKP ? j + 1 : j;
+        const float a1 = STEM_FWD_A(nx), b10 = bp[nx * 128], b11 = bp[nx * 128 + 32];
+        __builtin_amdgcn_sched_barrier(0);
+        acc[0] = __builtin_amdgcn_mfma_f32_32x32x2f32(a0, b00, acc[0], 0, 0, 0);
+        acc[1] = __builtin_amdgcn_mfma_f32_32x32x2f32(a0, b01, acc[1], 0, 0, 0);
+        __builtin_amdgcn_sched_barrier(0);
+        a0 = a1;
+        b00 = b10;
+        b01 = b11;
+      }
+#undef STEM_FWD_A
+      float* o = out + obase + l32;
+#pragma unroll
+      for (int e = 0; e < 16; ++e) {
+        const int p = p0 + 8 * (e >> 2) + 4 * lk + (e & 3);
+        if (p < len) {
+          o[p * g.ld_out] = acc[0][e];
+          o[p * g.ld_out + 32] = acc[1][e];
+        }
+      }
+    }
+    if (more) {
+      store_chunk(buf ^ 1);
+      __syncthreads();
+      buf ^= 1;
+      len = llen;
+      obase = lout;
+    } else {
+      len = 0;
+    }
+  }
+}
+MOPA_API int mopa_stem_fwd(const float* in, const float* weight, float* out, const int32_t* geom_host, void* stream) {
+  ConvGeom g;
+  memcpy(&g, geom_host, sizeof(g));
+  if (!stem_strip_geom(g) || g.KS != 1 || g.KH0 != 0 || g.KW0 != 0 || g.KWF != 2 || g.ld_out < 64 || !in || !weight || !out)
+    return MOPA_ERR_ARG;
+  if ((((uintptr_t)in | (uintptr_t)weight) & 15) != 0 || ((uintptr_t)out & 3) != 0) return MOPA_ERR_ARG;
+  if ((int64_t)FSP * g.ld_out >= (1ll << 31)) return MOPA_ERR_ARG;
+  const int64_t nchunks = (int64_t)g.B * g.OHl * ((g.OWl + FSP - 1) / FSP);
+  if (nchunks >= (1ll << 31)) return MOPA_ERR_ARG;
+  const int64_t cpb = cdiv64(nchunks, 1024);
+  k_stem_fwd_strip<<<(unsigned)cdiv64(nchunks, cpb), 256, 0, (hipStream_t)stream>>>(in, weight, out, g, (int)cpb, (int)nchunks);
+  MOPA_CHECK_LAUNCH();
+  return MOPA_OK;
 }
 
 __global__ __launch_bounds__(256) void k_wino_dw(const float* __restrict__ slabs, int nsplit, int64_t n, float* __restrict__ dw,
diff --git a/mopa_amd/csrc/exec_table.inc b/mopa_amd/csrc/exec_table.inc
--- a/mopa_amd/csrc/exec_table.inc
+++ b/mopa_amd/csrc/exec_table.inc
@@ -112,6 +112,7 @@
   "mopa_stem_bwd_weight_bn",
   "mopa_stem_bwd_weight_bn2",
   "mopa_stem_dgrad_image",
+  "mopa_stem_fwd",
   "mopa_vgi_box_free",
   "mopa_vgi_candidates",
   "mopa_vgi_compact_cells",
@@ -145,7 +146,7 @@
   "mopa_wino_weight",
   "mopa_zero_rows",
 };
-static const int EXEC_N = 145;
+static const int EXEC_N = 146;
 static int exec_dispatch(int id, const int64_t* a, int nargs) {
   switch (id) {
     case 0: return nargs == 6 ? mopa_a2d2prep_map((const double*)(uintptr_t)a[0], (int32_t)a[1], (int32_t)a[2], (int16_t*)(uintptr_t)a[3], (uint16_t*)(uintptr_t)a[4], (void*)(uintptr_t)a[5]) : MOPA_ERR_ARG;
@@ -261,38 +262,39 @@
     case 110: return nargs == 15 ? mopa_stem_bwd_weight_bn((const float*)(uintptr_t)a[0], (const float*)(uintptr_t)a[1], (int32_t)a[2], (const float*)(uintptr_t)a[3], (int32_t)a[4], (const float*)(uintptr_t)a[5], (const float*)(uintptr_t)a[6], (int32_t)a[7], (int32_t)a[8], (float*)(uintptr_t)a[9], (const int32_t*)(uintptr_t)a[10], (int32_t)a[11], (void*)(uintptr_t)a[12], (size_t)a[13], (void*)(uintptr_t)a[14]) : MOPA_ERR_ARG;
     case 111: return nargs == 15 ? mopa_stem_bwd_weight_bn2((const float*)(uintptr_t)a[0], (const float*)(uintptr_t)a[1], (int32_t)a[2], (const float*)(uintptr_t)a[3], (int32_t)a[4], (const float*)(uintptr_t)a[5], (const float*)(uintptr_t)a[6], (int32_t)a[7], (int32_t)a[8], (float*)(uintptr_t)a[9], (const int32_t*)(uintptr_t)a[10], (int32_t)a[11], (void*)(uintptr_t)a[12], (size_t)a[13], (void*)(uintptr_t)a[14]) : MOPA_ERR_ARG;
     case 112: return nargs == 10 ? mopa_stem_dgrad_image((const float*)(uintptr_t)a[0], (int32_t)a[1], (int32_t)a[2], (int32_t)a[3], (int32_t)a[4], (int32_t)a[5], (int32_t)a[6], (const float*)(uintptr_t)a[7], (float*)(uintptr_t)a[8], (void*)(uintptr_t)a[9]) : MOPA_ERR_ARG;
-    case 113: return nargs == 13 ? mopa_vgi_box_free((const int32_t*)(uintptr_t)a[0], (int32_t)a[1], (int32_t)a[2], (int32_t)a[3], (int32_t)a[4], (int32_t)a[5], (int32_t)a[6], (int32_t)a[7], (int32_t)a[8], (uint8_t*)(uintptr_t)a[9], (void*)(uintptr_t)a[10], (size_t)a[11], (void*)(uintptr_t)a[12]) : MOPA_ERR_ARG;
-    case 114: return nargs == 13 ? mopa_vgi_candidates((const uint8_t*)(uintptr_t)a[0], (int32_t)a[1], (int32_t)a[2], (int32_t)a[3], (const double*)(uintptr_t)a[4], (const uint8_t*)(uintptr_t)a[5], (int32_t)a[6], (int32_t)a[7], (int32_t)a[8], (int32_t)a[9], (uint8_t*)(uintptr_t)a[10], (int32_t*)(uintptr_t)a[11], (void*)(uintptr_t)a[12]) : MOPA_ERR_ARG;
-    case 115: return nargs == 8 ? mopa_vgi_compact_cells((const uint8_t*)(uintptr_t)a[0], (int32_t)a[1], (int32_t)a[2], (int32_t)a[3], (int32_t)a[4], (int32_t*)(uintptr_t)a[5], (int32_t*)(uintptr_t)a[6], (void*)(uintptr_t)a[7]) : MOPA_ERR_ARG;
-    case 116: return nargs == 13 ? mopa_vgi_first_points((const float*)(uintptr_t)a[0], (int32_t)a[1], (int32_t)a[2], (float)slot_f(a[3]), (int32_t)a[4], (int32_t)a[5], (int32_t)a[6], (int32_t)a[7], (int32_t)a[8], (const uint8_t*)(uintptr_t)a[9], (int32_t*)(uintptr_t)a[10], (int32_t*)(uintptr_t)a[11], (void*)(uintptr_t)a[12]) : MOPA_ERR_ARG;
-    case 117: return nargs == 15 ? mopa_vgi_first_points_rep((const float*)(uintptr_t)a[0], (int32_t)a[1], (int32_t)a[2], (float)slot_f(a[3]), (double)slot_f(a[4]), (int32_t)a[5], (int32_t)a[6], (int32_t)a[7], (int32_t)a[8], (int32_t)a[9], (int32_t*)(uintptr_t)a[10], (int32_t*)(uintptr_t)a[11], (void*)(uintptr_t)a[12], (size_t)a[13], (void*)(uintptr_t)a[14]) : MOPA_ERR_ARG;
-    case 118: return nargs == 6 ? mopa_vgi_ground_cells((const int32_t*)(uintptr_t)a[0], (const uint8_t*)(uintptr_t)a[1], (int32_t)a[2], (int32_t)a[3], (uint8_t*)(uintptr_t)a[4], (void*)(uintptr_t)a[5]) : MOPA_ERR_ARG;
-    case 119: return nargs == 11 ? mopa_vgi_range_keep((const double*)(uintptr_t)a[0], (int32_t)a[1], (int32_t)a[2], (double)slot_f(a[3]), (double)slot_f(a[4]), (int32_t)a[5], (int32_t)a[6], (uint8_t*)(uintptr_t)a[7], (void*)(uintptr_t)a[8], (size_t)a[9], (void*)(uintptr_t)a[10]) : MOPA_ERR_ARG;
-    case 120: return nargs == 15 ? mopa_vgi_road_height((const float*)(uintptr_t)a[0], (int32_t)a[1], (int32_t)a[2], (float)slot_f(a[3]), (const int32_t*)(uintptr_t)a[4], (const uint8_t*)(uintptr_t)a[5], (int32_t)a[6], (int32_t)a[7], (int32_t)a[8], (int32_t)a[9], (int32_t)a[10], (int32_t)a[11], (int32_t)a[12], (double*)(uintptr_t)a[13], (void*)(uintptr_t)a[14]) : MOPA_ERR_ARG;
-    case 121: return nargs == 12 ? mopa_voxel_hash_build((const int64_t*)(uintptr_t)a[0], (int64_t)a[1], (uint64_t*)(uintptr_t)a[2], (int32_t*)(uintptr_t)a[3], (int64_t)a[4], (int32_t*)(uintptr_t)a[5], (uint64_t*)(uintptr_t)a[6], (int32_t*)(uintptr_t)a[7], (int32_t*)(uintptr_t)a[8], (void*)(uintptr_t)a[9], (size_t)a[10], (void*)(uintptr_t)a[11]) : MOPA_ERR_ARG;
-    case 122: return nargs == 12 ? mopa_voxelize((const float*)(uintptr_t)a[0], (int32_t)a[1], (float)slot_f(a[2]), (int32_t)a[3], (const double*)(uintptr_t)a[4], (int32_t)a[5], (int64_t)a[6], (int64_t*)(uintptr_t)a[7], (uint8_t*)(uintptr_t)a[8], (void*)(uintptr_t)a[9], (size_t)a[10], (void*)(uintptr_t)a[11]) : MOPA_ERR_ARG;
-    case 123: return nargs == 14 ? mopa_voxelize_f64((const double*)(uintptr_t)a[0], (int32_t)a[1], (const uint8_t*)(uintptr_t)a[2], (const double*)(uintptr_t)a[3], (double)slot_f(a[4]), (int32_t)a[5], (const double*)(uintptr_t)a[6], (int32_t)a[7], (int64_t)a[8], (int64_t*)(uintptr_t)a[9], (uint8_t*)(uintptr_t)a[10], (void*)(uintptr_t)a[11], (size_t)a[12], (void*)(uintptr_t)a[13]) : MOPA_ERR_ARG;
-    case 124: return nargs == 10 ? mopa_wce_bwd((const float*)(uintptr_t)a[0], (const int64_t*)(uintptr_t)a[1], (const float*)(uintptr_t)a[2], (int32_t)a[3], (int32_t)a[4], (int64_t)a[5], (const float*)(uintptr_t)a[6], (const float*)(uintptr_t)a[7], (float*)(uintptr_t)a[8], (void*)(uintptr_t)a[9]) : MOPA_ERR_ARG;
-    case 125: return nargs == 12 ? mopa_wce_fwd((const float*)(uintptr_t)a[0], (const int64_t*)(uintptr_t)a[1], (const float*)(uintptr_t)a[2], (int32_t)a[3], (int32_t)a[4], (int64_t)a[5], (float*)(uintptr_t)a[6], (float*)(uintptr_t)a[7], (int32_t*)(uintptr_t)a[8], (void*)(uintptr_t)a[9], (size_t)a[10], (void*)(uintptr_t)a[11]) : MOPA_ERR_ARG;
-    case 126: return nargs == 10 ? mopa_wino4_bwd_weight((const float*)(uintptr_t)a[0], (const float*)(uintptr_t)a[1], (int32_t)a[2], (int32_t)a[3], (int32_t)a[4], (float*)(uintptr_t)a[5], (int32_t)a[6], (void*)(uintptr_t)a[7], (size_t)a[8], (void*)(uintptr_t)a[9]) : MOPA_ERR_ARG;
-    case 127: return nargs == 17 ? mopa_wino4_conv((const float*)(uintptr_t)a[0], (int32_t)a[1], (const float*)(uintptr_t)a[2], (const float*)(uintptr_t)a[3], (float*)(uintptr_t)a[4], (int32_t)a[5], (int32_t)a[6], (int32_t)a[7], (int32_t)a[8], (int32_t)a[9], (int32_t)a[10], (int32_t)a[11], (const float*)(uintptr_t)a[12], (int32_t)a[13], (int32_t)a[14], (float*)(uintptr_t)a[15], (void*)(uintptr_t)a[16]) : MOPA_ERR_ARG;
-    case 128: return nargs == 16 ? mopa_wino4_conv9((const float*)(uintptr_t)a[0], (int32_t)a[1], (const float*)(uintptr_t)a[2], (const float*)(uintptr_t)a[3], (float*)(uintptr_t)a[4], (int32_t)a[5], (int32_t)a[6], (int32_t)a[7], (int32_t)a[8], (int32_t)a[9], (int32_t)a[10], (int32_t)a[11], (const float*)(uintptr_t)a[12], (int32_t)a[13], (int32_t)a[14], (void*)(uintptr_t)a[15]) : MOPA_ERR_ARG;
-    case 129: return nargs == 8 ? mopa_wino4_dout((const float*)(uintptr_t)a[0], (int32_t)a[1], (int32_t)a[2], (int32_t)a[3], (int32_t)a[4], (int32_t)a[5], (float*)(uintptr_t)a[6], (void*)(uintptr_t)a[7]) : MOPA_ERR_ARG;
-    case 130: return nargs == 12 ? mopa_wino4_gemm_output((const float*)(uintptr_t)a[0], (const float*)(uintptr_t)a[1], (const float*)(uintptr_t)a[2], (float*)(uintptr_t)a[3], (int32_t)a[4], (int32_t)a[5], (int32_t)a[6], (int32_t)a[7], (int32_t)a[8], (int32_t)a[9], (int32_t)a[10], (void*)(uintptr_t)a[11]) : MOPA_ERR_ARG;
-    case 131: return nargs == 8 ? mopa_wino4_input((const float*)(uintptr_t)a[0], (int32_t)a[1], (int32_t)a[2], (int32_t)a[3], (int32_t)a[4], (int32_t)a[5], (float*)(uintptr_t)a[6], (void*)(uintptr_t)a[7]) : MOPA_ERR_ARG;
-    case 132: return nargs == 11 ? mopa_wino4_input_bn((const float*)(uintptr_t)a[0], (int32_t)a[1], (int32_t)a[2], (int32_t)a[3], (int32_t)a[4], (int32_t)a[5], (const float*)(uintptr_t)a[6], (int32_t)a[7], (int32_t)a[8], (float*)(uintptr_t)a[9], (void*)(uintptr_t)a[10]) : MOPA_ERR_ARG;
-    case 133: return nargs == 10 ? mopa_wino4_output((const float*)(uintptr_t)a[0], (int32_t)a[1], (int32_t)a[2], (int32_t)a[3], (int32_t)a[4], (const float*)(uintptr_t)a[5], (float*)(uintptr_t)a[6], (int32_t)a[7], (int32_t)a[8], (void*)(uintptr_t)a[9]) : MOPA_ERR_ARG;
-    case 134: return nargs == 6 ? mopa_wino4_weight((const float*)(uintptr_t)a[0], (int32_t)a[1], (int32_t)a[2], (int32_t)a[3], (float*)(uintptr_t)a[4], (void*)(uintptr_t)a[5]) : MOPA_ERR_ARG;
-    case 135: return nargs == 6 ? mopa_wino4_weight_f((const float*)(uintptr_t)a[0], (int32_t)a[1], (int32_t)a[2], (int32_t)a[3], (float*)(uintptr_t)a[4], (void*)(uintptr_t)a[5]) : MOPA_ERR_ARG;
-    case 136: return nargs == 6 ? mopa_wino4_weight_q((const float*)(uintptr_t)a[0], (int32_t)a[1], (int32_t)a[2], (int32_t)a[3], (float*)(uintptr_t)a[4], (void*)(uintptr_t)a[5]) : MOPA_ERR_ARG;
-    case 137: return nargs == 6 ? mopa_wino4_weight_t((const float*)(uintptr_t)a[0], (int32_t)a[1], (int32_t)a[2], (int32_t)a[3], (float*)(uintptr_t)a[4], (void*)(uintptr_t)a[5]) : MOPA_ERR_ARG;
-    case 138: return nargs == 17 ? mopa_wino4_wgrad_fused((const float*)(uintptr_t)a[0], (int32_t)a[1], (const float*)(uintptr_t)a[2], (int32_t)a[3], (int32_t)a[4], (const float*)(uintptr_t)a[5], (int32_t)a[6], (int32_t)a[7], (int32_t)a[8], (int32_t)a[9], (int32_t)a[10], (int32_t)a[11], (float*)(uintptr_t)a[12], (int32_t)a[13], (void*)(uintptr_t)a[14], (size_t)a[15], (void*)(uintptr_t)a[16]) : MOPA_ERR_ARG;
-    case 139: return nargs == 10 ? mopa_wino_bwd_weight((const float*)(uintptr_t)a[0], (const float*)(uintptr_t)a[1], (int32_t)a[2], (int32_t)a[3], (int32_t)a[4], (float*)(uintptr_t)a[5], (int32_t)a[6], (void*)(uintptr_t)a[7], (size_t)a[8], (void*)(uintptr_t)a[9]) : MOPA_ERR_ARG;
-    case 140: return nargs == 8 ? mopa_wino_dout((const float*)(uintptr_t)a[0], (int32_t)a[1], (int32_t)a[2], (int32_t)a[3], (int32_t)a[4], (int32_t)a[5], (float*)(uintptr_t)a[6], (void*)(uintptr_t)a[7]) : MOPA_ERR_ARG;
-    case 141: return nargs == 8 ? mopa_wino_input((const float*)(uintptr_t)a[0], (int32_t)a[1], (int32_t)a[2], (int32_t)a[3], (int32_t)a[4], (int32_t)a[5], (float*)(uintptr_t)a[6], (void*)(uintptr_t)a[7]) : MOPA_ERR_ARG;
-    case 142: return nargs == 10 ? mopa_wino_output((const float*)(uintptr_t)a[0], (int32_t)a[1], (int32_t)a[2], (int32_t)a[3], (int32_t)a[4], (const float*)(uintptr_t)a[5], (float*)(uintptr_t)a[6], (int32_t)a[7], (int32_t)a[8], (void*)(uintptr_t)a[9]) : MOPA_ERR_ARG;
-    case 143: return nargs == 6 ? mopa_wino_weight((const float*)(uintptr_t)a[0], (int32_t)a[1], (int32_t)a[2], (int32_t)a[3], (float*)(uintptr_t)a[4], (void*)(uintptr_t)a[5]) : MOPA_ERR_ARG;
-    case 144: return nargs == 5 ? mopa_zero_rows((float*)(uintptr_t)a[0], (int32_t)a[1], (int64_t)a[2], (int32_t)a[3], (void*)(uintptr_t)a[4]) : MOPA_ERR_ARG;
+    case 113: return nargs == 5 ? mopa_stem_fwd((const float*)(uintptr_t)a[0], (const float*)(uintptr_t)a[1], (float*)(uintptr_t)a[2], (const int32_t*)(uintptr_t)a[3], (void*)(uintptr_t)a[4]) : MOPA_ERR_ARG;
+    case 114: return nargs == 13 ? mopa_vgi_box_free((const int32_t*)(uintptr_t)a[0], (int32_t)a[1], (int32_t)a[2], (int32_t)a[3], (int32_t)a[4], (int32_t)a[5], (int32_t)a[6], (int32_t)a[7], (int32_t)a[8], (uint8_t*)(uintptr_t)a[9], (void*)(uintptr_t)a[10], (size_t)a[11], (void*)(uintptr_t)a[12]) : MOPA_ERR_ARG;
+    case 115: return nargs == 13 ? mopa_vgi_candidates((const uint8_t*)(uintptr_t)a[0], (int32_t)a[1], (int32_t)a[2], (int32_t)a[3], (const double*)(uintptr_t)a[4], (const uint8_t*)(uintptr_t)a[5], (int32_t)a[6], (int32_t)a[7], (int32_t)a[8], (int32_t)a[9], (uint8_t*)(uintptr_t)a[10], (int32_t*)(uintptr_t)a[11], (void*)(uintptr_t)a[12]) : MOPA_ERR_ARG;
+    case 116: return nargs == 8 ? mopa_vgi_compact_cells((const uint8_t*)(uintptr_t)a[0], (int32_t)a[1], (int32_t)a[2], (int32_t)a[3], (int32_t)a[4], (int32_t*)(uintptr_t)a[5], (int32_t*)(uintptr_t)a[6], (void*)(uintptr_t)a[7]) : MOPA_ERR_ARG;
+    case 117: return nargs == 13 ? mopa_vgi_first_points((const float*)(uintptr_t)a[0], (int32_t)a[1], (int32_t)a[2], (float)slot_f(a[3]), (int32_t)a[4], (int32_t)a[5], (int32_t)a[6], (int32_t)a[7], (int32_t)a[8], (const uint8_t*)(uintptr_t)a[9], (int32_t*)(uintptr_t)a[10], (int32_t*)(uintptr_t)a[11], (void*)(uintptr_t)a[12]) : MOPA_ERR_ARG;
+    case 118: return nargs == 15 ? mopa_vgi_first_points_rep((const float*)(uintptr_t)a[0], (int32_t)a[1], (int32_t)a[2], (float)slot_f(a[3]), (double)slot_f(a[4]), (int32_t)a[5], (int32_t)a[6], (int32_t)a[7], (int32_t)a[8], (int32_t)a[9], (int32_t*)(uintptr_t)a[10], (int32_t*)(uintptr_t)a[11], (void*)(uintptr_t)a[12], (size_t)a[13], (void*)(uintptr_t)a[14]) : MOPA_ERR_ARG;
+    case 119: return nargs == 6 ? mopa_vgi_ground_cells((const int32_t*)(uintptr_t)a[0], (const uint8_t*)(uintptr_t)a[1], (int32_t)a[2], (int32_t)a[3], (uint8_t*)(uintptr_t)a[4], (void*)(uintptr_t)a[5]) : MOPA_ERR_ARG;
+    case 120: return nargs == 11 ? mopa_vgi_range_keep((const double*)(uintptr_t)a[0], (int32_t)a[1], (int32_t)a[2], (double)slot_f(a[3]), (double)slot_f(a[4]), (int32_t)a[5], (int32_t)a[6], (uint8_t*)(uintptr_t)a[7], (void*)(uintptr_t)a[8], (size_t)a[9], (void*)(uintptr_t)a[10]) : MOPA_ERR_ARG;
+    case 121: return nargs == 15 ? mopa_vgi_road_height((const float*)(uintptr_t)a[0], (int32_t)a[1], (int32_t)a[2], (float)slot_f(a[3]), (const int32_t*)(uintptr_t)a[4], (const uint8_t*)(uintptr_t)a[5], (int32_t)a[6], (int32_t)a[7], (int32_t)a[8], (int32_t)a[9], (int32_t)a[10], (int32_t)a[11], (int32_t)a[12], (double*)(uintptr_t)a[13], (void*)(uintptr_t)a[14]) : MOPA_ERR_ARG;
+    case 122: return nargs == 12 ? mopa_voxel_hash_build((const int64_t*)(uintptr_t)a[0], (int64_t)a[1], (uint64_t*)(uintptr_t)a[2], (int32_t*)(uintptr_t)a[3], (int64_t)a[4], (int32_t*)(uintptr_t)a[5], (uint64_t*)(uintptr_t)a[6], (int32_t*)(uintptr_t)a[7], (int32_t*)(uintptr_t)a[8], (void*)(uintptr_t)a[9], (size_t)a[10], (void*)(uintptr_t)a[11]) : MOPA_ERR_ARG;
+    case 123: return nargs == 12 ? mopa_voxelize((const float*)(uintptr_t)a[0], (int32_t)a[1], (float)slot_f(a[2]), (int32_t)a[3], (const double*)(uintptr_t)a[4], (int32_t)a[5], (int64_t)a[6], (int64_t*)(uintptr_t)a[7], (uint8_t*)(uintptr_t)a[8], (void*)(uintptr_t)a[9], (size_t)a[10], (void*)(uintptr_t)a[11]) : MOPA_ERR_ARG;
+    case 124: return nargs == 14 ? mopa_voxelize_f64((const double*)(uintptr_t)a[0], (int32_t)a[1], (const uint8_t*)(uintptr_t)a[2], (const double*)(uintptr_t)a[3], (double)slot_f(a[4]), (int32_t)a[5], (const double*)(uintptr_t)a[6], (int32_t)a[7], (int64_t)a[8], (int64_t*)(uintptr_t)a[9], (uint8_t*)(uintptr_t)a[10], (void*)(uintptr_t)a[11], (size_t)a[12], (void*)(uintptr_t)a[13]) : MOPA_ERR_ARG;
+    case 125: return nargs == 10 ? mopa_wce_bwd((const float*)(uintptr_t)a[0], (const int64_t*)(uintptr_t)a[1], (const float*)(uintptr_t)a[2], (int32_t)a[3], (int32_t)a[4], (int64_t)a[5], (const float*)(uintptr_t)a[6], (const float*)(uintptr_t)a[7], (float*)(uintptr_t)a[8], (void*)(uintptr_t)a[9]) : MOPA_ERR_ARG;
+    case 126: return nargs == 12 ? mopa_wce_fwd((const float*)(uintptr_t)a[0], (const int64_t*)(uintptr_t)a[1], (const float*)(uintptr_t)a[2], (int32_t)a[3], (int32_t)a[4], (int64_t)a[5], (float*)(uintptr_t)a[6], (float*)(uintptr_t)a[7], (int32_t*)(uintptr_t)a[8], (void*)(uintptr_t)a[9], (size_t)a[10], (void*)(uintptr_t)a[11]) : MOPA_ERR_ARG;
+    case 127: return nargs == 10 ? mopa_wino4_bwd_weight((const float*)(uintptr_t)a[0], (const float*)(uintptr_t)a[1], (int32_t)a[2], (int32_t)a[3], (int32_t)a[4], (float*)(uintptr_t)a[5], (int32_t)a[6], (void*)(uintptr_t)a[7], (size_t)a[8], (void*)(uintptr_t)a[9]) : MOPA_ERR_ARG;
+    case 128: return nargs == 17 ? mopa_wino4_conv((const float*)(uintptr_t)a[0], (int32_t)a[1], (const float*)(uintptr_t)a[2], (const float*)(uintptr_t)a[3], (float*)(uintptr_t)a[4], (int32_t)a[5], (int32_t)a[6], (int32_t)a[7], (int32_t)a[8], (int32_t)a[9], (int32_t)a[10], (int32_t)a[11], (const float*)(uintptr_t)a[12], (int32_t)a[13], (int32_t)a[14], (float*)(uintptr_t)a[15], (void*)(uintptr_t)a[16]) : MOPA_ERR_ARG;
+    case 129: return nargs == 16 ? mopa_wino4_conv9((const float*)(uintptr_t)a[0], (int32_t)a[1], (const float*)(uintptr_t)a[2], (const float*)(uintptr_t)a[3], (float*)(uintptr_t)a[4], (int32_t)a[5], (int32_t)a[6], (int32_t)a[7], (int32_t)a[8], (int32_t)a[9], (int32_t)a[10], (int32_t)a[11], (const float*)(uintptr_t)a[12], (int32_t)a[13], (int32_t)a[14], (void*)(uintptr_t)a[15]) : MOPA_ERR_ARG;
+    case 130: return nargs == 8 ? mopa_wino4_dout((const float*)(uintptr_t)a[0], (int32_t)a[1], (int32_t)a[2], (int32_t)a[3], (int32_t)a[4], (int32_t)a[5], (float*)(uintptr_t)a[6], (void*)(uintptr_t)a[7]) : MOPA_ERR_ARG;
+    case 131: return nargs == 12 ? mopa_wino4_gemm_output((const float*)(uintptr_t)a[0], (const float*)(uintptr_t)a[1], (const float*)(uintptr_t)a[2], (float*)(uintptr_t)a[3], (int32_t)a[4], (int32_t)a[5], (int32_t)a[6], (int32_t)a[7], (int32_t)a[8], (int32_t)a[9], (int32_t)a[10], (void*)(uintptr_t)a[11]) : MOPA_ERR_ARG;
+    case 132: return nargs == 8 ? mopa_wino4_input((const float*)(uintptr_t)a[0], (int32_t)a[1], (int32_t)a[2], (int32_t)a[3], (int32_t)a[4], (int32_t)a[5], (float*)(uintptr_t)a[6], (void*)(uintptr_t)a[7]) : MOPA_ERR_ARG;
+    case 133: return nargs == 11 ? mopa_wino4_input_bn((const float*)(uintptr_t)a[0], (int32_t)a[1], (int32_t)a[2], (int32_t)a[3], (int32_t)a[4], (int32_t)a[5], (const float*)(uintptr_t)a[6], (int32_t)a[7], (int32_t)a[8], (float*)(uintptr_t)a[9], (void*)(uintptr_t)a[10]) : MOPA_ERR_ARG;
+    case 134: return nargs == 10 ? mopa_wino4_output((const float*)(uintptr_t)a[0], (int32_t)a[1], (int32_t)a[2], (int32_t)a[3], (int32_t)a[4], (const float*)(uintptr_t)a[5], (float*)(uintptr_t)a[6], (int32_t)a[7], (int32_t)a[8], (void*)(uintptr_t)a[9]) : MOPA_ERR_ARG;
+    case 135: return nargs == 6 ? mopa_wino4_weight((const float*)(uintptr_t)a[0], (int32_t)a[1], (int32_t)a[2], (int32_t)a[3], (float*)(uintptr_t)a[4], (void*)(uintptr_t)a[5]) : MOPA_ERR_ARG;
+    case 136: return nargs == 6 ? mopa_wino4_weight_f((const float*)(uintptr_t)a[0], (int32_t)a[1], (int32_t)a[2], (int32_t)a[3], (float*)(uintptr_t)a[4], (void*)(uintptr_t)a[5]) : MOPA_ERR_ARG;
+    case 137: return nargs == 6 ? mopa_wino4_weight_q((const float*)(uintptr_t)a[0], (int32_t)a[1], (int32_t)a[2], (int32_t)a[3], (float*)(uintptr_t)a[4], (void*)(uintptr_t)a[5]) : MOPA_ERR_ARG;
+    case 138: return nargs == 6 ? mopa_wino4_weight_t((const float*)(uintptr_t)a[0], (int32_t)a[1], (int32_t)a[2], (int32_t)a[3], (float*)(uintptr_t)a[4], (void*)(uintptr_t)a[5]) : MOPA_ERR_ARG;
+    case 139: return nargs == 17 ? mopa_wino4_wgrad_fused((const float*)(uintptr_t)a[0], (int32_t)a[1], (const float*)(uintptr_t)a[2], (int32_t)a[3], (int32_t)a[4], (const float*)(uintptr_t)a[5], (int32_t)a[6], (int32_t)a[7], (int32_t)a[8], (int32_t)a[9], (int32_t)a[10], (int32_t)a[11], (float*)(uintptr_t)a[12], (int32_t)a[13], (void*)(uintptr_t)a[14], (size_t)a[15], (void*)(uintptr_t)a[16]) : MOPA_ERR_ARG;
+    case 140: return nargs == 10 ? mopa_wino_bwd_weight((const float*)(uintptr_t)a[0], (const float*)(uintptr_t)a[1], (int32_t)a[2], (int32_t)a[3], (int32_t)a[4], (float*)(uintptr_t)a[5], (int32_t)a[6], (void*)(uintptr_t)a[7], (size_t)a[8], (void*)(uintptr_t)a[9]) : MOPA_ERR_ARG;
+    case 141: return nargs == 8 ? mopa_wino_dout((const float*)(uintptr_t)a[0], (int32_t)a[1], (int32_t)a[2], (int32_t)a[3], (int32_t)a[4], (int32_t)a[5], (float*)(uintptr_t)a[6], (void*)(uintptr_t)a[7]) : MOPA_ERR_ARG;
+    case 142: return nargs == 8 ? mopa_wino_input((const float*)(uintptr_t)a[0], (int32_t)a[1], (int32_t)a[2], (int32_t)a[3], (int32_t)a[4], (int32_t)a[5], (float*)(uintptr_t)a[6], (void*)(uintptr_t)a[7]) : MOPA_ERR_ARG;
+    case 143: return nargs == 10 ? mopa_wino_output((const float*)(uintptr_t)a[0], (int32_t)a[1], (int32_t)a[2], (int32_t)a[3], (int32_t)a[4], (const float*)(uintptr_t)a[5], (float*)(uintptr_t)a[6], (int32_t)a[7], (int32_t)a[8], (void*)(uintptr_t)a[9]) : MOPA_ERR_ARG;
+    case 144: return nargs == 6 ? mopa_wino_weight((const float*)(uintptr_t)a[0], (int32_t)a[1], (int32_t)a[2], (int32_t)a[3], (float*)(uintptr_t)a[4], (void*)(uintptr_t)a[5]) : MOPA_ERR_ARG;
+    case 145: return nargs == 5 ? mopa_zero_rows((float*)(uintptr_t)a[0], (int32_t)a[1], (int64_t)a[2], (int32_t)a[3], (void*)(uintptr_t)a[4]) : MOPA_ERR_ARG;
     default: return MOPA_ERR_ARG;
   }
 }
diff --git a/mopa_amd/dense2d.py b/mopa_amd/dense2d.py
--- a/mopa_amd/dense2d.py
+++ b/mopa_amd/dense2d.py
@@ -550,6 +550,14 @@
 STEM_BN_FUSED_BWD = os.environ.get("MOPA_STEM_BN_FUSED_BWD", "1") != "0" and os.environ.get("MOPA_CONV2D_MFMA", "1") != "0"
 STEM_BWD2 = frozenset({"1": ("wgrad", "pool"), "0": ()}.get(os.environ.get("MOPA_STEM_BWD2", "1"), (os.environ.get("MOPA_STEM_BWD2"),)))
 STEM_BWD2_MIN_PIXELS = int(os.environ.get("MOPA_STEM_BWD2_MIN_PIXELS", str(1 << 17)))
+STEM_PACKED = os.environ.get("MOPA_STEM_PACKED", "1") != "0"
+
+
+def stem_forward(x_ptr, w, out_ptr, geom):
+    if STEM_PACKED and _CONV2D_MFMA and geom[0] * geom[1] * geom[2] < 1 << 29:
+        call("mopa_stem_fwd", x_ptr, ptr(w), out_ptr, ctypes.addressof(geom), stream())
+    else:
+        igemm(x_ptr, w, None, out_ptr, geom)
 BN_MASK_BITS = os.environ.get("MOPA_BN_MASK_BITS", "1") != "0"
 BN_COLSUM_FUSED = os.environ.get("MOPA_BN_COLSUM_FUSED", "1") != "0"
 
@@ -756,7 +764,7 @@
     c1 = Img(J[0], B, Hp, Wp, 0, 64) if lazy_stem else new_img(B, Hp, Wp, 64, dev)
     stem_g = _geom(B=B, IH=Hp + 6, IW=Wp + 8, OHl=Hp, OWl=Wp, OHa=Hp, OWa=Wp, IDX=4, TH=7, TW=2, KWF=2, Cin=16,
                    Cout=64, ld_in=4, ld_out=c1.ld)
-    igemm(ptr(x4), w1, None, c1.p, stem_g)
+    stem_forward(ptr(x4), w1, c1.p, stem_g)
     bn1 = BnOp(P, pre + "bn1", G=G, stem_grid=(B, Hp, Wp))
     tape.append(("stem", x4, c1, stem_g, bn1))
     H2, W2 = Hp // 2, Wp // 2
```

New measurement: 422.1 (median of 6 runs). 1.01x the previous value.
